# johnpeterflynn/surface-texture-inpainting-net

Hardware: AMD Instinct MI355X
Metric: vertices/sec forward+backward on 200k-vert ScanNet mesh; scatter-add GB/s vs HBM roofline (higher is better)
Workload: dtype f32; 1 GPU; STINet 3-D config, synthetic mesh 200704 vertices / 1200642 directed edges / 3 levels per GPU, step = plan build + fwd + L1 + bwd + all-reduce + Adam; vertices_per_gpu=200704, edges_per_gpu=1200642, levels=3, parallelism=dp1, hip_graph=False

## Files before the change

include/stin_hip.h:

```cpp
#ifndef STIN_HIP_H
#define STIN_HIP_H

#include <stddef.h>
#include <stdint.h>

#ifdef __cplusplus
extern "C" {
#endif

#define STIN_VERSION 102

#define STIN_OK 0
#define STIN_E_NULL (-1)
#define STIN_E_SIZE (-2)
#define STIN_E_ALIGN (-3)
#define STIN_E_WORKSPACE (-4)
#define STIN_E_UNSUPPORTED (-5)

typedef void* stin_stream_t;
typedef void* stin_event_t;
typedef uint16_t stin_bf16_t;

int stin_version(void);
const char* stin_error_string(int code);
// ... 44 lines not shown
int stin_relabel_many_i64(const stin_relabel_job_t* jobs, int n_jobs, stin_stream_t stream);
int stin_narrow_i64_to_i32(const int64_t* src, int64_t n, int64_t limit, int32_t* dst, int32_t* bad,
                           stin_stream_t stream);

#define STIN_SEG_NONTEMPORAL 2
int stin_segment_sum_f32(const float* src, int64_t ld_src, const int32_t* rowptr, const int32_t* col,
                         int64_t N, int C, int mean, float* out, int64_t ld_out, stin_stream_t stream);

int stin_edge_relu_mean_fwd_f32(const float* A, int64_t lda, const float* B, int64_t ldb,
                                const int32_t* rowptr, const int32_t* col, int64_t N, int H,
                                float* out, int64_t ldo, int indicator, uint32_t* mask, stin_stream_t stream);
int stin_edge_relu_mean_fwd_map_f32(const float* A, int64_t lda, const float* B, int64_t ldb, const int32_t* rowptr,
                                    const int32_t* col, const int32_t* row_map, int64_t N, int H, float* out, int64_t ldo,
                                    int indicator, uint32_t* mask, stin_stream_t stream);
int stin_edge_relu_mean_bwd_dst_mask_f32(const float* G, int64_t ldg, const uint32_t* mask, const int32_t* rowptr,
                                         int64_t N, int H, float* dA, int64_t ldda, stin_stream_t stream);
int stin_edge_relu_mean_bwd_src_mask_f32(const float* G, int64_t ldg, const float* w_src, const uint32_t* mask,
                                         const int32_t* rowptr_src, const int32_t* col_src, const int32_t* xslot,
                                         int64_t N, int H, float* dB, int64_t lddb, stin_stream_t stream);
int stin_edge_relu_mean_bwd_mask_f32(const float* G, int64_t ldg, const uint32_t* mask, const int32_t* rowptr_dst,
                                     const float* w_src, const int32_t* rowptr_src, const int32_t* col_src,
                                     const int32_t* xslot, int64_t N, int H, float* dA, int64_t ldda, float* dB,
                                     int64_t lddb, const float* copy_src, int64_t ld_copy_src, float* copy_dst,
                                     int64_t ld_copy_dst, int C_copy, stin_stream_t stream);
int stin_edge_relu_mean_fwd_ti_f32(const float* b1, const float* B, int64_t ldb, const int32_t* rowptr, const int32_t* col,
                                   int64_t N, int H, float* out, int64_t ldo, int indicator, uint32_t* mask, stin_stream_t stream);
int64_t stin_edge_bwd_ti_colsum_rows(int64_t N, int H);
int stin_edge_bwd_ti_colsum_fold_f32(const float* colsum, int64_t rows, int H, float* db1, stin_stream_t stream);
int stin_edge_relu_mean_bwd_mask_ti_f32(const float* G, int64_t ldg, const uint32_t* mask, const int32_t* rowptr_dst,
                                        const float* w_src, const int32_t* rowptr_src, const int32_t* col_src,
                                        const int32_t* xslot, int64_t N, int H, float* D, int64_t ldd, const float* copy_src,
                                        int64_t ld_copy_src, float* copy_dst, int64_t ld_copy_dst, int C_copy, float* colsum,
                                        int64_t colsum_rows, stin_stream_t stream);
int stin_edge_relu_mean_bwd_dst_f32(const float* A, int64_t lda, const float* B, int64_t ldb,
                                    const float* G, int64_t ldg, const int32_t* rowptr,
                                    const int32_t* col, int64_t N, int H, float* dA, int64_t ldda,
                                    stin_stream_t stream);
int stin_edge_relu_mean_bwd_src_f32(const float* A, int64_t lda, const float* B, int64_t ldb,
                                    const float* G, int64_t ldg, const float* inv_deg,
                                    const int32_t* rowptr_src, const int32_t* col_src, int64_t N, int H,
                                    float* dB, int64_t lddb, stin_stream_t stream);

int stin_pool_max_fwd_f32(const float* x, int64_t ldx, const int32_t* rowptr, const int32_t* col,
                          int64_t n_coarse, int C, float* out, int64_t ldo, int32_t* arg,
                          stin_stream_t stream);
int stin_pool_max_bwd_f32(const float* g, int64_t ldg, const int32_t* arg, const int32_t* trace,
                          int64_t n_fine, int C, float* gx, int64_t ldgx, stin_stream_t stream);
int stin_gather_rows_f32(const float* src, int64_t ld_src, const int32_t* idx, const float* row_scale,
                         int64_t n_out, int C, float* out, int64_t ldo, stin_stream_t stream);
int stin_gather_add_rows_f32(const float* a, int64_t lda, const int32_t* idx_a, const float* b, int64_t ldb,
                             const int32_t* idx_b, int64_t n_out, int C, float* out, int64_t ldo, stin_stream_t stream);
int64_t stin_segment_mean_stats_groups(int64_t N, int C);
int stin_segment_mean_stats_f32(const float* src, int64_t ld_src, const int32_t* rowptr, const int32_t* col, int64_t N, int C,
                                float* out, int64_t ldo, double* partial, size_t partial_bytes, stin_stream_t stream);
int64_t stin_gather_add_rows_stats_groups(int64_t N, int C);
int stin_gather_add_rows_stats_f32(const float* a, int64_t lda, const int32_t* idx_a, const float* b, int64_t ldb,
                                   const int32_t* idx_b, int64_t N, int C, float* out, int64_t ldo, double* partial,
                                   size_t partial_bytes, stin_stream_t stream);
int stin_batch_pool_i64(const int64_t* batch, const int32_t* rowptr, const int32_t* col, int64_t n_coarse,
                        int64_t* out, stin_stream_t stream);
int stin_gather_i64(const int64_t* src, const int32_t* idx, int64_t n_out, int64_t* out,
                    stin_stream_t stream);
int stin_norm_group_ids_i64(const int64_t* batch, const int32_t* ptr_sum, int B, int64_t n_rows, int32_t* gid, int32_t* sid,
                            stin_stream_t stream);

#define STIN_RED_SUM 0
#define STIN_RED_CSQ 1
#define STIN_RED_DOT_ELU 2
#define STIN_RED_COEF_XC 3
#define STIN_RED_MOMENTS 4
#define STIN_RED_DOT_BN 5
#define STIN_RED_DOT_BN_RELU 6
#define STIN_POST_NONE 0
#define STIN_POST_SCALE 1
#define STIN_POST_RSTD 2
#define STIN_POST_NORM_COEF 3
size_t stin_colreduce_workspace_bytes(int C, int B);
int stin_colreduce_f32(int mode, const float* x, int64_t ldx, const float* gout, int64_t ldg, int64_t N,
                       int C, const int32_t* ptr, int B, const int32_t* gid, const int32_t* sid,
                       const float* mean, const float* rstd, const float* coef, int post,
                       const float* inv_cnt, float eps, float* out0, float* out1,
                       void* workspace, size_t workspace_bytes, stin_stream_t stream);
int stin_norm_act_res_fwd_f32(const float* x, int64_t ldx, const float* mean, const float* rstd,
                              const int32_t* gid, const float* res, int64_t ldres, int64_t N, int C, int act,
                              float* y, int64_t ldy, stin_stream_t stream);
int stin_norm_act_res_fwd_map_f32(const float* x, int64_t ldx, const float* mean, const float* rstd, const int32_t* gid,
                                  const float* res, int64_t ldres, const int32_t* row_map, int64_t N, int C, int act, float* y,
                                  int64_t ldy, stin_stream_t stream);
int stin_norm_act_bwd_f32(const float* x, int64_t ldx, const float* gout, int64_t ldg, const float* mean,
                          const float* rstd, const float* a, const float* k, const float* m,
                          const int32_t* gid, const int32_t* sid, int64_t N, int C, int act, float* dx,
                          int64_t lddx, stin_stream_t stream);

#define STIN_GEMM_F32 0
#define STIN_GEMM_BF16X3 2
#define STIN_GEMM_BF16X6 3
#define STIN_GEMM_F16X3 4
#define STIN_GEMM_W_BF16 0x200
#define STIN_GEMM_W_PRESPLIT 0x100
#define STIN_GEMM_W_FRAG 0x400
int stin_gemm_w_is_frag(int Nc, int K);
int stin_gemm_split_weights_f32(const float* W, int64_t ldw, int Nc, int K, int precision, float* out, int64_t ldo,
                                stin_stream_t stream);
int stin_gemm_nt_f32(const float* A, int64_t lda, const float* W, int64_t ldw, const float* bias,
                     const float* row_mask, int64_t ld_mask, const float* residual, int64_t ld_res, int64_t M,
                     int Nc, int K, float* C, int64_t ldc, int precision, stin_stream_t stream);
size_t stin_gemm_tn_workspace_bytes(int64_t M, int Nc, int K, int ones_column);
int stin_gemm_tn_f32(const float* G, int64_t ldg, const float* X, int64_t ldx, int64_t M, int Nc, int K,
                     int ones_column, const float* row_weight, int64_t ld_weight, float* dW, int64_t lddw,
                     int precision, void* workspace, size_t workspace_bytes, stin_stream_t stream);

int stin_gemm_tn_wb_f32(const float* G, int64_t ldg, const float* X, int64_t ldx, int64_t M, int Nc, int K,
                        const float* row_weight, int64_t ld_weight, float* dW, int64_t lddw, float* db, int precision,
                        void* workspace, size_t workspace_bytes, stin_stream_t stream);

size_t stin_linear_tanh_bwd_workspace_bytes(int64_t N, int K, int Nc);
int stin_linear_tanh_fwd_f32(const float* x, int64_t ldx, const float* W, const float* b, int64_t N, int K, int Nc, float* y,
                             stin_stream_t stream);
int stin_linear_tanh_bwd_f32(const float* g, const float* y, const float* x, int64_t ldx, const float* W, int64_t N, int K, int Nc,
                             float* dx, int64_t lddx, float* dW, float* db, void* workspace, size_t workspace_bytes,
                             stin_stream_t stream);

int stin_cols_axpy_rowmask_f32(float* dst, int64_t ldd, const float* src, int64_t lds, const int32_t* rowptr, int64_t N, int c0,
                               int c1, float alpha, stin_stream_t stream);
int stin_cols_axpy_rowmask_bf16(stin_bf16_t* dst, int64_t ldd, const stin_bf16_t* src, int64_t lds, const int32_t* rowptr,
                                int64_t N, int c0, int c1, float alpha, stin_stream_t stream);

int stin_pad_rows_f32(const float* x, int64_t ldx, int64_t N, int Cin, int Cp, float* out, stin_stream_t stream);
int stin_pad_rows_bf16(const stin_bf16_t* x, int64_t ldx, int64_t N, int Cin, int Cp, stin_bf16_t* out, stin_stream_t stream);

int64_t stin_gemm_nt_dotelu_groups(int64_t M, int Nc, int K, int precision);
int stin_gemm_nt_dotelu_f32(const float* A, int64_t lda, const float* W, int64_t ldw, const float* bias, const float* residual,
                            int64_t ld_res, int64_t M, int Nc, int K, float* C, int64_t ldc, int precision, const float* nx,
                            int64_t ld_nx, const float* nmean, const float* nrstd, double* partial, size_t partial_bytes,
                            stin_stream_t stream);
int stin_norm_coef_from_partials_f32(const double* partial, int64_t groups, int C, const float* rstd, const float* inv_cnt,
                                     float* k, float* m, stin_stream_t stream);

int stin_bn_act_fwd_f32(const float* x, int64_t ldx, const float* mean, const float* rstd, const float* gamma,
                        const float* beta, int64_t N, int C, int act, float* y, int64_t ldy, stin_stream_t stream);
int stin_bn_act_bwd_f32(const float* x, int64_t ldx, const float* gout, int64_t ldg, const float* mean, const float* rstd,
                        const float* gamma, const float* beta, const float* P, const float* Q, float inv_n, int64_t N,
                        int C, int act, float* dx, int64_t lddx, stin_stream_t stream);

int stin_bn_mean_bwd_f32(const float* m, int64_t ldm, const float* g, int64_t ldg, const int32_t* dst, const float* inv_deg,
                         const float* mean, const float* rstd, const float* gamma, const float* P, const float* Q,
                         float inv_e, int64_t E, int C, float* dm, int64_t lddm, stin_stream_t stream);

int stin_bn_running_stats_f32(const float* mean, const float* rstd, int C, float eps, float unbias, float momentum,
                              float* running_mean, float* running_var, stin_stream_t stream);

int stin_gemm_nt_bn_f32(const float* A, int64_t lda, const float* W, int64_t ldw, const float* mean, const float* rstd,
                        const float* gamma, const float* beta, int64_t M, int Nc, int K, float* C, int64_t ldc, int precision,
                        stin_stream_t stream);
int stin_gemm_tn_bn_f32(const float* G, int64_t ldg, const float* X, int64_t ldx, const float* mean, const float* rstd,
                        const float* gamma, const float* beta, int64_t M, int Nc, int K, float* dW, int64_t lddw, int precision,
                        void* workspace, size_t workspace_bytes, stin_stream_t stream);
int stin_gemm_nt_stream_f32(const float* A, int64_t lda, const float* W, int64_t ldw, const float* mean, const float* rstd,
                            const float* gamma, const float* beta, int64_t M, int Nc, int K, float* C, int64_t ldc, int precision,
                            stin_stream_t stream);
int64_t stin_gemm_nt_bn_bwd_groups(int64_t M, int Nc, int K, int precision);
int stin_gemm_nt_bn_bwd_stats_f32(const float* A, int64_t lda, const float* W, int64_t ldw, const float* X, int64_t ldx,
                                  const float* mean, const float* rstd, const float* gamma, const float* beta, int64_t M, int Nc,
                                  int K, int precision, double* partial, size_t partial_bytes, float* sums, stin_stream_t stream);
int stin_gemm_nt_bn_bwd_apply_f32(const float* A, int64_t lda, const float* W, int64_t ldw, const float* X, int64_t ldx,
                                  const float* mean, const float* rstd, const float* gamma, const float* beta, const float* sums,
                                  float inv_n, int64_t M, int Nc, int K, float* dx, int64_t lddx, int precision,
                                  stin_stream_t stream);
int stin_scmn_pack_f32(const float* W1, const float* W2, const float* gamma1, const float* beta1, const float* gamma2,
                       const float* beta2, int cin, int h2, int cout, int trans_inv, float* wcat, float* wcatT, float* w2T,
                       float* gb1, float* gb2, stin_stream_t stream);
int stin_scmn_unpack_f32(const float* dwcat, int cin, int h2, int trans_inv, float* dW1, stin_stream_t stream);
int stin_bn_affine_res_fwd_f32(const float* x, int64_t ldx, const float* mean, const float* rstd, const float* gamma,
                               const float* beta, const int32_t* rowptr, const float* res, int64_t ldres, int64_t N, int C,
                               int relu, float* y, int64_t ldy, stin_stream_t stream);
int stin_relu_mask_bwd_f32(const float* g, int64_t ldg, const float* y, int64_t ldy, const int32_t* rowptr, int64_t N, int C,
                           int relu, float* g_eff, float* g_in, stin_stream_t stream);
int stin_concat_unpool_f32(const float* skip, int64_t ld_skip, const float* coarse, int64_t ld_coarse, const int32_t* trace, int64_t N,
                           int cs, int cu, float* out, int64_t ldo, stin_stream_t stream);

typedef struct stin_pack_job {
    const float *W1, *b1, *Ws, *bs, *W2;
    float *wcat, *bcat, *wcatT, *w2T, *w2s;
    int Cin, Cp, H, Cout, has_shortcut, trans_inv, fwd_split, bwd_split;
} stin_pack_job_t;
int stin_edgeconv_pack_many_f32(const stin_pack_job_t* jobs_device, int n_jobs, int64_t max_elems, stin_stream_t stream);
int stin_edgeconv_pack_f32(const float* W1, const float* b1, const float* Ws, const float* bs, const float* W2,
                           int Cin, int Cp, int H, int Cout, int has_shortcut, int trans_inv, float* wcat,
                           float* bcat, float* wcatT, float* w2T, float* w2s, int fwd_split, int bwd_split,
                           stin_stream_t stream);
int stin_edgeconv_unpack_grads_f32(const float* dwb, const float* dw2b, int Cin, int Cp, int H, int Cout,
                                   int has_shortcut, int trans_inv, float* dW1, float* db1, float* dWs, float* dbs,
                                   float* dW2, float* db2, stin_stream_t stream);
int stin_norm_bwd_coef_f32(const float* T1, const float* S0, const float* rstd, const float* inv_cnt, int B, int C,
                           float* k, float* m, stin_stream_t stream);
int stin_norm_bwd_coef_m_quirk_f32(const float* S0, const float* U, const float* rstd, const float* inv_cnt, int B, int C,
                                   float* m, stin_stream_t stream);

size_t stin_masked_l1_workspace_bytes(int64_t N, int C);
int stin_masked_l1_loss_f32(const float* out, const float* color, const int64_t* mask, int64_t N, int C,
                            int use_weight, float* loss, float* grad, void* workspace, size_t workspace_bytes,
                            stin_stream_t stream);
#define STIN_SEG_MIN_CLASSES 2
#define STIN_SEG_MAX_CLASSES 128
size_t stin_seg_ce_workspace_bytes(int64_t N);
int stin_seg_ce_fwd_f32(const float* logits, int64_t ld, int64_t M, const int64_t* rows, const int64_t* target, int64_t N, int C,
                        const float* weight, int64_t ignore_index, float* loss, double* den, int64_t* confusion, int32_t* bad,
                        void* workspace, size_t workspace_bytes, stin_stream_t stream);
int stin_seg_ce_bwd_f32(const float* logits, int64_t ld, const int64_t* target, int64_t N, int C, const float* weight,
                        int64_t ignore_index, const float* grad_loss, const double* den, float* dlogits, int64_t ldd,
                        stin_stream_t stream);
size_t stin_total_variation_workspace_bytes(int64_t N);
int stin_total_variation_f32(const float* x, int64_t ldx, const int32_t* rowptr_dst, const int32_t* col_dst, int64_t N, int C,
                             float* out, void* workspace, size_t workspace_bytes, stin_stream_t stream);
int stin_graph_laplace_f32(const float* x, int64_t ldx, const int32_t* rowptr_dst, const int32_t* col_dst, int64_t N, int C,
                           float* out, int64_t ldo, stin_stream_t stream);
#define STIN_METRICS_ONE_PASS 0
#define STIN_METRICS_STAGED 1
size_t stin_inpaint_metrics_workspace_bytes(int64_t N);
int stin_inpaint_metrics_f32(const float* out, int64_t ldo, const float* color, const int64_t* mask, const int32_t* rowptr_dst,
                             const int32_t* col_dst, const int32_t* perm, int64_t N, int C, int composite, int use_weight,
                             float data_range, const float* loss, int layout, float* row_out, void* workspace,
                             size_t workspace_bytes, stin_stream_t stream);
int stin_adam_f32(float* p, const float* g, float* m, float* v, float* vmax, int64_t n, double lr, double beta1,
                  double beta2, double eps, double weight_decay, int step, int amsgrad, stin_stream_t stream);

int64_t stin_gemm_nt_colstats_groups(int64_t M, int Nc, int K, int precision);
int stin_gemm_nt_colstats_f32(const float* A, int64_t lda, const float* W, int64_t ldw, const float* bias,
                              const float* row_mask, int64_t ld_mask, const float* residual, int64_t ld_res, int64_t M,
                              int Nc, int K, float* C, int64_t ldc, int precision, double* colstats, size_t colstats_bytes,
                              stin_stream_t stream);
int stin_moments_final_f32(const double* partial, int64_t groups, int C, const float* inv_cnt, float eps, float* mean,
                           float* rstd, stin_stream_t stream);
int stin_norm_fold_rows(int64_t N, int C, int64_t groups);
int stin_norm_act_res_fwd_fold_f32(const double* partial, int64_t groups, const float* x, int64_t ldx, const float* res,
                                   int64_t ldres, const float* inv_cnt, float eps, int64_t N, int C, float* mean, float* rstd,
                                   float* y, int64_t ldy, stin_stream_t stream);
int stin_norm_act_res_fwd_fold_map_f32(const double* partial, int64_t groups, const float* x, int64_t ldx, const float* res,
                                       int64_t ldres, const int32_t* row_map, const float* inv_cnt, float eps, int64_t N, int C,
                                       float* mean, float* rstd, float* y, int64_t ldy, stin_stream_t stream);
int stin_norm_act_bwd_fold_f32(const double* partial, int64_t groups, const float* x, int64_t ldx, const float* gout, int64_t ldg,
                               const float* mean, const float* rstd, const float* inv_cnt, int64_t N, int C, float* dx,
                               int64_t lddx, stin_stream_t stream);

int stin_segment_sum_bf16(const stin_bf16_t* src, int64_t ld_src, const int32_t* rowptr, const int32_t* col,
                          int64_t n_rows, int C, int mean, stin_bf16_t* out, int64_t ld_out, stin_stream_t stream);
int stin_edge_relu_mean_fwd_bf16(const stin_bf16_t* A, int64_t lda, const stin_bf16_t* B, int64_t ldb,
                                 const int32_t* rowptr, const int32_t* col, int64_t N, int H, stin_bf16_t* out,
                                 int64_t ldo, int indicator, uint32_t* mask, stin_stream_t stream);
int stin_edge_relu_mean_bwd_dst_mask_bf16(const stin_bf16_t* G, int64_t ldg, const uint32_t* mask,
                                          const int32_t* rowptr, int64_t N, int H, stin_bf16_t* dA, int64_t ldda,
                                          stin_stream_t stream);
int stin_edge_relu_mean_bwd_src_mask_bf16(const stin_bf16_t* G, int64_t ldg, const float* w_src, const uint32_t* mask,
                                          const int32_t* rowptr_src, const int32_t* col_src, const int32_t* xslot,
                                          int64_t N, int H, stin_bf16_t* dB, int64_t lddb, stin_stream_t stream);
int stin_edge_relu_mean_bwd_mask_bf16(const stin_bf16_t* G, int64_t ldg, const uint32_t* mask, const int32_t* rowptr_dst,
                                      const float* w_src, const int32_t* rowptr_src, const int32_t* col_src,
                                      const int32_t* xslot, int64_t N, int H, stin_bf16_t* dA, int64_t ldda,
                                      stin_bf16_t* dB, int64_t lddb, const stin_bf16_t* copy_src, int64_t ld_copy_src,
                                      stin_bf16_t* copy_dst, int64_t ld_copy_dst, int C_copy, stin_stream_t stream);
int stin_pool_max_fwd_bf16(const stin_bf16_t* x, int64_t ldx, const int32_t* rowptr, const int32_t* col,
                           int64_t n_coarse, int C, stin_bf16_t* out, int64_t ldo, int32_t* arg, stin_stream_t stream);
int stin_pool_max_bwd_bf16(const stin_bf16_t* g, int64_t ldg, const int32_t* arg, const int32_t* trace,
                           int64_t n_fine, int C, stin_bf16_t* gx, int64_t ldgx, stin_stream_t stream);
int stin_gather_rows_bf16(const stin_bf16_t* src, int64_t ld_src, const int32_t* idx, const float* row_scale,
                          int64_t n_out, int C, stin_bf16_t* out, int64_t ldo, stin_stream_t stream);
int stin_colreduce_bf16(int mode, const stin_bf16_t* x, int64_t ldx, const stin_bf16_t* gout, int64_t ldg, int64_t N,
                        int C, const int32_t* ptr, int B, const int32_t* gid, const int32_t* sid, const float* mean,
                        const float* rstd, const float* coef, int post, const float* inv_cnt, float eps, float* out0,
                        float* out1, void* workspace, size_t workspace_bytes, stin_stream_t stream);
int stin_norm_act_res_fwd_bf16(const stin_bf16_t* x, int64_t ldx, const float* mean, const float* rstd,
                               const int32_t* gid, const stin_bf16_t* res, int64_t ldres, int64_t N, int C, int act,
                               stin_bf16_t* y, int64_t ldy, stin_stream_t stream);
int stin_norm_act_bwd_bf16(const stin_bf16_t* x, int64_t ldx, const stin_bf16_t* gout, int64_t ldg, const float* mean,
                           const float* rstd, const float* a, const float* k, const float* m, const int32_t* gid,
                           const int32_t* sid, int64_t N, int C, int act, stin_bf16_t* dx, int64_t lddx,
                           stin_stream_t stream);
int stin_gemm_nt_bf16(const stin_bf16_t* A, int64_t lda, const float* W, int64_t ldw, const float* bias,
                      const stin_bf16_t* row_mask, int64_t ld_mask, const stin_bf16_t* residual, int64_t ld_res,
                      int64_t M, int Nc, int K, void* C, int64_t ldc, int c_is_f32, stin_stream_t stream);
int stin_gemm_tn_bf16(const stin_bf16_t* G, int64_t ldg, const stin_bf16_t* X, int64_t ldx, int64_t M, int Nc, int K,
                      int ones_column, const stin_bf16_t* row_weight, int64_t ld_weight, float* dW, int64_t lddw,
                      void* workspace, size_t workspace_bytes, stin_stream_t stream);
int stin_gemm_tn_wb_bf16(const stin_bf16_t* G, int64_t ldg, const stin_bf16_t* X, int64_t ldx, int64_t M, int Nc, int K,
                         const stin_bf16_t* row_weight, int64_t ld_weight, float* dW, int64_t lddw, float* db,
                         void* workspace, size_t workspace_bytes, stin_stream_t stream);
int stin_linear_tanh_fwd_bf16(const stin_bf16_t* x, int64_t ldx, const float* W, const float* b, int64_t N, int K, int Nc,
                              float* y, stin_stream_t stream);
int stin_linear_tanh_bwd_bf16(const float* g, const float* y, const stin_bf16_t* x, int64_t ldx, const float* W, int64_t N, int K,
                              int Nc, stin_bf16_t* dx, int64_t lddx, float* dW, float* db, void* workspace,
                              size_t workspace_bytes, stin_stream_t stream);

#define STIN_TI_COMPACT 2
#define STIN_BLOCK_PACKED 0x800
size_t stin_edgeconv_block_fwd_workspace_bytes(int Cin, int Cp, int H, int Cout, int has_shortcut, int B);
int stin_edgeconv_block_fwd_pack_offsets(int Cp, int H, int Cout, int has_shortcut, size_t* off_wcat, size_t* off_w2s,
                                         size_t* off_bcat);
size_t stin_edgeconv_block_bwd_workspace_bytes(int64_t N, int Cp, int H, int Cout, int has_shortcut, int B, int storage);
#define STIN_OP_BLOCK 0
#define STIN_OP_POOL_MAX 1
#define STIN_OP_UNPOOL 2
typedef struct stin_net_op {
    int32_t kind, Cin, Cp, H, Cout, has_shortcut, trans_inv, prec_fwd, fwd_split, bwd_split, B, slice_quirk, use_side, y_from_src,
        reserved1, reserved2;
    float eps;
    int32_t reserved3;
    int64_t n_out, n_in, ldx, ldo, lddx, ldy, ldh;
    uint64_t fwd_ws_bytes, bwd_ws_bytes;
    const void* x;
    void* out;
    void* dx;
    const float *W1, *b1, *W2, *b2, *Ws, *bs;
    float *wcatT, *w2T;
    void* fwd_ws;
    const int32_t *rowptr_dst, *col_dst, *rowptr_src, *col_src, *xslot;
    const float* w_src;
    const int32_t *ptr_sum, *ptr_true, *gid, *sid;
    const float* inv_cnt;
    void *Y, *hE;
    uint32_t* mask;
    void* agg;
    float *mean, *rstd;
    int32_t* arg;
    const int32_t* trace;
    float *dW1, *db1, *dW2, *db2, *dWs, *dbs;
    void* bwd_ws;
    stin_event_t ev_dy, ev_done;
    stin_event_t ev_edge0, ev_edge1;
} stin_net_op_t;
int stin_net_fwd(int storage, const stin_net_op_t* ops, int n_ops, stin_stream_t stream);
int stin_net_bwd(int storage, const stin_net_op_t* ops, int n_ops, const void* g, int64_t ldg, int prec_bwd, stin_stream_t stream,
                 stin_stream_t wgrad_stream);

size_t stin_edgeconv_wgrad_workspace_bytes(int64_t N, int Cp, int H, int Cout, int has_shortcut);
int stin_edgeconv_wgrad(int storage, const void* dagg, int64_t ld_dagg, const void* hE, int64_t ldh, const void* dY,
                        int64_t ldy, const void* x, int64_t ldx, int64_t N, int Cin, int Cp, int H, int Cout,
                        int has_shortcut, int trans_inv, int precision, float* dW1, float* db1, float* dW2, float* db2,
                        float* dWs, float* dbs, void* workspace, size_t workspace_bytes, stin_stream_t stream);
int stin_edgeconv_wgrad_ti(int storage, const void* dagg, int64_t ld_dagg, const void* hE, int64_t ldh, const void* dY,
                           int64_t ldy, const void* x, int64_t ldx, int64_t N, int Cin, int Cp, int H, int Cout,
                           int has_shortcut, int trans_inv, int precision, float* dW1, float* db1, float* dW2, float* db2,
                           float* dWs, float* dbs, const float* ti_colsum, int64_t ti_rows, void* workspace,
                           size_t workspace_bytes, stin_stream_t stream);

int stin_dilated_walk_f32(const int32_t* rowptr, const int32_t* col, const int32_t* row_of, const float* pos,
                          const float* nrm, int64_t N, int64_t E, const int32_t* dilations, int n_dil, int32_t* out,
                          stin_stream_t stream);
int stin_dilated_walk_f64(const int32_t* rowptr, const int32_t* col, const int32_t* row_of, const double* pos,
                          const double* nrm, int64_t N, int64_t E, const int32_t* dilations, int n_dil, int32_t* out,
                          stin_stream_t stream);

size_t stin_voxel_cluster_workspace_bytes(int64_t N);
int stin_voxel_cluster_f64(const double* coords, int64_t N, double voxel, int64_t* trace, float* new_coords, int64_t* state,
                           void* workspace, size_t workspace_bytes, stin_stream_t stream);
size_t stin_coalesce_workspace_bytes(int64_t E);
int stin_coalesce_pairs_i64(const int64_t* a, const int64_t* b, const int64_t* map, int64_t map_n, int64_t E, int64_t n, int drop_loops,
                            int64_t* out_a, int64_t* out_b, int64_t* state, void* workspace, size_t workspace_bytes,
                            stin_stream_t stream);

size_t stin_mask_adjacency_workspace_bytes(int64_t N);
int stin_mask_adjacency_i64(const int64_t* src, const int64_t* dst, int64_t E, int64_t N, int32_t* rowptr, int32_t* col,
                            int32_t* bad, void* workspace, size_t workspace_bytes, stin_stream_t stream);
size_t stin_circle_mask_workspace_bytes(int64_t N, int num_masks, int num_graphs);
int stin_circle_mask_run(const int32_t* rowptr, const int32_t* col, int64_t N, const int64_t* ptr, int num_graphs, int num_masks,
                         int radius, double frac, uint64_t seed, const int64_t* graph_seeds, int max_iters, const int64_t* centres,
                         int64_t num_centres,
                         int32_t* dist, int64_t* mask, int64_t* info, int64_t* centre_log, int64_t log_cap, void* workspace,
                         size_t workspace_bytes, stin_stream_t stream);
int stin_augment_rewrite_f32(float* x, int64_t ldx, const float* color, int64_t ldc, const int32_t* dist, int radius, int64_t* mask,
                             int64_t N, const float* lin, const float* rot, stin_stream_t stream);

#define STIN_CROP_VERTICES 0
#define STIN_CROP_EDGES 1
#define STIN_CROP_DILATED 2
#define STIN_CROP_OCCURS 3
#define STIN_CROP_TRACE 4
#define STIN_CROP_MAX_SEGS 1024
#define STIN_CROP_MAX_CROPS 65535
typedef struct stin_crop_seg {
    int64_t kind, level, vseg, aux, n, base, width, ibase;
    const void* src;
    void* out;
    int64_t* ids_out;
    void *p0, *p1;
    int64_t reserved[3];
} stin_crop_seg_t;
size_t stin_crop_workspace_bytes(int64_t total);
int stin_crop_mark(const stin_crop_seg_t* segs, int n_segs, int64_t max_n, const double* boxes, int n_crops, int64_t total,
                   int64_t inbox_total, uint8_t* inbox, uint8_t* flags, int32_t* pos, int64_t* bounds, int32_t* status,
                   void* workspace, size_t workspace_bytes, stin_stream_t stream);
int stin_crop_gather(const stin_crop_seg_t* segs, int n_segs, int64_t max_n, int n_crops, const uint8_t* flags, const int32_t* pos,
                     stin_stream_t stream);
int stin_crop_traces(const stin_crop_seg_t* segs, int n_segs, int64_t max_n, int n_crops, const uint8_t* flags, const int32_t* pos,
                     int32_t* info, int32_t* status, stin_stream_t stream);
size_t stin_label_pool_workspace_bytes(int64_t n0, int n_labels);
int stin_label_pool_i64(const int64_t* trace0, const int64_t* labels, int64_t n_orig, int64_t n0, int n_labels, int64_t* out,
                        int32_t* status, void* workspace, size_t workspace_bytes, stin_stream_t stream);

int stin_nearest_chunks(int64_t Q, int64_t P);
size_t stin_nearest_workspace_bytes(int64_t Q, int chunks);
int stin_nearest_f64(const double* queries, int64_t n_query_rows, const double* points, int64_t P, const int64_t* q_index,
                     const int64_t* q_count, int64_t Q, int chunks, int64_t* out_index, double* out_d2, int64_t* flags,
                     void* workspace, size_t workspace_bytes, stin_stream_t stream);
size_t stin_trace_workspace_bytes(int64_t n_old, int64_t n_new);
int stin_trace_scatter_i64(const int64_t* new_id, const int64_t* row_ptr, int64_t R, const int64_t* old_id, const int64_t* row_of,
                           int64_t n_entries, int64_t n_old, int64_t n_new, int64_t* trace, int64_t* state, void* workspace,
                           size_t workspace_bytes, stin_stream_t stream);
int stin_trace_unassigned_i64(const int64_t* trace, int64_t n_old, int64_t* list, int64_t* state, stin_stream_t stream);
int stin_trace_check_i64(const int64_t* trace, int64_t n_old, const int64_t* row_ptr, int64_t R, int64_t n_new, int64_t* state,
                         void* workspace, size_t workspace_bytes, stin_stream_t stream);
int stin_cluster_mean_f32(const float* coords, int64_t n, const int64_t* order, const int64_t* seg_ptr, int64_t n_seg, float* out,
                          stin_stream_t stream);

#ifdef __cplusplus
}
#endif
#endif
```

surface_texture_inpainting_net_amd/csrc/stin_block.hip:

```cpp
#include "stin_common.h"

namespace {

inline size_t up256(size_t v) { return (v + 255) & ~(size_t)255; }
inline char* align256(void* p) { return reinterpret_cast<char*>((reinterpret_cast<uintptr_t>(p) + 255) & ~(uintptr_t)255); }
inline char* carve(char*& p, size_t bytes) {
    char* r = p;
    p += up256(bytes);
    return r;
}
#define STIN_TRY(expr)            \
    do {                          \
        const int rc_ = (expr);   \
        if (rc_ != STIN_OK) return rc_; \
    } while (0)

inline const void* col_off(const void* base, int64_t cols, int storage) {
    return static_cast<const char*>(base) + cols * (storage ? 2 : 4);
}

inline size_t yw_wide(int H, int Cout, int has_shortcut) { return 2 * (size_t)H + (has_shortcut ? Cout : 0); }

struct BwdLayout {
    size_t dagg, dhE, dY;
    size_t coef[5];
    size_t red, red_bytes;
    size_t tn;
};
inline BwdLayout bwd_layout(int64_t N, int H, int Cout, int has_shortcut, int B, int storage) {
    const size_t es = storage ? 2 : 4;
    BwdLayout L;
    size_t o = 0;
    auto take = [&o](size_t bytes) {
        const size_t r = o;
        o += up256(bytes);
        return r;
    };
    L.dagg = take((size_t)N * Cout * es);
    L.dhE = take((size_t)N * H * es);
    L.dY = take((size_t)N * yw_wide(H, Cout, has_shortcut) * es);
    for (size_t& c : L.coef) c = take((size_t)B * Cout * 4);
    L.red_bytes = stin_colreduce_workspace_bytes(Cout, B);
    L.red = take(L.red_bytes);
    L.tn = o;
    return L;
}

inline int colreduce(int storage, int mode, const void* x, int64_t ldx, const void* gout, int64_t ldg, int64_t N, int C, const int32_t* ptr,
                     int B, const int32_t* gid, const int32_t* sid, const float* mean, const float* rstd, const float* coef, int post,
                     const float* inv_cnt, float eps, float* out0, float* out1, void* ws, size_t ws_bytes, stin_stream_t stream) {
    if (storage)
        return stin_colreduce_bf16(mode, static_cast<const stin_bf16_t*>(x), ldx, static_cast<const stin_bf16_t*>(gout), ldg, N, C, ptr, B,
                                   gid, sid, mean, rstd, coef, post, inv_cnt, eps, out0, out1, ws, ws_bytes, stream);
    return stin_colreduce_f32(mode, static_cast<const float*>(x), ldx, static_cast<const float*>(gout), ldg, N, C, ptr, B, gid, sid, mean,
                              rstd, coef, post, inv_cnt, eps, out0, out1, ws, ws_bytes, stream);
}

int fwd_stats(int storage, const stin_net_op_t& J, void* red_ws, size_t red_bytes, stin_stream_t stream) {
    if (!J.slice_quirk)
        return colreduce(storage, STIN_RED_MOMENTS, J.agg, J.Cout, nullptr, 0, J.n_out, J.Cout, J.ptr_sum, J.B, J.gid, nullptr, nullptr,
                         nullptr, nullptr, STIN_POST_NONE, J.inv_cnt, J.eps, J.mean, J.rstd, red_ws, red_bytes, stream);
    STIN_TRY(colreduce(storage, STIN_RED_SUM, J.agg, J.Cout, nullptr, 0, J.n_out, J.Cout, J.ptr_sum, J.B, J.gid, nullptr, nullptr, nullptr,
                       nullptr, STIN_POST_SCALE, J.inv_cnt, J.eps, J.mean, nullptr, red_ws, red_bytes, stream));
    return colreduce(storage, STIN_RED_CSQ, J.agg, J.Cout, nullptr, 0, J.n_out, J.Cout, J.ptr_sum, J.B, J.gid, nullptr, J.mean, nullptr,
                     nullptr, STIN_POST_RSTD, J.inv_cnt, J.eps, J.rstd, nullptr, red_ws, red_bytes, stream);
}

int bwd_norm_coef(int storage, const stin_net_op_t& J, const void* g, int64_t ldg, float* const coef[5], void* red_ws, size_t red_bytes,
                  stin_stream_t stream) {
    float *kk = coef[0], *mm = coef[1], *t1 = coef[2], *s0 = coef[3], *uu = coef[4];
    if (!J.sid)
        return colreduce(storage, STIN_RED_DOT_ELU, J.agg, J.Cout, g, ldg, J.n_out, J.Cout, J.ptr_true, J.B, J.gid, nullptr, J.mean, J.rstd,
                         nullptr, STIN_POST_NORM_COEF, J.inv_cnt, 0.f, kk, mm, red_ws, red_bytes, stream);
    STIN_TRY(colreduce(storage, STIN_RED_DOT_ELU, J.agg, J.Cout, g, ldg, J.n_out, J.Cout, J.ptr_true, J.B, J.gid, nullptr, J.mean, J.rstd,
                       nullptr, STIN_POST_NONE, J.inv_cnt, 0.f, t1, s0, red_ws, red_bytes, stream));
    STIN_TRY(stin_norm_bwd_coef_f32(t1, s0, J.rstd, J.inv_cnt, J.B, J.Cout, kk, mm, stream));
    STIN_TRY(colreduce(storage, STIN_RED_COEF_XC, J.agg, J.Cout, nullptr, 0, J.n_out, J.Cout, J.ptr_true, J.B, J.gid, J.sid, J.mean, nullptr,
                       kk, STIN_POST_NONE, J.inv_cnt, 0.f, uu, nullptr, red_ws, red_bytes, stream));
    return stin_norm_bwd_coef_m_quirk_f32(s0, uu, J.rstd, J.inv_cnt, J.B, J.Cout, mm, stream);
}

#define STIN_EDGE_BRACKET(CALL)                                                               \
    do {                                                                                      \
        if (J.ev_edge0) (void)hipEventRecord((hipEvent_t)J.ev_edge0, (hipStream_t)stream);    \
        STIN_TRY(CALL);                                                                       \
        if (J.ev_edge1) (void)hipEventRecord((hipEvent_t)J.ev_edge1, (hipStream_t)stream);    \
    } while (0)

}

extern "C" size_t stin_edgeconv_block_fwd_workspace_bytes(int Cin, int Cp, int H, int Cout, int has_shortcut, int B) {
    if (Cp <= 0 || H <= 0 || Cout <= 0 || B <= 0) return 0;
    const size_t Yw = yw_wide(H, Cout, has_shortcut);
    (void)Cin;
    return up256(Yw * Cp * 4) + up256((size_t)Cout * H * 4) + up256(Yw * 4) + up256(stin_colreduce_workspace_bytes(Cout, B)) + 256;
}

extern "C" int stin_edgeconv_block_fwd_pack_offsets(int Cp, int H, int Cout, int has_shortcut, size_t* off_wcat, size_t* off_w2s,
                                                    size_t* off_bcat) {
    if (Cp <= 0 || H <= 0 || Cout <= 0 || !off_wcat || !off_w2s || !off_bcat) return STIN_E_SIZE;
    *off_wcat = 0;
    *off_w2s = up256(yw_wide(H, Cout, has_shortcut) * Cp * 4);
    *off_bcat = *off_w2s + up256((size_t)Cout * H * 4);
    return STIN_OK;
}

extern "C" size_t stin_edgeconv_block_bwd_workspace_bytes(int64_t N, int Cp, int H, int Cout, int has_shortcut, int B,
                                                          int storage) {
    if (N < 0 || Cp <= 0 || H <= 0 || Cout <= 0 || B <= 0) return 0;
    return bwd_layout(N, H, Cout, has_shortcut, B, storage).tn + up256(stin_edgeconv_wgrad_workspace_bytes(N, Cp, H, Cout, has_shortcut)) + 256;
}

static bool commutes(int storage, const stin_net_op_t& Un, const stin_net_op_t& J) {
    return storage == 0 && Un.kind == STIN_OP_UNPOOL && J.kind == STIN_OP_BLOCK && J.y_from_src != 0 && J.x == Un.out &&
           J.n_out == Un.n_out && J.Cin == Un.Cout && J.Cp == J.Cin && J.ldx == Un.ldo && J.has_shortcut != 0 &&
           J.trans_inv != STIN_TI_COMPACT && Un.trace != nullptr && Un.x != nullptr && Un.n_in > 0;
}

static int block_fwd(int storage, const stin_net_op_t& J, stin_stream_t stream, const stin_net_op_t* Un = nullptr) {
    const int64_t N = J.n_out;
    const int Cp = J.Cp, H = J.H, Cout = J.Cout;
    STIN_REQUIRE(N >= 0 && J.Cin > 0 && Cp >= J.Cin && H > 0 && Cout > 0 && J.B > 0, STIN_E_SIZE);
    STIN_REQUIRE((J.x || Un) && J.W1 && J.W2 && J.rowptr_dst && J.wcatT && J.w2T && J.Y && J.hE && J.agg && J.mean && J.rstd && J.out &&
                     J.fwd_ws,
                 STIN_E_NULL);
    STIN_REQUIRE(J.fwd_ws_bytes >= stin_edgeconv_block_fwd_workspace_bytes(J.Cin, Cp, H, Cout, J.has_shortcut, J.B), STIN_E_WORKSPACE);
    const bool compact = J.trans_inv == STIN_TI_COMPACT;
    STIN_REQUIRE(!compact || storage == 0, STIN_E_UNSUPPORTED);
    const int Yw = stin_yw(H, Cout, J.has_shortcut, J.trans_inv);
    const size_t Yw_max = yw_wide(H, Cout, J.has_shortcut);
    STIN_REQUIRE(J.ldy >= Yw, STIN_E_SIZE);
    char* p = align256(J.fwd_ws);
    float* wcat = reinterpret_cast<float*>(carve(p, Yw_max * Cp * 4));
    float* w2s = reinterpret_cast<float*>(carve(p, (size_t)Cout * H * 4));
    float* bcat = reinterpret_cast<float*>(carve(p, Yw_max * 4));
    void* red_ws = p;
    const size_t red_bytes = stin_colreduce_workspace_bytes(Cout, J.B);

    const bool packed = (J.fwd_split & STIN_BLOCK_PACKED) != 0;
    int fwd_split = J.fwd_split & ~STIN_BLOCK_PACKED, bwd_split = J.bwd_split;
    if (storage == 1) fwd_split = bwd_split = (Cp % 8 == 0 && Cout % 8 == 0) ? STIN_GEMM_W_BF16 : 0;
    if (!packed)
        STIN_TRY(stin_edgeconv_pack_f32(J.W1, J.b1, J.Ws, J.bs, J.W2, J.Cin, Cp, H, Cout, J.has_shortcut, J.trans_inv, wcat, bcat, J.wcatT,
                                        J.w2T, fwd_split ? w2s : nullptr, fwd_split, bwd_split, stream));
    const float* w2_op = fwd_split ? w2s : J.W2;
    const int wbf = (storage == 1 && fwd_split) ? STIN_GEMM_W_BF16 : 0;
    const int pf = fwd_split ? (J.prec_fwd | STIN_GEMM_W_PRESPLIT | (fwd_split & STIN_GEMM_W_FRAG)) : J.prec_fwd;
    const void* res = J.has_shortcut ? col_off(static_cast<const void*>(J.Y), (int64_t)(Yw - Cout), storage) : J.x;
    const int64_t ld_res = J.has_shortcut ? J.ldy : J.ldx;
    if (storage == 0) {
        float* Yf = static_cast<float*>(J.Y);
        float* hf = static_cast<float*>(J.hE);
        float* aggf = static_cast<float*>(J.agg);
        const int32_t* row_map = Un ? Un->trace : nullptr;
        if (Un)
            STIN_TRY(stin_gemm_nt_f32(static_cast<const float*>(Un->x), Un->ldx, wcat, Cp, bcat, nullptr, 0, nullptr, 0, Un->n_in, Yw, Cp,
                                      Yf, J.ldy, pf, stream));
        else
            STIN_TRY(stin_gemm_nt_f32(static_cast<const float*>(J.x), J.ldx, wcat, Cp, bcat, nullptr, 0, nullptr, 0, N, Yw, Cp, Yf, J.ldy,
                                      pf, stream));
        if (Un)
            STIN_EDGE_BRACKET(stin_edge_relu_mean_fwd_map_f32(Yf, J.ldy, Yf + H, J.ldy, J.rowptr_dst, J.col_dst, row_map, N, H, hf, J.ldh,
                                                              1, J.mask, stream));
        else if (compact)
            STIN_EDGE_BRACKET(stin_edge_relu_mean_fwd_ti_f32(J.b1, Yf, J.ldy, J.rowptr_dst, J.col_dst, N, H, hf, J.ldh, 1, J.mask, stream));
        else
            STIN_EDGE_BRACKET(stin_edge_relu_mean_fwd_f32(Yf, J.ldy, Yf + H, J.ldy, J.rowptr_dst, J.col_dst, N, H, hf, J.ldh, 1, J.mask,
                                                          stream));
        const int64_t stat_groups = (J.B == 1 && J.gid == nullptr && !J.slice_quirk) ? stin_gemm_nt_colstats_groups(N, Cout, H, pf) : 0;
        const bool fused_stats = stat_groups > 0 && (size_t)stat_groups * 2 * Cout * sizeof(double) + 256 <= red_bytes;
        bool normed = false;
        if (fused_stats) {
            double* partial = reinterpret_cast<double*>(align256(red_ws));
            STIN_TRY(stin_gemm_nt_colstats_f32(hf, J.ldh, w2_op, H, J.b2, hf + H, J.ldh, nullptr, 0, N, Cout, H, aggf, Cout, pf, partial,
                                               (size_t)stat_groups * 2 * Cout * sizeof(double), stream));
            int rc_fold = STIN_E_UNSUPPORTED;
            if (N > 0 && stin_norm_fold_rows(N, Cout, stat_groups) > 0)
                rc_fold = row_map
                              ? stin_norm_act_res_fwd_fold_map_f32(partial, stat_groups, aggf, Cout, static_cast<const float*>(res), ld_res,
                                                                   row_map, J.inv_cnt, J.eps, N, Cout, J.mean, J.rstd,
                                                                   static_cast<float*>(J.out), J.ldo, stream)
                              : stin_norm_act_res_fwd_fold_f32(partial, stat_groups, aggf, Cout, static_cast<const float*>(res), ld_res,
                                                               J.inv_cnt, J.eps, N, Cout, J.mean, J.rstd, static_cast<float*>(J.out),
                                                               J.ldo, stream);
            if (rc_fold == STIN_OK) normed = true;
            else if (rc_fold != STIN_E_UNSUPPORTED) return rc_fold;
            else STIN_TRY(stin_moments_final_f32(partial, stat_groups, Cout, J.inv_cnt, J.eps, J.mean, J.rstd, stream));
        } else {
            STIN_TRY(stin_gemm_nt_f32(hf, J.ldh, w2_op, H, J.b2, hf + H, J.ldh, nullptr, 0, N, Cout, H, aggf, Cout, pf, stream));
            STIN_TRY(fwd_stats(0, J, red_ws, red_bytes, stream));
        }
        if (!normed && row_map)
            STIN_TRY(stin_norm_act_res_fwd_map_f32(aggf, Cout, J.mean, J.rstd, J.gid, static_cast<const float*>(res), ld_res, row_map, N,
                                                   Cout, 1, static_cast<float*>(J.out), J.ldo, stream));
        else if (!normed)
            STIN_TRY(stin_norm_act_res_fwd_f32(aggf, Cout, J.mean, J.rstd, J.gid, static_cast<const float*>(res), ld_res, N, Cout, 1,
                                               static_cast<float*>(J.out), J.ldo, stream));
    } else {
        stin_bf16_t* Yh = static_cast<stin_bf16_t*>(J.Y);
        stin_bf16_t* hh = static_cast<stin_bf16_t*>(J.hE);
        STIN_TRY(stin_gemm_nt_bf16(static_cast<const stin_bf16_t*>(J.x), J.ldx, wcat, Cp, bcat, nullptr, 0, nullptr, 0, N, Yw, Cp, Yh, J.ldy,
                                   wbf, stream));
        STIN_EDGE_BRACKET(stin_edge_relu_mean_fwd_bf16(Yh, J.ldy, Yh + H, J.ldy, J.rowptr_dst, J.col_dst, N, H, hh, J.ldh, 1, J.mask, stream));
        STIN_TRY(stin_gemm_nt_bf16(hh, J.ldh, w2_op, H, J.b2, hh + H, J.ldh, nullptr, 0, N, Cout, H, J.agg, Cout, wbf, stream));
        STIN_TRY(fwd_stats(1, J, red_ws, red_bytes, stream));
        STIN_TRY(stin_norm_act_res_fwd_bf16(static_cast<const stin_bf16_t*>(J.agg), Cout, J.mean, J.rstd, J.gid,
                                            static_cast<const stin_bf16_t*>(res), ld_res, N, Cout, 1, static_cast<stin_bf16_t*>(J.out),
                                            J.ldo, stream));
    }
    return STIN_OK;
}

struct BwdLink {
    const float* next_agg = nullptr;
    int64_t next_ld = 0;
    const float* next_mean = nullptr;
    const float* next_rstd = nullptr;
    double* next_partial = nullptr;
    size_t next_partial_bytes = 0;
    int64_t produced_groups = 0;
    const double* pre_partial = nullptr;
    int64_t pre_groups = 0;
};

static int block_bwd(int storage, const stin_net_op_t& J, const void* g, int64_t ldg, int prec_bwd, stin_stream_t stream,
                     stin_stream_t wgrad_stream, BwdLink* link) {
    const int64_t N = J.n_out;
    const int Cp = J.Cp, H = J.H, Cout = J.Cout, has_shortcut = J.has_shortcut;
    STIN_REQUIRE(N >= 0 && J.Cin > 0 && Cp >= J.Cin && H > 0 && Cout > 0 && J.B > 0, STIN_E_SIZE);
    STIN_REQUIRE(g && J.x && J.hE && J.mask && J.agg && J.mean && J.rstd && J.wcatT && J.w2T && J.rowptr_dst && J.rowptr_src && J.col_src &&
                     J.xslot && J.w_src && J.inv_cnt && J.dW1 && J.dW2 && J.bwd_ws && (!has_shortcut || J.dWs),
                 STIN_E_NULL);
    STIN_REQUIRE(J.bwd_ws_bytes >= stin_edgeconv_block_bwd_workspace_bytes(N, Cp, H, Cout, has_shortcut, J.B, storage), STIN_E_WORKSPACE);
    const bool compact = J.trans_inv == STIN_TI_COMPACT;
    STIN_REQUIRE(!compact || storage == 0, STIN_E_UNSUPPORTED);
    const int Yw = stin_yw(H, Cout, has_shortcut, J.trans_inv);
    const BwdLayout L = bwd_layout(N, H, Cout, has_shortcut, J.B, storage);
    char* base = align256(J.bwd_ws);
    void* dagg = base + L.dagg;
    void* dhE = base + L.dhE;
    void* dY = base + L.dY;
    float* ti_colsum = nullptr;
    int64_t ti_rows = 0;
    if (compact) {
        ti_rows = stin_edge_bwd_ti_colsum_rows(N, H);
        ti_colsum = reinterpret_cast<float*>(static_cast<char*>(dY) + up256((size_t)N * Yw * 4));
        STIN_REQUIRE(up256((size_t)N * Yw * 4) + (size_t)ti_rows * H * 4 <= up256((size_t)N * yw_wide(H, Cout, has_shortcut) * 4),
                     STIN_E_WORKSPACE);
    }
    float* coef[5];
    for (int i = 0; i < 5; ++i) coef[i] = reinterpret_cast<float*>(base + L.coef[i]);
    float *kk = coef[0], *mm = coef[1];
    const int32_t* sid_n = J.sid ? J.sid : J.gid;
    void* red_ws = base + L.red;
    void* tn_ws = base + L.tn;
    const size_t tn_bytes = (size_t)J.bwd_ws_bytes - (size_t)(static_cast<char*>(tn_ws) - static_cast<char*>(J.bwd_ws));
    const int pb = J.bwd_split ? (prec_bwd | STIN_GEMM_W_PRESPLIT | (J.bwd_split & STIN_GEMM_W_FRAG)) : prec_bwd;
    hipStream_t hs = (hipStream_t)stream;
    const bool side = J.use_side && wgrad_stream != nullptr && wgrad_stream != stream;
    if (side) STIN_REQUIRE(J.ev_dy && J.ev_done, STIN_E_NULL);
    stin_stream_t ws_ = side ? wgrad_stream : stream;
    bool bind_on = false;
    if (side && N > 0 && J.ev_edge1 == nullptr) {
        hipStreamCaptureStatus cs = hipStreamCaptureStatusNone;
        bind_on = hipStreamIsCapturing(hs, &cs) == hipSuccess && cs == hipStreamCaptureStatusNone;
    }
    struct StopEventGuard { ~StopEventGuard() { stin_tl_stop_event = nullptr; } } stop_event_guard;
    bool bound = false;
    auto fork = [&]() -> int {
        if (!side) return STIN_OK;
        hipError_t e = bound ? hipSuccess : hipEventRecord((hipEvent_t)J.ev_dy, hs);
        if (e == hipSuccess) e = hipStreamWaitEvent((hipStream_t)wgrad_stream, (hipEvent_t)J.ev_dy, 0);
        return (int)e;
    };

    if (storage == 0) {
        const float* gf = static_cast<const float*>(g);
        const float* hf = static_cast<const float*>(J.hE);
        const float* aggf = static_cast<const float*>(J.agg);
        float* dYf = static_cast<float*>(dY);
        if (link != nullptr && link->pre_partial != nullptr && link->pre_groups > 0 && !J.sid && J.B == 1 && J.gid == nullptr) {
            STIN_TRY(stin_norm_coef_from_partials_f32(link->pre_partial, link->pre_groups, Cout, J.rstd, J.inv_cnt, kk, mm, stream));
        } else {
            STIN_TRY(bwd_norm_coef(0, J, g, ldg, coef, red_ws, L.red_bytes, stream));
        }
        STIN_TRY(stin_norm_act_bwd_f32(aggf, Cout, gf, ldg, J.mean, J.rstd, J.rstd, kk, mm, J.gid, sid_n, N, Cout, 1,
                                       static_cast<float*>(dagg), Cout, stream));
        STIN_TRY(stin_gemm_nt_f32(static_cast<const float*>(dagg), Cout, J.w2T, Cout, nullptr, nullptr, 0, nullptr, 0, N, H, Cout,
                                  static_cast<float*>(dhE), H, pb, stream));
        float* dYs = dYf + (Yw - Cout);
        const bool ride = has_shortcut && N > 0 && Cout % 4 == 0 && ldg % 4 == 0 && Yw % 4 == 0 && stin_aligned16(gf) &&
                          stin_aligned16(dYs) && Cout <= H;
        const bool bind = bind_on && (!has_shortcut || ride);
        if (bind) stin_tl_stop_event = (hipEvent_t)J.ev_dy;
        if (compact)
            STIN_EDGE_BRACKET(stin_edge_relu_mean_bwd_mask_ti_f32(static_cast<const float*>(dhE), H, J.mask, J.rowptr_dst, J.w_src,
                                                                 J.rowptr_src, J.col_src, J.xslot, N, H, dYf, Yw, ride ? gf : nullptr, ldg,
                                                                 ride ? dYs : nullptr, Yw, ride ? Cout : 0, ti_colsum, ti_rows, stream));
        else
            STIN_EDGE_BRACKET(stin_edge_relu_mean_bwd_mask_f32(static_cast<const float*>(dhE), H, J.mask, J.rowptr_dst, J.w_src, J.rowptr_src,
                                                              J.col_src, J.xslot, N, H, dYf, Yw, dYf + H, Yw, ride ? gf : nullptr, ldg,
                                                              ride ? dYs : nullptr, Yw, ride ? Cout : 0, stream));
        if (has_shortcut && N > 0 && !ride) {
            hipError_t e = hipMemcpy2DAsync(dYs, (size_t)Yw * 4, gf, (size_t)ldg * 4, (size_t)Cout * 4, (size_t)N,
                                            hipMemcpyDeviceToDevice, hs);
            if (e != hipSuccess) return (int)e;
        }
        bound = bind && stin_tl_stop_event == nullptr;
        stin_tl_stop_event = nullptr;
        STIN_TRY(fork());
        STIN_TRY(stin_edgeconv_wgrad_ti(0, dagg, Cout, hf, J.ldh, dYf, Yw, J.x, J.ldx, N, J.Cin, Cp, H, Cout, has_shortcut, J.trans_inv,
                                        prec_bwd, J.dW1, J.db1, J.dW2, J.db2, J.dWs, J.dbs, ti_colsum, ti_rows, tn_ws, tn_bytes, ws_));
        if (J.dx != nullptr) {
            const bool link_ok = link != nullptr && link->next_agg != nullptr && link->next_ld % 4 == 0 && stin_aligned16(link->next_agg) &&
                                 stin_aligned16(link->next_mean) && stin_aligned16(link->next_rstd) && link->next_partial != nullptr;
            const int64_t lg = link_ok ? stin_gemm_nt_dotelu_groups(N, Cp, Yw, pb) : 0;
            if (lg > 0 && (size_t)lg * 2 * Cp * sizeof(double) <= link->next_partial_bytes) {
                STIN_TRY(stin_gemm_nt_dotelu_f32(dYf, Yw, J.wcatT, Yw, nullptr, has_shortcut ? nullptr : gf, ldg, N, Cp, Yw,
                                                 static_cast<float*>(J.dx), J.lddx, pb, link->next_agg, link->next_ld, link->next_mean,
                                                 link->next_rstd, link->next_partial, link->next_partial_bytes, stream));
                link->produced_groups = lg;
            } else {
                STIN_TRY(stin_gemm_nt_f32(dYf, Yw, J.wcatT, Yw, nullptr, nullptr, 0, has_shortcut ? nullptr : gf, ldg, N, Cp, Yw,
                                          static_cast<float*>(J.dx), J.lddx, pb, stream));
            }
        }
    } else {
        const stin_bf16_t* gh = static_cast<const stin_bf16_t*>(g);
        const stin_bf16_t* hh = static_cast<const stin_bf16_t*>(J.hE);
        stin_bf16_t* dYh = static_cast<stin_bf16_t*>(dY);
        STIN_TRY(bwd_norm_coef(1, J, g, ldg, coef, red_ws, L.red_bytes, stream));
        STIN_TRY(stin_norm_act_bwd_bf16(static_cast<const stin_bf16_t*>(J.agg), Cout, gh, ldg, J.mean, J.rstd, J.rstd, kk, mm, J.gid, sid_n,
                                        N, Cout, 1, static_cast<stin_bf16_t*>(dagg), Cout, stream));
        const int wbb = (Cp % 8 == 0 && Cout % 8 == 0) ? STIN_GEMM_W_BF16 : 0;
        STIN_TRY(stin_gemm_nt_bf16(static_cast<const stin_bf16_t*>(dagg), Cout, J.w2T, Cout, nullptr, nullptr, 0, nullptr, 0, N, H, Cout,
                                   dhE, H, wbb, stream));
        const bool ride = has_shortcut && N > 0 && Cout % 8 == 0 && ldg % 8 == 0 && Yw % 8 == 0 && stin_aligned16(gh) &&
                          stin_aligned16(dYh + 2 * H);
        const bool bind = bind_on && (!has_shortcut || ride);
        if (bind) stin_tl_stop_event = (hipEvent_t)J.ev_dy;
        STIN_EDGE_BRACKET(stin_edge_relu_mean_bwd_mask_bf16(static_cast<const stin_bf16_t*>(dhE), H, J.mask, J.rowptr_dst, J.w_src,
                                                           J.rowptr_src, J.col_src, J.xslot, N, H, dYh, Yw, dYh + H, Yw, ride ? gh : nullptr,
                                                           ldg, ride ? dYh + 2 * H : nullptr, Yw, ride ? Cout : 0, stream));
        if (has_shortcut && N > 0 && !ride) {
            hipError_t e = hipMemcpy2DAsync(dYh + 2 * H, (size_t)Yw * 2, gh, (size_t)ldg * 2, (size_t)Cout * 2, (size_t)N,
                                            hipMemcpyDeviceToDevice, hs);
            if (e != hipSuccess) return (int)e;
        }
        bound = bind && stin_tl_stop_event == nullptr;
        stin_tl_stop_event = nullptr;
        STIN_TRY(fork());
        STIN_TRY(stin_edgeconv_wgrad(1, dagg, Cout, hh, J.ldh, dYh, Yw, J.x, J.ldx, N, J.Cin, Cp, H, Cout, has_shortcut, J.trans_inv, prec_bwd,
                                     J.dW1, J.db1, J.dW2, J.db2, J.dWs, J.dbs, tn_ws, tn_bytes, ws_));
        if (J.dx != nullptr)
            STIN_TRY(stin_gemm_nt_bf16(dYh, Yw, J.wcatT, Yw, nullptr, nullptr, 0, has_shortcut ? nullptr : gh, ldg, N, Cp, Yw, J.dx, J.lddx,
                                       wbb, stream));
    }
    if (side || J.ev_done != nullptr) {
        hipError_t e = hipEventRecord((hipEvent_t)J.ev_done, side ? (hipStream_t)wgrad_stream : hs);
        if (e != hipSuccess) return (int)e;
    }
    return STIN_OK;
}

extern "C" int stin_net_fwd(int storage, const stin_net_op_t* ops, int n_ops, stin_stream_t stream) {
    STIN_REQUIRE(n_ops >= 0 && (n_ops == 0 || ops != nullptr), STIN_E_NULL);
    STIN_REQUIRE(storage == 0 || storage == 1, STIN_E_UNSUPPORTED);
    for (int i = 0; i < n_ops; ++i) {
        const stin_net_op_t& J = ops[i];
        if (J.kind == STIN_OP_BLOCK) {
            const stin_net_op_t* un = (i > 0 && commutes(storage, ops[i - 1], J)) ? &ops[i - 1] : nullptr;
            STIN_REQUIRE(un != nullptr || J.y_from_src == 0, STIN_E_UNSUPPORTED);
            STIN_TRY(block_fwd(storage, J, stream, un));
        } else if (J.kind == STIN_OP_POOL_MAX) {
            if (storage)
                STIN_TRY(stin_pool_max_fwd_bf16(static_cast<const stin_bf16_t*>(J.x), J.ldx, J.rowptr_dst, J.col_dst, J.n_out, J.Cout,
                                                static_cast<stin_bf16_t*>(J.out), J.ldo, J.arg, stream));
            else
                STIN_TRY(stin_pool_max_fwd_f32(static_cast<const float*>(J.x), J.ldx, J.rowptr_dst, J.col_dst, J.n_out, J.Cout,
                                               static_cast<float*>(J.out), J.ldo, J.arg, stream));
        } else if (J.kind == STIN_OP_UNPOOL) {
            if (J.out == nullptr && i + 1 < n_ops && commutes(storage, J, ops[i + 1])) continue;
            if (storage)
                STIN_TRY(stin_gather_rows_bf16(static_cast<const stin_bf16_t*>(J.x), J.ldx, J.trace, nullptr, J.n_out, J.Cout,
                                               static_cast<stin_bf16_t*>(J.out), J.ldo, stream));
            else
                STIN_TRY(stin_gather_rows_f32(static_cast<const float*>(J.x), J.ldx, J.trace, nullptr, J.n_out, J.Cout,
                                              static_cast<float*>(J.out), J.ldo, stream));
        } else {
            return STIN_E_UNSUPPORTED;
        }
    }
    return STIN_OK;
}

extern "C" int stin_net_bwd(int storage, const stin_net_op_t* ops, int n_ops, const void* g, int64_t ldg, int prec_bwd,
                            stin_stream_t stream, stin_stream_t wgrad_stream) {
    STIN_REQUIRE(n_ops >= 0 && (n_ops == 0 || ops != nullptr), STIN_E_NULL);
    STIN_REQUIRE(storage == 0 || storage == 1, STIN_E_UNSUPPORTED);
    const void* gi = g;
    int64_t ldgi = ldg;
    const double* pre_partial = nullptr;
    int64_t pre_groups = 0;
    for (int i = n_ops - 1; i >= 0; --i) {
        const stin_net_op_t& J = ops[i];
        STIN_REQUIRE(J.dx != nullptr || i == 0, STIN_E_NULL);
        if (J.kind == STIN_OP_BLOCK) {
            BwdLink link;
            link.pre_partial = pre_partial;
            link.pre_groups = pre_groups;
            pre_partial = nullptr;
            pre_groups = 0;
            if (storage == 0 && i > 0 && J.dx != nullptr && ops[i - 1].kind == STIN_OP_BLOCK) {
                const stin_net_op_t& Pn = ops[i - 1];
                if (Pn.B == 1 && Pn.gid == nullptr && Pn.sid == nullptr && Pn.n_out == J.n_out && Pn.Cout == J.Cp && J.Cin == J.Cp &&
                    Pn.bwd_ws != nullptr) {
                    const BwdLayout Ln = bwd_layout(Pn.n_out, Pn.H, Pn.Cout, Pn.has_shortcut, Pn.B, storage);
                    link.next_agg = static_cast<const float*>(Pn.agg);
                    link.next_ld = Pn.Cout;
                    link.next_mean = Pn.mean;
                    link.next_rstd = Pn.rstd;
                    link.next_partial = reinterpret_cast<double*>(align256(Pn.bwd_ws) + Ln.red);
                    link.next_partial_bytes = Ln.red_bytes > 256 ? Ln.red_bytes - 256 : 0;
                }
            }
            STIN_TRY(block_bwd(storage, J, gi, ldgi, prec_bwd, stream, wgrad_stream, &link));
            if (link.produced_groups > 0) {
                pre_partial = link.next_partial;
                pre_groups = link.produced_groups;
            }
        } else if (J.kind == STIN_OP_POOL_MAX) {
            if (J.dx != nullptr) {
                if (storage)
                    STIN_TRY(stin_pool_max_bwd_bf16(static_cast<const stin_bf16_t*>(gi), ldgi, J.arg, J.trace, J.n_in, J.Cout,
                                                    static_cast<stin_bf16_t*>(J.dx), J.lddx, stream));
                else
                    STIN_TRY(stin_pool_max_bwd_f32(static_cast<const float*>(gi), ldgi, J.arg, J.trace, J.n_in, J.Cout,
                                                   static_cast<float*>(J.dx), J.lddx, stream));
            }
        } else if (J.kind == STIN_OP_UNPOOL) {
            if (J.dx != nullptr) {
                if (storage)
                    STIN_TRY(stin_segment_sum_bf16(static_cast<const stin_bf16_t*>(gi), ldgi, J.rowptr_dst, J.col_dst, J.n_in, J.Cout, 0,
                                                   static_cast<stin_bf16_t*>(J.dx), J.lddx, stream));
                else
                    STIN_TRY(stin_segment_sum_f32(static_cast<const float*>(gi), ldgi, J.rowptr_dst, J.col_dst, J.n_in, J.Cout,
                                                  (J.n_out * (int64_t)J.Cout * 4 > ((int64_t)256 << 20)) ? STIN_SEG_NONTEMPORAL : 0,
                                                  static_cast<float*>(J.dx), J.lddx, stream));
            }
        } else {
            return STIN_E_UNSUPPORTED;
        }
        gi = J.dx;
        ldgi = J.lddx;
    }
    return STIN_OK;
}
```

surface_texture_inpainting_net_amd/csrc/stin_common.h:

```cpp
#pragma once
#include <hip/hip_runtime.h>
#include <hip/hip_ext.h>
#include <stdint.h>
#include "../../include/stin_hip.h"

static_assert(sizeof(stin_plan_job_t) == 120, "stin_plan_job_t layout");
static_assert(sizeof(stin_order_level_t) == 32, "stin_order_level_t layout");
static_assert(sizeof(stin_relabel_job_t) == 64, "stin_relabel_job_t layout");
static_assert(sizeof(stin_pack_job_t) == 112, "stin_pack_job_t layout");
static_assert(sizeof(stin_net_op_t) == 480, "stin_net_op_t layout");
static_assert(sizeof(stin_crop_seg_t) == 128, "stin_crop_seg_t layout");

#define STIN_WAVE 64

#define STIN_REQUIRE(cond, code) \
    do {                         \
        if (!(cond)) return (code); \
    } while (0)

static inline void stin_clear_stale_error() { (void)hipGetLastError(); }

extern thread_local hipEvent_t stin_tl_stop_event;
#define STIN_LAUNCH_STOP(KERNEL, GRID, BLOCK_, STREAM, ...)                                                          \
    do {                                                                                                             \
        if (stin_tl_stop_event != nullptr) {                                                                         \
            hipExtLaunchKernelGGL(KERNEL, GRID, BLOCK_, 0, STREAM, nullptr, stin_tl_stop_event, 0, __VA_ARGS__);     \
            stin_tl_stop_event = nullptr;                                                                            \
        } else {                                                                                                     \
            hipLaunchKernelGGL(KERNEL, GRID, BLOCK_, 0, STREAM, __VA_ARGS__);                                        \
        }                                                                                                            \
    } while (0)

static inline int stin_launch_status() {
    hipError_t e = hipGetLastError();
    return e == hipSuccess ? STIN_OK : (int)e;
}

__host__ __device__ static inline bool stin_w_frag_shape(int Nc, int K) {
    if (K % 64 != 0) return false;
    if ((Nc == 256 && K >= 512) || (Nc == 128 && K >= 256)) return true;
    return Nc % 32 == 0 && K >= 128 && K <= 256 && Nc >= 320;
}

__host__ __device__ static inline int stin_yw(int H, int Cout, int has_shortcut, int trans_inv) {
    return (trans_inv == STIN_TI_COMPACT ? H : 2 * H) + (has_shortcut ? Cout : 0);
}

#include <atomic>
static inline int stin_ticket_slot(std::atomic<unsigned>& seq_eager, std::atomic<unsigned>& seq_captured, int slots, hipStream_t stream) {
    hipStreamCaptureStatus cs = hipStreamCaptureStatusNone;
    const bool capturing = hipStreamIsCapturing(stream, &cs) == hipSuccess && cs != hipStreamCaptureStatusNone;
    const unsigned half = (unsigned)slots / 2;
    if (capturing) return (int)(half + seq_captured.fetch_add(1, std::memory_order_relaxed) % half);
    return (int)(seq_eager.fetch_add(1, std::memory_order_relaxed) % half);
}

static inline int stin_device_slot() {
    int d = 0;
    return (hipGetDevice(&d) == hipSuccess && d >= 0 && d < 64) ? d : 0;
}
static inline int stin_cu_count_dev() {
    static std::atomic<int> n[64];
    const int d = stin_device_slot();
    int v = n[d].load(std::memory_order_relaxed);
    if (v == 0) {
        if (hipDeviceGetAttribute(&v, hipDeviceAttributeMultiprocessorCount, d) != hipSuccess || v <= 0) v = 256;
        n[d].store(v, std::memory_order_relaxed);
    }
    return v;
}
struct stin_once_per_device {
    std::atomic<unsigned long long> mask{0};
    bool first() {
        const unsigned long long bit = 1ull << stin_device_slot();
        return (mask.fetch_or(bit, std::memory_order_relaxed) & bit) == 0;
    }
};

static inline bool stin_aligned16(const void* p) { return (reinterpret_cast<uintptr_t>(p) & 15u) == 0; }

static inline int stin_group_lanes(int c4) {
    int g = 1;
    while (g < c4 && g < STIN_WAVE) g <<= 1;
    return g;
}

__device__ __forceinline__ float4 ld4(const float* p) { return *reinterpret_cast<const float4*>(p); }
__device__ __forceinline__ void st4(float* p, float4 v) { *reinterpret_cast<float4*>(p) = v; }

typedef __bf16 stin_bf16;
typedef __bf16 stin_bf16x4 __attribute__((ext_vector_type(4)));
__device__ __forceinline__ float4 ld4(const stin_bf16* p) {
    const uint2 r = *reinterpret_cast<const uint2*>(p);
    return make_float4(__uint_as_float(r.x << 16), __uint_as_float(r.x & 0xffff0000u), __uint_as_float(r.y << 16),
                       __uint_as_float(r.y & 0xffff0000u));
}
__device__ __forceinline__ void st4(stin_bf16* p, float4 v) {
    stin_bf16x4 h = {(stin_bf16)v.x, (stin_bf16)v.y, (stin_bf16)v.z, (stin_bf16)v.w};
    *reinterpret_cast<stin_bf16x4*>(p) = h;
}
__device__ __forceinline__ float ld1(const float* p) { return *p; }
__device__ __forceinline__ float ld1(const stin_bf16* p) { return (float)*p; }
__device__ __forceinline__ void st1(float* p, float v) { *p = v; }
__device__ __forceinline__ void st1(stin_bf16* p, float v) { *p = (stin_bf16)v; }

template <typename T> static inline bool stin_aligned_vec4(const void* p) {
    return (reinterpret_cast<uintptr_t>(p) & (4 * sizeof(T) - 1)) == 0;
}

struct stin_bn_tf {
    const float *mean, *rstd, *gamma, *beta;
};
__device__ __forceinline__ void stin_bn_st(const stin_bn_tf& tf, int c, float& s, float& t) {
    s = tf.gamma[c] * tf.rstd[c];
    t = tf.beta[c] - tf.mean[c] * s;
}
__device__ __forceinline__ float stin_bn_relu(float v, float s, float t) { return fmaxf(v * s + t, 0.f); }
struct stin_bn_coef4 {
    float4 s, t;
};
__device__ __forceinline__ stin_bn_coef4 stin_bn_coef4_load(const stin_bn_tf& tf, int c) {
    stin_bn_coef4 q;
    stin_bn_st(tf, c, q.s.x, q.t.x);
    stin_bn_st(tf, c + 1, q.s.y, q.t.y);
    stin_bn_st(tf, c + 2, q.s.z, q.t.z);
    stin_bn_st(tf, c + 3, q.s.w, q.t.w);
    return q;
}
__device__ __forceinline__ float4 stin_bn_relu4(float4 v, const stin_bn_coef4& q) {
    return make_float4(stin_bn_relu(v.x, q.s.x, q.t.x), stin_bn_relu(v.y, q.s.y, q.t.y), stin_bn_relu(v.z, q.s.z, q.t.z),
                       stin_bn_relu(v.w, q.s.w, q.t.w));
}
__device__ __forceinline__ float4 stin_bn_relu4_ragged(float4 v, const stin_bn_tf& tf, int c, int lim) {
    float s, t;
    if (c + 0 < lim) { stin_bn_st(tf, c, s, t); v.x = stin_bn_relu(v.x, s, t); }
    if (c + 1 < lim) { stin_bn_st(tf, c + 1, s, t); v.y = stin_bn_relu(v.y, s, t); }
    if (c + 2 < lim) { stin_bn_st(tf, c + 2, s, t); v.z = stin_bn_relu(v.z, s, t); }
    if (c + 3 < lim) { stin_bn_st(tf, c + 3, s, t); v.w = stin_bn_relu(v.w, s, t); }
    return v;
}

struct stin_tn_problem {
    stin_bn_tf xtf;
    const float *G, *X, *row_w;
    float* slab;
    int64_t ldg, ldx, ld_w, M, chunks;
    int Nc, K, Kq, has_bias, rows_per_chunk, tiles_i, tiles_j, TI, TJ, vec;
    unsigned block0;
};
struct stin_tn_batch {
    stin_tn_problem p[2];
    int n;
};
int stin_tn_problem_init(stin_tn_problem* p, int storage, const void* G, int64_t ldg, const void* X, int64_t ldx, int64_t M,
                         int Nc, int K, int ones_column, const void* row_w, int64_t ld_w, int precision, float* slab,
                         int* ws_eligible);
int stin_tn_slabs(const stin_tn_problem* p, int storage, int precision, stin_stream_t stream);
bool stin_tn_ws_enabled();
int stin_tn_ws_launch(stin_tn_batch batch, stin_stream_t stream);
```

surface_texture_inpainting_net_amd/csrc/stin_gemm.hip:

```cpp
#include <cstdlib>
#include <type_traits>
#include "stin_common.h"

namespace {

typedef float f32x16 __attribute__((ext_vector_type(16)));

constexpr int BLOCK = 256;
constexpr int BK = 32;

__device__ __forceinline__ bool nt_block_tile(int64_t M, int Nc, int BM, int BN, int64_t& m0, int& n0) {
    const int64_t L = blockIdx.x;
    const int ncol = (Nc + BN - 1) / BN;
    if ((M + BM - 1) / BM < 16) {
        m0 = (L / ncol) * BM;
        n0 = (int)(L % ncol) * BN;
        return true;
    }
    const int64_t j = L >> 3;
    const int64_t rt = (j / ncol) * 8 + (L & 7);
    if (rt * BM >= M) return false;
    m0 = rt * BM;
    n0 = (int)(j % ncol) * BN;
    return true;
// ... 176 lines not shown
            else
                hipLaunchKernelGGL((k_gemm_nt_bf16s<128, 128, 2, 2, 2, _Float16, true, true>), grid, dim3(BLOCK), 0, stream, STIN_NT_ARGS);
        } else {
            dim3 grid(nt_grid(M, Nc, 64, 64));
            if (precision == STIN_GEMM_BF16X3)
                hipLaunchKernelGGL((k_gemm_nt_bf16s<64, 64, 2, 2, 2, __bf16, true, true>), grid, dim3(BLOCK), 0, stream, STIN_NT_ARGS);
            else
                hipLaunchKernelGGL((k_gemm_nt_bf16s<64, 64, 2, 2, 2, _Float16, true, true>), grid, dim3(BLOCK), 0, stream, STIN_NT_ARGS);
        }
    } else if (precision == STIN_GEMM_BF16X3) STIN_NT_PICK(k_gemm_nt_bf16s, 2, __bf16);
    else if (precision == STIN_GEMM_BF16X6) STIN_NT_PICK(k_gemm_nt_bf16s, 3, __bf16);
    else if (precision == STIN_GEMM_F16X3) STIN_NT_PICK(k_gemm_nt_bf16s, 2, _Float16);
    else STIN_NT_PICK(k_gemm_nt);
#undef STIN_NT_PICK
#undef STIN_NT
#undef STIN_NT_ARGS
    return stin_launch_status();
}

extern "C" int stin_gemm_nt_stream_f32(const float* A, int64_t lda, const float* W, int64_t ldw, const float* mean, const float* rstd,
                                       const float* gamma, const float* beta, int64_t M, int Nc, int K, float* C, int64_t ldc,
                                       int precision, stin_stream_t stream);
namespace {
constexpr int64_t STREAM_MIN_ROWS = 65536;
inline bool stream_enabled() {
    const char* e = getenv("STIN_NT_STREAM");
    return e == nullptr || atoi(e) != 0;
}
}

extern "C" int stin_gemm_nt_f32(const float* A, int64_t lda, const float* W, int64_t ldw, const float* bias,
                                const float* row_mask, int64_t ld_mask, const float* residual, int64_t ld_res, int64_t M,
                                int Nc, int K, float* C, int64_t ldc, int precision, stin_stream_t stream) {
    if (M >= STREAM_MIN_ROWS && bias == nullptr && row_mask == nullptr && residual == nullptr && stream_enabled()) {
        const int rc = stin_gemm_nt_stream_f32(A, lda, W, ldw, nullptr, nullptr, nullptr, nullptr, M, Nc, K, C, ldc, precision, stream);
        if (rc != STIN_E_UNSUPPORTED) return rc;
    } else if (M >= STREAM_MIN_ROWS && stream_enabled()) {
        const int rc = stream_nt_epi_try(A, lda, W, ldw, bias, row_mask, ld_mask, residual, ld_res, M, Nc, K, C, ldc, precision, (hipStream_t)stream, 0);
        if (rc != STIN_E_UNSUPPORTED) return rc;
    }
    return gemm_nt_f32_impl(A, lda, W, ldw, bias, row_mask, ld_mask, residual, ld_res, M, Nc, K, C, ldc, precision, nullptr, stream);
}

extern "C" int stin_gemm_nt_bn_f32(const float* A, int64_t lda, const float* W, int64_t ldw, const float* mean, const float* rstd,
                                   const float* gamma, const float* beta, int64_t M, int Nc, int K, float* C, int64_t ldc,
                                   int precision, stin_stream_t stream) {
    STIN_REQUIRE((precision & (STIN_GEMM_W_PRESPLIT | STIN_GEMM_W_FRAG)) == 0, STIN_E_UNSUPPORTED);
    if (M >= STREAM_MIN_ROWS && mean != nullptr && stream_enabled()) {
        const int rc = stin_gemm_nt_stream_f32(A, lda, W, ldw, mean, rstd, gamma, beta, M, Nc, K, C, ldc, precision, stream);
        if (rc != STIN_E_UNSUPPORTED) return rc;
    }
    stin_bn_tf tf;
    tf.mean = mean;
    tf.rstd = rstd;
    tf.gamma = gamma;
    tf.beta = beta;
    return gemm_nt_f32_impl(A, lda, W, ldw, nullptr, nullptr, 0, nullptr, 0, M, Nc, K, C, ldc, precision, nullptr, stream, nullptr, &tf);
}

namespace {
struct StreamGeo {
    int kc, nt, ncb, bpc;
    size_t lds;
    int64_t gx;
};
inline bool stream_geo(int64_t M, int Nc, int K, bool tf, StreamGeo* g, int mode = 0, int precision = STIN_GEMM_BF16X3) {
    if (M <= 0 || Nc <= 0 || Nc % 4 != 0 || K < 64 || K > 512 || K % 64 != 0) return false;
    g->kc = 64;
    const char* e = getenv("STIN_NT_STREAM_NT");
    int nt = e != nullptr ? atoi(e) : 0;
    if (nt != 2 && nt != 4) nt = (Nc <= 64 || mode == 1) ? 2 : 4;
    const size_t esz = precision == STIN_GEMM_BF16X6 ? 6 : 4;
    auto lds_of = [&](int nt_) { return esz * ((size_t)K * 32 * nt_ + (size_t)128 * g->kc) + (tf ? (size_t)8 * K : 0) + (mode != 0 ? (size_t)24 * 32 * nt_ : 0); };
    if (lds_of(nt) > 160 * 1024) nt = 2;
    if (lds_of(nt) > 160 * 1024) return false;
    g->nt = nt;
    g->lds = lds_of(nt);
    if (g->lds < 4 * 2 * 32 * nt * sizeof(double)) g->lds = 4 * 2 * 32 * nt * sizeof(double);
    g->ncb = (Nc + 32 * nt - 1) / (32 * nt);
    g->bpc = (int)((160 * 1024) / g->lds);
    if (g->bpc > 2) g->bpc = 2;
    int64_t gx = (int64_t)stin_cu_count() * g->bpc / g->ncb;
    if (gx < 1) gx = 1;
    const int64_t need = ((M + 31) / 32 + 3) / 4;
    g->gx = need < gx ? need : gx;
    return true;
}
inline bool stream_ok(const float* A, int64_t lda, const float* W, int64_t ldw, const float* X, int64_t ldx, const float* C, int64_t ldc,
                      int precision) {
    return lda % 4 == 0 && ldw % 4 == 0 && stin_aligned16(A) && stin_aligned16(W) && ldx % 4 == 0 && ldc % 4 == 0 && stin_aligned16(X) &&
           stin_aligned16(C) &&
           (precision == STIN_GEMM_BF16X3 || precision == STIN_GEMM_BF16X6 || precision == STIN_GEMM_F16X3);
}
struct StreamEpi {
    const float *bias = nullptr, *row_mask = nullptr, *res = nullptr;
    int64_t ld_mask = 0, ld_res = 0;
    int wpre = 0;
};
template <int MODE, bool TF>
int stream_launch(const float* A, int64_t lda, const float* W, int64_t ldw, const float* X, int64_t ldx, const stin_bn_tf& tf,
                  const float* P, const float* Q, float inv_n, int64_t M, int Nc, int K, double* partial, float* C, int64_t ldc,
                  int precision, hipStream_t stream, const StreamEpi epi = StreamEpi()) {
    StreamGeo g;
    if (!stream_geo(M, Nc, K, TF, &g, MODE, precision)) return STIN_E_UNSUPPORTED;
    const dim3 grid((unsigned)g.gx, (unsigned)g.ncb);
#define STIN_STREAM(KC_, NT_, NS_, PT_)                                                                                              \
    do {                                                                                                                             \
        static stin_once_per_device attr_once;                                                                                                \
        if (attr_once.first()) {                                                                                                             \
            (void)hipFuncSetAttribute((const void*)k_gemm_nt_stream<KC_, NT_, NS_, PT_, MODE, TF>, hipFuncAttributeMaxDynamicSharedMemorySize, \
                                      160 * 1024);                                                                                   \
        }                                                                                                                            \
        hipLaunchKernelGGL((k_gemm_nt_stream<KC_, NT_, NS_, PT_, MODE, TF>), grid, dim3(BLOCK), g.lds, stream, A, lda, W, ldw, M, Nc, K, X, \
                           ldx, tf, P, Q, inv_n, partial, C, ldc, epi.bias, epi.row_mask, epi.ld_mask, epi.res, epi.ld_res, epi.wpre);       \
    } while (0)
#define STIN_STREAM_P(KC_, NT_)                                                  \
    do {                                                                         \
        if (precision == STIN_GEMM_BF16X3) STIN_STREAM(KC_, NT_, 2, __bf16);     \
        else if (precision == STIN_GEMM_BF16X6) STIN_STREAM(KC_, NT_, 3, __bf16); \
        else STIN_STREAM(KC_, NT_, 2, _Float16);                                 \
    } while (0)
    if (g.kc == 64 && g.nt == 2) STIN_STREAM_P(64, 2);
    else if (g.kc == 64) STIN_STREAM_P(64, 4);
    else if (g.nt == 2) STIN_STREAM_P(128, 2);
    else STIN_STREAM_P(128, 4);
#undef STIN_STREAM_P
#undef STIN_STREAM
    return stin_launch_status();
}
}
static int stream_nt_presplit_try(const float* A, int64_t lda, const float* W, int64_t ldw, const float* bias, const float* row_mask,
                                  int64_t ld_mask, const float* residual, int64_t ld_res, int64_t M, int Nc, int K, float* C,
                                  int64_t ldc, int precision, hipStream_t stream) {
    const char* er = getenv("STIN_NT_STREAM_PRE_ROWS");
    const int64_t min_rows = er != nullptr ? atoll(er) : 500000;
    const char* e = getenv("STIN_NT_STREAM");
    if (M < min_rows || (e != nullptr && atoi(e) == 0)) return STIN_E_UNSUPPORTED;
    return stream_nt_epi_try(A, lda, W, ldw, bias, row_mask, ld_mask, residual, ld_res, M, Nc, K, C, ldc, precision, stream, 1);
}
static int stream_nt_epi_try(const float* A, int64_t lda, const float* W, int64_t ldw, const float* bias, const float* row_mask,
                             int64_t ld_mask, const float* residual, int64_t ld_res, int64_t M, int Nc, int K, float* C, int64_t ldc,
                             int precision, hipStream_t stream, int wpre) {
    StreamGeo g;
    if (!(precision == STIN_GEMM_BF16X3 || precision == STIN_GEMM_F16X3) || !stream_geo(M, Nc, K, false, &g, 0, precision) ||
        !stream_ok(A, lda, W, ldw, nullptr, 0, C, ldc, precision) || (bias != nullptr && !stin_aligned16(bias)) ||
        (residual != nullptr && (ld_res % 4 != 0 || !stin_aligned16(residual))))
        return STIN_E_UNSUPPORTED;
    StreamEpi epi;
    epi.bias = bias;
    epi.row_mask = row_mask;
    epi.ld_mask = ld_mask;
    epi.res = residual;
    epi.ld_res = ld_res;
    epi.wpre = wpre;
    stin_bn_tf tf;
    tf.mean = tf.rstd = tf.gamma = tf.beta = nullptr;
    return stream_launch<0, false>(A, lda, W, ldw, nullptr, 0, tf, nullptr, nullptr, 0.f, M, Nc, K, nullptr, C, ldc, precision, stream, epi);
}
extern "C" int64_t stin_gemm_nt_bn_bwd_groups(int64_t M, int Nc, int K, int precision) {
    if (!(precision == STIN_GEMM_BF16X3 || precision == STIN_GEMM_BF16X6 || precision == STIN_GEMM_F16X3)) return 0;
    const char* e = getenv("STIN_NT_BNBWD");
    if (e != nullptr && atoi(e) == 0) return 0;
    StreamGeo g;
    return (K <= 128 && stream_geo(M, Nc, K, false, &g, 1, precision)) ? g.gx : 0;
}
extern "C" int stin_gemm_nt_bn_bwd_stats_f32(const float* A, int64_t lda, const float* W, int64_t ldw, const float* X, int64_t ldx,
                                             const float* mean, const float* rstd, const float* gamma, const float* beta, int64_t M,
                                             int Nc, int K, int precision, double* partial, size_t partial_bytes, float* sums,
                                             stin_stream_t stream) {
    stin_clear_stale_error();
    STIN_REQUIRE(lda >= K && ldw >= K && ldx >= Nc, STIN_E_SIZE);
    StreamGeo g;
    STIN_REQUIRE(K <= 128 && stream_geo(M, Nc, K, false, &g, 1, precision) && stream_ok(A, lda, W, ldw, X, ldx, nullptr, 0, precision), STIN_E_UNSUPPORTED);
    STIN_REQUIRE(A && W && X && mean && rstd && gamma && beta && partial && sums, STIN_E_NULL);
    STIN_REQUIRE(partial_bytes >= (size_t)g.gx * 2 * (size_t)Nc * sizeof(double), STIN_E_WORKSPACE);
    stin_bn_tf tf;
    tf.mean = mean;
    tf.rstd = rstd;
    tf.gamma = gamma;
    tf.beta = beta;
    const int rc = stream_launch<1, false>(A, lda, W, ldw, X, ldx, tf, nullptr, nullptr, 0.f, M, Nc, K, partial, nullptr, 0, precision,
                                           (hipStream_t)stream);
    if (rc != STIN_OK) return rc;
    hipLaunchKernelGGL(k_partial_sums_final, dim3((unsigned)((2 * Nc + 63) / 64)), dim3(1024), 0, (hipStream_t)stream, partial, g.gx, 2 * Nc,
                       sums);
    return stin_launch_status();
}
extern "C" int stin_gemm_nt_bn_bwd_apply_f32(const float* A, int64_t lda, const float* W, int64_t ldw, const float* X, int64_t ldx,
                                             const float* mean, const float* rstd, const float* gamma, const float* beta,
                                             const float* sums, float inv_n, int64_t M, int Nc, int K, float* dx, int64_t lddx,
                                             int precision, stin_stream_t stream) {
    stin_clear_stale_error();
    STIN_REQUIRE(lda >= K && ldw >= K && ldx >= Nc && lddx >= Nc, STIN_E_SIZE);
    StreamGeo g;
    STIN_REQUIRE(K <= 128 && stream_geo(M, Nc, K, false, &g, 2, precision) && stream_ok(A, lda, W, ldw, X, ldx, dx, lddx, precision), STIN_E_UNSUPPORTED);
    STIN_REQUIRE(A && W && X && mean && rstd && gamma && beta && sums && dx, STIN_E_NULL);
    stin_bn_tf tf;
    tf.mean = mean;
    tf.rstd = rstd;
    tf.gamma = gamma;
    tf.beta = beta;
    return stream_launch<2, false>(A, lda, W, ldw, X, ldx, tf, sums, sums + Nc, inv_n, M, Nc, K, nullptr, dx, lddx, precision,
                                   (hipStream_t)stream);
}
extern "C" int stin_gemm_nt_stream_f32(const float* A, int64_t lda, const float* W, int64_t ldw, const float* mean, const float* rstd,
                                       const float* gamma, const float* beta, int64_t M, int Nc, int K, float* C, int64_t ldc,
                                       int precision, stin_stream_t stream) {
    stin_clear_stale_error();
    STIN_REQUIRE(lda >= K && ldw >= K && ldc >= Nc, STIN_E_SIZE);
    StreamGeo g;
    STIN_REQUIRE(stream_geo(M, Nc, K, mean != nullptr, &g, 0, precision) && stream_ok(A, lda, W, ldw, nullptr, 0, C, ldc, precision), STIN_E_UNSUPPORTED);
    STIN_REQUIRE(A && W && C && (mean == nullptr || (rstd && gamma && beta)), STIN_E_NULL);
    stin_bn_tf tf;
    tf.mean = mean;
    tf.rstd = rstd;
    tf.gamma = gamma;
    tf.beta = beta;
    if (mean != nullptr)
        return stream_launch<0, true>(A, lda, W, ldw, nullptr, 0, tf, nullptr, nullptr, 0.f, M, Nc, K, nullptr, C, ldc, precision,
                                      (hipStream_t)stream);
    return stream_launch<0, false>(A, lda, W, ldw, nullptr, 0, tf, nullptr, nullptr, 0.f, M, Nc, K, nullptr, C, ldc, precision,
                                   (hipStream_t)stream);
}

extern "C" int64_t stin_gemm_nt_colstats_groups(int64_t M, int Nc, int K, int precision) {
    const bool ok = (precision & STIN_GEMM_W_PRESPLIT) && (precision & STIN_GEMM_W_FRAG) && Nc <= 256 && stin_w_frag_shape(Nc, K);
    const int p = precision & ~(STIN_GEMM_W_PRESPLIT | STIN_GEMM_W_FRAG);
    if (!ok || M <= 0 || (p != STIN_GEMM_BF16X3 && p != STIN_GEMM_F16X3)) return 0;
    const int pmts = panel_tiles(M, Nc, K);
    if (pmts > 0) return 2 * ((M + 32 * pmts - 1) / (32 * pmts));
    return (M + 63) / 64;
}
extern "C" int stin_gemm_nt_colstats_f32(const float* A, int64_t lda, const float* W, int64_t ldw, const float* bias,
                                         const float* row_mask, int64_t ld_mask, const float* residual, int64_t ld_res,
                                         int64_t M, int Nc, int K, float* C, int64_t ldc, int precision, double* colstats,
                                         size_t colstats_bytes, stin_stream_t stream) {
    const int64_t groups = stin_gemm_nt_colstats_groups(M, Nc, K, precision);
    STIN_REQUIRE(groups > 0, STIN_E_UNSUPPORTED);
    STIN_REQUIRE(colstats != nullptr, STIN_E_NULL);
    STIN_REQUIRE(colstats_bytes >= (size_t)groups * 2 * (size_t)Nc * sizeof(double), STIN_E_WORKSPACE);
    return gemm_nt_f32_impl(A, lda, W, ldw, bias, row_mask, ld_mask, residual, ld_res, M, Nc, K, C, ldc, precision, colstats, stream);
}

extern "C" int64_t stin_gemm_nt_dotelu_groups(int64_t M, int Nc, int K, int precision) {
    const bool ok = (precision & STIN_GEMM_W_PRESPLIT) && (precision & STIN_GEMM_W_FRAG) && stin_w_frag_shape(Nc, K);
    const int p = precision & ~(STIN_GEMM_W_PRESPLIT | STIN_GEMM_W_FRAG);
    if (!ok || M <= 0 || (p != STIN_GEMM_BF16X3 && p != STIN_GEMM_F16X3)) return 0;
    const char* e = getenv("STIN_DOTELU_FUSED");
    if (e != nullptr && atoi(e) == 0) return 0;
    const int pmts = panel_tiles(M, Nc, K);
    return pmts > 0 ? 2 * ((M + 32 * pmts - 1) / (32 * pmts)) : 0;
}
extern "C" int stin_gemm_nt_dotelu_f32(const float* A, int64_t lda, const float* W, int64_t ldw, const float* bias,
                                       const float* residual, int64_t ld_res, int64_t M, int Nc, int K, float* C, int64_t ldc,
                                       int precision, const float* nx, int64_t ld_nx, const float* nmean, const float* nrstd,
                                       double* partial, size_t partial_bytes, stin_stream_t stream) {
    const int64_t groups = stin_gemm_nt_dotelu_groups(M, Nc, K, precision);
    STIN_REQUIRE(groups > 0, STIN_E_UNSUPPORTED);
    STIN_REQUIRE(nx && nmean && nrstd && partial, STIN_E_NULL);
    STIN_REQUIRE(ld_nx >= Nc, STIN_E_SIZE);
    STIN_REQUIRE(ld_nx % 4 == 0 && stin_aligned16(nx) && stin_aligned16(nmean) && stin_aligned16(nrstd), STIN_E_ALIGN);
    STIN_REQUIRE(partial_bytes >= (size_t)groups * 2 * (size_t)Nc * sizeof(double), STIN_E_WORKSPACE);
    NtDotElu de;
    de.x = nx;
    de.ldx = ld_nx;
    de.mean = nmean;
    de.rstd = nrstd;
    return gemm_nt_f32_impl(A, lda, W, ldw, bias, nullptr, 0, residual, ld_res, M, Nc, K, C, ldc, precision, partial, stream, &de);
}

extern "C" size_t stin_gemm_tn_workspace_bytes(int64_t M, int Nc, int K, int ones_column) {
    if (M < 0 || Nc <= 0 || K <= 0) return 0;
    (void)ones_column;
    const int TI = tn_tile(Nc), TJ = tn_tile(K);
    const int tiles = ((Nc + TI - 1) / TI) * ((K + TJ - 1) / TJ);
    int64_t chunks = 1;
    for (int rule = 0; rule < 2; ++rule) {
        const int rows = tn_rows_per_chunk(M, tiles, rule == 1);
        const int64_t c = (M + rows - 1) / rows;
        if (c > chunks) chunks = c;
    }
    if (K <= 16) {
        const int rows = tn_skinny_rows(M);
        const int64_t c = (M + rows - 1) / rows;
        if (c > chunks) chunks = c;
    }
    if (Nc >= 256 && K >= 256) {
        const int rows = tn_rows_per_chunk(M, ((Nc + 255) / 256) * ((K + 255) / 256), true);
        const int64_t c = (M + rows - 1) / rows;
        if (c > chunks) chunks = c;
    }
    return (size_t)chunks * (size_t)tn_chunk_stride(Nc, (K + 3) & ~3) * sizeof(float) + 256;
}

int stin_tn_problem_init(stin_tn_problem* p, int storage, const void* G, int64_t ldg, const void* X, int64_t ldx, int64_t M,
                         int Nc, int K, int ones_column, const void* row_w, int64_t ld_w, int precision, float* slab,
                         int* ws_eligible) {
    STIN_REQUIRE(M >= 0 && Nc > 0 && K > 0 && ldg >= Nc && ldx >= K, STIN_E_SIZE);
    STIN_REQUIRE(slab && (M == 0 || (G && X)), STIN_E_NULL);
    p->xtf.mean = p->xtf.rstd = p->xtf.gamma = p->xtf.beta = nullptr;
    p->G = static_cast<const float*>(G);
    p->X = static_cast<const float*>(X);
    p->row_w = static_cast<const float*>(row_w);
    p->slab = slab;
    p->ldg = ldg;
    p->ldx = ldx;
    p->ld_w = ld_w;
    p->M = M;
    p->Nc = Nc;
    p->K = K;
    const int a16 = storage ? 8 : 4;
    const bool vec16 = (Nc % a16 == 0) && (K % a16 == 0) && (ldg % a16 == 0) && (ldx % a16 == 0) && stin_aligned16(G) && stin_aligned16(X);
    const bool big = storage == 1 && vec16 && tn_b16_big_tile(Nc, K);
    p->TI = big ? 256 : tn_tile(Nc);
    p->TJ = big ? 256 : tn_tile(K);
    if (!big && storage == 0 && precision == STIN_GEMM_BF16X3 && vec16 && M > 0 && Nc >= 32 && K >= 32 && stin_tn_ws_enabled()) {
        p->TI = 128;
        p->TJ = 128;
    }
    p->tiles_i = (Nc + p->TI - 1) / p->TI;
    p->tiles_j = (K + p->TJ - 1) / p->TJ;
    p->rows_per_chunk = tn_rows_per_chunk(M, p->tiles_i * p->tiles_j, big || tn_one_per_cu(storage, precision, p->TI, p->TJ, M));
    if (tn_skinny_shape(storage, Nc, K, ldg, ldx, G, X)) {
        p->TI = p->TJ = 0;
        p->tiles_i = p->tiles_j = 1;
        p->rows_per_chunk = tn_skinny_rows(M);
    }
    p->chunks = M > 0 ? (M + p->rows_per_chunk - 1) / p->rows_per_chunk : 0;
    p->Kq = (K + 3) & ~3;
    p->has_bias = ones_column ? 1 : 0;
    p->block0 = 0;
    const int a = storage ? 8 : 4;
    p->vec = (Nc % a == 0) && (K % a == 0) && (ldg % a == 0) && (ldx % a == 0) && stin_aligned16(G) && stin_aligned16(X);
    if (ws_eligible)
        *ws_eligible = (storage == 0 && precision == STIN_GEMM_BF16X3 && p->TI == 128 && p->TJ == 128 && p->vec && M > 0 &&
                        stin_tn_ws_enabled()) ? 1 : 0;
    return STIN_OK;
}

int stin_tn_slabs(const stin_tn_problem* p, int storage, int precision, stin_stream_t stream_) {
    hipStream_t stream = (hipStream_t)stream_;
    if (p->chunks <= 0) return STIN_OK;
    const int64_t M = p->M, ldg = p->ldg, ldx = p->ldx, ld_weight = p->ld_w, chunks = p->chunks;
    const int Nc = p->Nc, K = p->K, Kq = p->Kq, has_bias = p->has_bias, rows = p->rows_per_chunk, tiles_i = p->tiles_i,
              tiles_j = p->tiles_j, TI = p->TI, TJ = p->TJ;
    const bool vec = p->vec != 0;
    float* slab = p->slab;
    const int64_t blocks = (chunks >= 8 ? ((chunks + 7) / 8) * 8 : chunks) * (int64_t)tiles_i * tiles_j;
    if (storage == 1) {
        const stin_bf16* G = reinterpret_cast<const stin_bf16*>(p->G);
        const stin_bf16* X = reinterpret_cast<const stin_bf16*>(p->X);
        const stin_bf16* row_weight = reinterpret_cast<const stin_bf16*>(p->row_w);
#define STIN_TNK(TI_, TJ_)                                                                                            \
    do {                                                                                                              \
        if (vec) hipLaunchKernelGGL((k_gemm_tn_b16<TI_, TJ_, true>), dim3((unsigned)blocks), dim3(BLOCK), 0, stream, G, ldg, X, ldx, M, Nc, K, Kq, has_bias, row_weight, ld_weight, rows, tiles_i, tiles_j, chunks, slab); \
        else hipLaunchKernelGGL((k_gemm_tn_b16<TI_, TJ_, false>), dim3((unsigned)blocks), dim3(BLOCK), 0, stream, G, ldg, X, ldx, M, Nc, K, Kq, has_bias, row_weight, ld_weight, rows, tiles_i, tiles_j, chunks, slab);    \
    } while (0)
#define STIN_TNTR(WI_, WJ_, MT_, NT_)                                                                                  \
    do {                                                                                                              \
        typedef TrGeom<WI_, WJ_, MT_, NT_> Geo_;                                                                      \
        static stin_once_per_device attr_once;                                                                                 \
        if (attr_once.first()) {                                                                                              \
            (void)hipFuncSetAttribute((const void*)k_gemm_tn_b16_tr<WI_, WJ_, MT_, NT_>, hipFuncAttributeMaxDynamicSharedMemorySize, Geo_::LDS); \
        }                                                                                                             \
        hipLaunchKernelGGL((k_gemm_tn_b16_tr<WI_, WJ_, MT_, NT_>), dim3((unsigned)blocks), dim3(Geo_::THREADS), Geo_::LDS, stream, G, ldg, X, \
                           ldx, M, Nc, K, Kq, has_bias, row_weight, ld_weight, rows, tiles_i, tiles_j, chunks, slab);  \
    } while (0)
        if (TI == 256 && TJ == 256) {
            STIN_TNTR(2, 4, 4, 2);
        } else if (TI == 128 && TJ == 128 && vec && Nc % 8 == 0 && K % 8 == 0 && tn_b16_tr_enabled(Nc, K)) {
            STIN_TNTR(2, 2, 2, 2);
        } else if (TI == 128 && TJ == 128) STIN_TNK(128, 128);
        else if (TI == 128) STIN_TNK(128, 64);
        else if (TJ == 128) STIN_TNK(64, 128);
        else STIN_TNK(64, 64);
#undef STIN_TNK
#undef STIN_TNTR
        return stin_launch_status();
    }
    const float *G = p->G, *X = p->X, *row_weight = p->row_w;
    if (TI == 0) {
        const int kp = (K + 3) & ~3;
        const size_t lds_x = (size_t)rows * (kp + 4) * sizeof(float), lds_o = (size_t)Nc * (kp + 1) * sizeof(float);
        const size_t lds = lds_x > lds_o ? lds_x : lds_o;
#define STIN_TNS(KP_)                                                                                                 \
    hipLaunchKernelGGL((k_gemm_tn_skinny<KP_>), dim3((unsigned)chunks), dim3(BLOCK), lds, stream, G, ldg, X, ldx, M, Nc, K, Kq, has_bias, \
                       row_weight, ld_weight, rows, slab)
        if (K <= 4) STIN_TNS(4);
        else if (K <= 8) STIN_TNS(8);
        else if (K <= 12) STIN_TNS(12);
        else STIN_TNS(16);
#undef STIN_TNS
        return stin_launch_status();
    }
    if (precision == STIN_GEMM_BF16X3 && TI == 128 && TJ == 128 && vec && stin_tn_ws_enabled()) {
        stin_tn_batch batch;
        batch.p[0] = *p;
        batch.p[1] = *p;
        batch.n = 1;
        return stin_tn_ws_launch(batch, stream_);
    }
#define STIN_TN(TI_, TJ_)                                                                                            \
    do {                                                                                                             \
        if (vec) hipLaunchKernelGGL((k_gemm_tn<TI_, TJ_, true>), dim3((unsigned)blocks), dim3(BLOCK), 0, stream, G, ldg, X, ldx, M, Nc, K, Kq, has_bias, row_weight, ld_weight, rows, tiles_i, tiles_j, chunks, slab, p->xtf); \
        else hipLaunchKernelGGL((k_gemm_tn<TI_, TJ_, false>), dim3((unsigned)blocks), dim3(BLOCK), 0, stream, G, ldg, X, ldx, M, Nc, K, Kq, has_bias, row_weight, ld_weight, rows, tiles_i, tiles_j, chunks, slab, p->xtf);    \
    } while (0)
#define STIN_TNB(TI_, TJ_, NS_)                                                                                      \
    do {                                                                                                             \
        if (vec) hipLaunchKernelGGL((k_gemm_tn_bf16s<TI_, TJ_, NS_, true>), dim3((unsigned)blocks), dim3(BLOCK), 0, stream, G, ldg, X, ldx, M, Nc, K, Kq, has_bias, row_weight, ld_weight, rows, tiles_i, tiles_j, chunks, slab, p->xtf); \
        else hipLaunchKernelGGL((k_gemm_tn_bf16s<TI_, TJ_, NS_, false>), dim3((unsigned)blocks), dim3(BLOCK), 0, stream, G, ldg, X, ldx, M, Nc, K, Kq, has_bias, row_weight, ld_weight, rows, tiles_i, tiles_j, chunks, slab, p->xtf);    \
    } while (0)
#define STIN_TN_PICK(LAUNCH, ...)                                   \
    do {                                                            \
        if (TI == 128 && TJ == 128) LAUNCH(128, 128, ##__VA_ARGS__); \
        else if (TI == 128) LAUNCH(128, 64, ##__VA_ARGS__);          \
        else if (TJ == 128) LAUNCH(64, 128, ##__VA_ARGS__);          \
        else LAUNCH(64, 64, ##__VA_ARGS__);                          \
    } while (0)
    if (precision == STIN_GEMM_BF16X3) STIN_TN_PICK(STIN_TNB, 2);
    else if (precision == STIN_GEMM_BF16X6) STIN_TN_PICK(STIN_TNB, 3);
    else STIN_TN_PICK(STIN_TN);
#undef STIN_TN_PICK
#undef STIN_TNB
#undef STIN_TN
    return stin_launch_status();
}

static int gemm_tn_f32_impl(const float* G, int64_t ldg, const float* X, int64_t ldx, int64_t M, int Nc, int K,
                           int ones_column, const float* row_weight, int64_t ld_weight, float* dW, int64_t lddw, float* db,
                           int precision, void* workspace, size_t workspace_bytes, stin_stream_t stream_,
                           const stin_bn_tf* xtf = nullptr) {
    stin_clear_stale_error();
    hipStream_t stream = (hipStream_t)stream_;
    const int Kp = K + ((ones_column && db == nullptr) ? 1 : 0);
    STIN_REQUIRE(M >= 0 && Nc > 0 && K > 0 && ldg >= Nc && ldx >= K && lddw >= Kp, STIN_E_SIZE);
    STIN_REQUIRE(dW && workspace && (M == 0 || (G && X)), STIN_E_NULL);
    STIN_REQUIRE(workspace_bytes >= stin_gemm_tn_workspace_bytes(M, Nc, K, ones_column), STIN_E_WORKSPACE);
    STIN_REQUIRE(precision == STIN_GEMM_F32 || precision == STIN_GEMM_BF16X3 || precision == STIN_GEMM_BF16X6,
                 STIN_E_UNSUPPORTED);
    float* slab = reinterpret_cast<float*>((reinterpret_cast<uintptr_t>(workspace) + 255) & ~(uintptr_t)255);
    stin_tn_problem p;
    int rc = stin_tn_problem_init(&p, 0, G, ldg, X, ldx, M, Nc, K, ones_column, row_weight, ld_weight, precision, slab, nullptr);
    if (rc != STIN_OK) return rc;
    STIN_REQUIRE((size_t)p.chunks * (size_t)tn_chunk_stride(Nc, p.Kq) * sizeof(float) + 256 <= workspace_bytes, STIN_E_WORKSPACE);
    if (xtf != nullptr) {
        STIN_REQUIRE(xtf->mean && xtf->rstd && xtf->gamma && xtf->beta, STIN_E_NULL);
        STIN_REQUIRE(p.TI != 0, STIN_E_UNSUPPORTED);
        p.xtf = *xtf;
        if (!(stin_aligned16(xtf->mean) && stin_aligned16(xtf->rstd) && stin_aligned16(xtf->gamma) && stin_aligned16(xtf->beta))) p.vec = 0;
    }
    rc = stin_tn_slabs(&p, 0, precision, stream_);
    if (rc != STIN_OK) return rc;
    const int64_t n4 = (int64_t)Nc * p.Kq / 4 + (p.has_bias ? (Nc + 3) / 4 : 0);
    hipLaunchKernelGGL(k_reduce_slabs, dim3((unsigned)((n4 + RS_COLS - 1) / RS_COLS)), dim3(BLOCK), 0, stream, slab, p.chunks, Nc, K,
                       p.Kq, p.has_bias, dW, lddw, db);
    return stin_launch_status();
}
extern "C" int stin_gemm_tn_f32(const float* G, int64_t ldg, const float* X, int64_t ldx, int64_t M, int Nc, int K,
                                int ones_column, const float* row_weight, int64_t ld_weight, float* dW, int64_t lddw,
                                int precision, void* workspace, size_t workspace_bytes, stin_stream_t stream_) {
    return gemm_tn_f32_impl(G, ldg, X, ldx, M, Nc, K, ones_column, row_weight, ld_weight, dW, lddw, nullptr, precision, workspace,
                            workspace_bytes, stream_);
}
extern "C" int stin_gemm_tn_bn_f32(const float* G, int64_t ldg, const float* X, int64_t ldx, const float* mean, const float* rstd,
                                   const float* gamma, const float* beta, int64_t M, int Nc, int K, float* dW, int64_t lddw,
                                   int precision, void* workspace, size_t workspace_bytes, stin_stream_t stream_) {
    stin_bn_tf tf;
    tf.mean = mean;
    tf.rstd = rstd;
    tf.gamma = gamma;
    tf.beta = beta;
    return gemm_tn_f32_impl(G, ldg, X, ldx, M, Nc, K, 0, nullptr, 0, dW, lddw, nullptr, precision, workspace, workspace_bytes, stream_, &tf);
}
extern "C" int stin_gemm_tn_wb_f32(const float* G, int64_t ldg, const float* X, int64_t ldx, int64_t M, int Nc, int K,
                                   const float* row_weight, int64_t ld_weight, float* dW, int64_t lddw, float* db, int precision,
                                   void* workspace, size_t workspace_bytes, stin_stream_t stream_) {
    STIN_REQUIRE(db != nullptr, STIN_E_NULL);
    return gemm_tn_f32_impl(G, ldg, X, ldx, M, Nc, K, 1, row_weight, ld_weight, dW, lddw, db, precision, workspace, workspace_bytes,
                            stream_);
}

extern "C" int stin_gemm_nt_bf16(const stin_bf16_t* A_, int64_t lda, const float* W, int64_t ldw, const float* bias,
                                 const stin_bf16_t* row_mask_, int64_t ld_mask, const stin_bf16_t* residual_,
                                 int64_t ld_res, int64_t M, int Nc, int K, void* C, int64_t ldc, int c_is_f32,
                                 stin_stream_t stream_) {
    stin_clear_stale_error();
    hipStream_t stream = (hipStream_t)stream_;
    const stin_bf16* A = reinterpret_cast<const stin_bf16*>(A_);
    const stin_bf16* row_mask = reinterpret_cast<const stin_bf16*>(row_mask_);
    const stin_bf16* residual = reinterpret_cast<const stin_bf16*>(residual_);
    STIN_REQUIRE(M >= 0 && Nc > 0 && K > 0 && lda >= K && ldw >= K && ldc >= Nc, STIN_E_SIZE);
    STIN_REQUIRE(residual == nullptr || ld_res >= Nc, STIN_E_SIZE);
    if (M == 0) return STIN_OK;
    STIN_REQUIRE(A && W && C, STIN_E_NULL);
    const bool wb = (c_is_f32 & STIN_GEMM_W_BF16) != 0;
    c_is_f32 &= 1;
    const bool vec = (K % 8 == 0) && (lda % 8 == 0) && (ldw % (wb ? 8 : 4) == 0) && stin_aligned16(A) && stin_aligned16(W);
    STIN_REQUIRE(!wb || vec, STIN_E_ALIGN);
    const int vec_out = (!c_is_f32 && Nc % 8 == 0 && ldc % 8 == 0 && stin_aligned16(C)) ? 1 : 0;
    const int force_tile = stin_nt_force_tile();
    const bool tall_tile = K >= 512 && ((M + 127) / 128) * ((Nc + 63) / 64) >= 1000;
#define STIN_NTB(BM_, BN_, WM_, WN_, OUT_)                                                                             \
    do {                                                                                                               \
        dim3 grid(nt_grid(M, Nc, BM_, BN_));                                                                           \
        if (wb) hipLaunchKernelGGL((k_gemm_nt_b16<BM_, BN_, WM_, WN_, OUT_, true, true>), grid, dim3(BLOCK), 0, stream, A, lda, W, ldw, bias, row_mask, ld_mask, residual, ld_res, M, Nc, K, (OUT_*)C, ldc, vec_out); \
        else if (vec) hipLaunchKernelGGL((k_gemm_nt_b16<BM_, BN_, WM_, WN_, OUT_, true>), grid, dim3(BLOCK), 0, stream, A, lda, W, ldw, bias, row_mask, ld_mask, residual, ld_res, M, Nc, K, (OUT_*)C, ldc, vec_out); \
        else hipLaunchKernelGGL((k_gemm_nt_b16<BM_, BN_, WM_, WN_, OUT_, false>), grid, dim3(BLOCK), 0, stream, A, lda, W, ldw, bias, row_mask, ld_mask, residual, ld_res, M, Nc, K, (OUT_*)C, ldc, vec_out);    \
    } while (0)
#define STIN_NTB_PICK(OUT_)                                                                          \
    do {                                                                                             \
        if (Nc <= 32) STIN_NTB(128, 32, 4, 1, OUT_);                                                 \
        else if (force_tile == 1) STIN_NTB(128, 128, 2, 2, OUT_);                                    \
        else if (force_tile == 2 || (force_tile == 0 && tall_tile)) STIN_NTB(128, 64, 2, 2, OUT_);   \
        else STIN_NTB(64, 64, 2, 2, OUT_);                                                           \
    } while (0)
    if (wb && K % BKB == 0 && nt_b16_glds_pays(M, Nc, K)) {
        const stin_bf16* Wb = reinterpret_cast<const stin_bf16*>(W);
#define STIN_GLDS(OUT_, WM_, WN_, MT_, NT_)                                                                             \
    do {                                                                                                               \
        typedef GlGeom<WM_, WN_, MT_, NT_> Geo_;                                                                       \
        static stin_once_per_device attr_once;                                                                                  \
        if (attr_once.first()) {                                                                                               \
            (void)hipFuncSetAttribute((const void*)k_gemm_nt_b16_glds<OUT_, WM_, WN_, MT_, NT_>, hipFuncAttributeMaxDynamicSharedMemorySize, Geo_::LDS); \
        }                                                                                                              \
        const int64_t nrow = (M + Geo_::BM - 1) / Geo_::BM, ncol = (Nc + Geo_::BN - 1) / Geo_::BN;                     \
        dim3 grid(ncol % 8 == 0 ? (unsigned)(nrow * ncol) : nt_grid(M, Nc, Geo_::BM, Geo_::BN));                       \
        hipLaunchKernelGGL((k_gemm_nt_b16_glds<OUT_, WM_, WN_, MT_, NT_>), grid, dim3(Geo_::THREADS), Geo_::LDS, stream, A, lda, Wb, ldw, \
                           bias, row_mask, ld_mask, residual, ld_res, M, Nc, K, (OUT_*)C, ldc, vec_out);                \
    } while (0)
        const bool big = nt_b16_big_tile(M, Nc, K);
        if (c_is_f32) {
            if (big) STIN_GLDS(float, 2, 4, 4, 2);
            else STIN_GLDS(float, 2, 2, 2, 2);
        } else {
            if (big) STIN_GLDS(stin_bf16, 2, 4, 4, 2);
            else STIN_GLDS(stin_bf16, 2, 2, 2, 2);
        }
#undef STIN_GLDS
        return stin_launch_status();
    }
    if (c_is_f32) STIN_NTB_PICK(float);
    else STIN_NTB_PICK(stin_bf16);
#undef STIN_NTB_PICK
#undef STIN_NTB
    return stin_launch_status();
}

static int gemm_tn_bf16_impl(const stin_bf16_t* G_, int64_t ldg, const stin_bf16_t* X_, int64_t ldx, int64_t M, int Nc,
                            int K, int ones_column, const stin_bf16_t* row_weight_, int64_t ld_weight, float* dW,
                            int64_t lddw, float* db, void* workspace, size_t workspace_bytes, stin_stream_t stream_) {
    stin_clear_stale_error();
    hipStream_t stream = (hipStream_t)stream_;
    const int Kp = K + ((ones_column && db == nullptr) ? 1 : 0);
    STIN_REQUIRE(M >= 0 && Nc > 0 && K > 0 && ldg >= Nc && ldx >= K && lddw >= Kp, STIN_E_SIZE);
    STIN_REQUIRE(dW && workspace && (M == 0 || (G_ && X_)), STIN_E_NULL);
    STIN_REQUIRE(workspace_bytes >= stin_gemm_tn_workspace_bytes(M, Nc, K, ones_column), STIN_E_WORKSPACE);
    float* slab = reinterpret_cast<float*>((reinterpret_cast<uintptr_t>(workspace) + 255) & ~(uintptr_t)255);
    stin_tn_problem p;
    int rc = stin_tn_problem_init(&p, 1, G_, ldg, X_, ldx, M, Nc, K, ones_column, row_weight_, ld_weight, STIN_GEMM_BF16X3, slab, nullptr);
    if (rc != STIN_OK) return rc;
    rc = stin_tn_slabs(&p, 1, STIN_GEMM_BF16X3, stream_);
    if (rc != STIN_OK) return rc;
    const int64_t n4 = (int64_t)Nc * p.Kq / 4 + (p.has_bias ? (Nc + 3) / 4 : 0);
    hipLaunchKernelGGL(k_reduce_slabs, dim3((unsigned)((n4 + RS_COLS - 1) / RS_COLS)), dim3(BLOCK), 0, stream, slab, p.chunks, Nc, K,
                       p.Kq, p.has_bias, dW, lddw, db);
    return stin_launch_status();
}
extern "C" int stin_gemm_tn_bf16(const stin_bf16_t* G_, int64_t ldg, const stin_bf16_t* X_, int64_t ldx, int64_t M, int Nc,
                                 int K, int ones_column, const stin_bf16_t* row_weight_, int64_t ld_weight, float* dW,
                                 int64_t lddw, void* workspace, size_t workspace_bytes, stin_stream_t stream_) {
    return gemm_tn_bf16_impl(G_, ldg, X_, ldx, M, Nc, K, ones_column, row_weight_, ld_weight, dW, lddw, nullptr, workspace,
                             workspace_bytes, stream_);
}
extern "C" int stin_gemm_tn_wb_bf16(const stin_bf16_t* G_, int64_t ldg, const stin_bf16_t* X_, int64_t ldx, int64_t M, int Nc,
                                    int K, const stin_bf16_t* row_weight_, int64_t ld_weight, float* dW, int64_t lddw, float* db,
                                    void* workspace, size_t workspace_bytes, stin_stream_t stream_) {
    STIN_REQUIRE(db != nullptr, STIN_E_NULL);
    return gemm_tn_bf16_impl(G_, ldg, X_, ldx, M, Nc, K, 1, row_weight_, ld_weight, dW, lddw, db, workspace, workspace_bytes, stream_);
}
```

surface_texture_inpainting_net_amd/csrc/stin_wgrad.hip:

```cpp
#include <cstdlib>
#include <type_traits>
#include "stin_common.h"

namespace {

typedef float f32x16 __attribute__((ext_vector_type(16)));
typedef __bf16 bf16x8 __attribute__((ext_vector_type(8)));
typedef __bf16 bf16x4 __attribute__((ext_vector_type(4)));

constexpr int WS_T = 128;
constexpr int WS_R = 32;
constexpr int WS_THREADS = 512;
constexpr int WS_PLANE = WS_T * WS_R;
__device__ __forceinline__ int ws_lds(int col, int g) {
    return ((col ^ ((col >> 5) & 1)) << 5) + ((((g >> 1) ^ (col >> 2)) & 3) << 3) + ((g & 1) << 2);
}

typedef float f32x2 __attribute__((ext_vector_type(2)));
typedef __bf16 bf16x2 __attribute__((ext_vector_type(2)));
__device__ __forceinline__ unsigned pack_bf16(float a, float b) {
    const f32x2 v = {a, b};
    return __builtin_bit_cast(unsigned, __builtin_convertvector(v, bf16x2));
}

#ifdef STIN_WS_STAMPS
__device__ unsigned long long* stin_ws_stamp_buf = nullptr;
#define WS_STAMP(i)                                                                                                   \
    do {                                                                                                              \
        if (lane == 0 && stin_ws_stamp_buf != nullptr && (i) < 64)                                                    \
            stin_ws_stamp_buf[((size_t)blockIdx.x * 8 + wave) * 64 + (i)] = __builtin_amdgcn_s_memtime();             \
    } while (0)
#define WS_ABL(bit) (((prio >> 4) & (bit)) != 0)
#else
#define WS_STAMP(i)
#define WS_ABL(bit) false
#endif

struct WsSlab {
    float4 g[4], x[4];
    float pw[4];
    bool pv[4];
};

__global__ __launch_bounds__(WS_THREADS) void k_gemm_tn_ws(const stin_tn_batch batch, const int prio) {
    __shared__ __attribute__((aligned(16))) __bf16 Gt[2][2][WS_PLANE];
    __shared__ __attribute__((aligned(16))) __bf16 Xt[2][2][WS_PLANE];
    __shared__ float bsum[8][WS_T + 4];

    const int tid = threadIdx.x, lane = tid & 63;
    const int wave = __builtin_amdgcn_readfirstlane(tid >> 6);
    const bool producer = wave >= 4;
    const int pi = (batch.n > 1 && blockIdx.x >= batch.p[1].block0) ? 1 : 0;
    const float* __restrict__ G = batch.p[pi].G;
    const float* __restrict__ X = batch.p[pi].X;
    const float* __restrict__ row_w = batch.p[pi].row_w;
    const int64_t ldg = batch.p[pi].ldg, ldx = batch.p[pi].ldx, ld_w = batch.p[pi].ld_w, M = batch.p[pi].M;
    const int64_t chunks = batch.p[pi].chunks;
    const int Nc = batch.p[pi].Nc, K = batch.p[pi].K, Kq = batch.p[pi].Kq;
    const int tiles_j = batch.p[pi].tiles_j, tiles = batch.p[pi].tiles_i * tiles_j;
    const int rows_per_chunk = batch.p[pi].rows_per_chunk;

    const int64_t b = (int64_t)blockIdx.x - batch.p[pi].block0;
    const int64_t xcd = b % 8, q = b / 8;
    const int64_t chunk = chunks >= 8 ? (q / tiles) * 8 + xcd : b / tiles;
    const int tile = (int)(chunks >= 8 ? q % tiles : b % tiles);
    if (chunk >= chunks) return;
    const int tj = tile % tiles_j, ti = tile / tiles_j;
    const int i0 = ti * WS_T, j0 = tj * WS_T;
    const int64_t mb = chunk * rows_per_chunk;
    const int64_t me = (mb + rows_per_chunk < M) ? mb + rows_per_chunk : M;
    const bool want_bias = batch.p[pi].has_bias && (tj == 0);

    if (prio == 1 && !producer) __builtin_amdgcn_s_setprio(1);
    if (prio == 2 && producer) __builtin_amdgcn_s_setprio(1);

    float* out = batch.p[pi].slab + chunk * ((int64_t)Nc * Kq + ((Nc + 3) & ~3));

    if (producer) {
        const int ptid = tid & 255;
        const int c4 = ptid % 32, rg = (ptid / 32) ^ ((c4 >> 2) & 1);
        const float* gp = G + (i0 + c4 * 4 < Nc ? i0 + c4 * 4 : 0) + (mb + rg * 4) * ldg;
        const int xcol = j0 + c4 * 4 < K ? j0 + c4 * 4 : 0;
        const float* xp = X + xcol + (mb + rg * 4) * ldx;
        const stin_bn_tf xtf = batch.p[pi].xtf;
        stin_bn_coef4 xq;
        xq.s = xq.t = make_float4(0.f, 0.f, 0.f, 0.f);
        if (xtf.mean != nullptr) xq = stin_bn_coef4_load(xtf, xcol);
        const float* wp = (want_bias && row_w != nullptr) ? row_w + (mb + rg * 4) * ld_w : nullptr;
        int64_t m_next = mb + rg * 4;
        float4 bs = make_float4(0.f, 0.f, 0.f, 0.f);
        auto load_slab = [&](WsSlab& S, auto FULL) {
            if (WS_ABL(4)) return;
#pragma unroll
            for (int r = 0; r < 4; ++r) {
                if (decltype(FULL)::value) {
                    S.g[r] = ld4(gp + r * ldg);
                    S.x[r] = ld4(xp + r * ldx);
                    if (wp != nullptr) S.pw[r] = wp[r * ld_w];
                    S.pv[r] = true;
                } else {
                    const bool in = m_next + r < me;
                    float4 vg = make_float4(0.f, 0.f, 0.f, 0.f), vx = vg;
                    if (in) {
                        vg = ld4(gp + r * ldg);
                        vx = ld4(xp + r * ldx);
                    }
                    S.g[r] = vg;
                    S.x[r] = vx;
                    S.pw[r] = (in && wp != nullptr) ? wp[r * ld_w] : 0.f;
                    S.pv[r] = in;
                }
            }
            gp += WS_R * ldg;
            xp += WS_R * ldx;
            if (wp != nullptr) wp += WS_R * ld_w;
            m_next += WS_R;
        };
        auto split_col = [&](float a, float b, float c, float d, __bf16* dst) {
            const unsigned h01 = pack_bf16(a, b), h23 = pack_bf16(c, d);
            const float r0 = a - __uint_as_float(h01 << 16), r1 = b - __uint_as_float(h01 & 0xffff0000u);
            const float r2 = c - __uint_as_float(h23 << 16), r3 = d - __uint_as_float(h23 & 0xffff0000u);
            *reinterpret_cast<uint2*>(dst) = make_uint2(h01, h23);
            *reinterpret_cast<uint2*>(dst + WS_PLANE) = make_uint2(pack_bf16(r0, r1), pack_bf16(r2, r3));
        };
        const int o0 = ws_lds(c4 * 4, rg), o1 = ws_lds(c4 * 4 + 1, rg), o2 = ws_lds(c4 * 4 + 2, rg), o3 = ws_lds(c4 * 4 + 3, rg);
        auto split_store = [&](const float4 (&p)[4], __bf16* plane) {
            split_col(p[0].x, p[1].x, p[2].x, p[3].x, plane + o0);
            split_col(p[0].y, p[1].y, p[2].y, p[3].y, plane + o1);
            split_col(p[0].z, p[1].z, p[2].z, p[3].z, plane + o2);
            split_col(p[0].w, p[1].w, p[2].w, p[3].w, plane + o3);
        };
        auto store_slab = [&](const WsSlab& S, int buf) {
            if (WS_ABL(2)) return;
            if (want_bias) {
#pragma unroll
                for (int r = 0; r < 4; ++r) {
                    const float w = S.pv[r] ? (row_w != nullptr ? S.pw[r] : 1.f) : 0.f;
                    bs.x += w * S.g[r].x;
                    bs.y += w * S.g[r].y;
                    bs.z += w * S.g[r].z;
                    bs.w += w * S.g[r].w;
                }
            }
            split_store(S.g, &Gt[buf][0][0]);
            if (xtf.mean != nullptr) {
                const float4 tx[4] = {stin_bn_relu4(S.x[0], xq), stin_bn_relu4(S.x[1], xq), stin_bn_relu4(S.x[2], xq), stin_bn_relu4(S.x[3], xq)};
                split_store(tx, &Xt[buf][0][0]);
            } else {
                split_store(S.x, &Xt[buf][0][0]);
            }
        };
        WsSlab S0, S1;
        WS_STAMP(0);
        load_slab(S0, std::false_type());
        load_slab(S1, std::false_type());
        store_slab(S0, 0);
        WS_STAMP(1);
        load_slab(S0, std::false_type());
        __syncthreads();
        WS_STAMP(2);
        int64_t m0 = mb;
        int st = 3;
        (void)st;
        for (; m0 + 5 * WS_R <= me; m0 += 2 * WS_R) {
            store_slab(S1, 1);
            WS_STAMP(st);
            load_slab(S1, std::true_type());
            __syncthreads();
            WS_STAMP(st + 1);
            store_slab(S0, 0);
            load_slab(S0, std::true_type());
            __syncthreads();
            st += 2;
        }
        WS_STAMP(62);
        for (; m0 < me; m0 += 2 * WS_R) {
            store_slab(S1, 1);
            load_slab(S1, std::false_type());
            __syncthreads();
            store_slab(S0, 0);
            load_slab(S0, std::false_type());
            __syncthreads();
        }
        WS_STAMP(63);
        if (want_bias) st4(&bsum[rg][c4 * 4], bs);
    } else {
        const int wi = (wave >> 1) & 1, wj = wave & 1;
        const int kh = lane >> 5, li = lane & 31;
        f32x16 acc[2][2];
#pragma unroll
        for (int a = 0; a < 2; ++a)
#pragma unroll
            for (int c = 0; c < 2; ++c)
#pragma unroll
                for (int r = 0; r < 16; ++r) acc[a][c][r] = 0.f;
        int ga[2], gc[2];
#pragma unroll
        for (int t = 0; t < 2; ++t) {
            ga[t] = wi * 64 + t * 32 + li;
            gc[t] = wj * 64 + t * 32 + li;
        }
        auto frag = [&](const __bf16* plane, int col, int ks) {
            return *reinterpret_cast<const bf16x8*>(plane + ws_lds(col, (ks >> 2) + 2 * kh));
        };
        auto multiply = [&](int buf) {
            if (WS_ABL(1)) return;
#pragma unroll
            for (int ks = 0; ks < WS_R; ks += 16) {
                bf16x8 a[2][2], c[2][2];
#pragma unroll
                for (int p = 0; p < 2; ++p)
#pragma unroll
                    for (int t = 0; t < 2; ++t) {
                        a[p][t] = frag(&Gt[buf][p][0], ga[t], ks);
                        c[p][t] = frag(&Xt[buf][p][0], gc[t], ks);
                    }
#pragma unroll
                for (int t = 0; t < 2; ++t)
#pragma unroll
                    for (int u = 0; u < 2; ++u) {
                        acc[t][u] = __builtin_amdgcn_mfma_f32_32x32x16_bf16(a[0][t], c[1][u], acc[t][u], 0, 0, 0);
                        acc[t][u] = __builtin_amdgcn_mfma_f32_32x32x16_bf16(a[1][t], c[0][u], acc[t][u], 0, 0, 0);
                        acc[t][u] = __builtin_amdgcn_mfma_f32_32x32x16_bf16(a[0][t], c[0][u], acc[t][u], 0, 0, 0);
                    }
            }
        };
        WS_STAMP(0);
        __syncthreads();
        WS_STAMP(2);
        int st = 3;
        (void)st;
        for (int64_t m0 = mb; m0 < me; m0 += 2 * WS_R) {
            multiply(0);
            WS_STAMP(st);
            __syncthreads();
            WS_STAMP(st + 1);
            multiply(1);
            __syncthreads();
            st += 2;
        }
        WS_STAMP(62);
#pragma unroll
        for (int u = 0; u < 2; ++u) {
            const int col = j0 + wj * 64 + u * 32 + li;
            if (col >= K) continue;
#pragma unroll
            for (int t = 0; t < 2; ++t)
#pragma unroll
                for (int r = 0; r < 16; ++r) {
                    const int row = i0 + wi * 64 + t * 32 + (r & 3) + 8 * (r >> 2) + 4 * kh;
                    if (row < Nc) out[(int64_t)row * Kq + col] = acc[t][u][r];
                }
        }
        WS_STAMP(63);
    }
    if (want_bias) {
        __syncthreads();
        if (tid < WS_T) {
            float t = 0.f;
#pragma unroll
            for (int r = 0; r < 8; ++r) t += bsum[r][tid];
            if (i0 + tid < Nc) out[(int64_t)Nc * Kq + i0 + tid] = t;
        }
    }
}

constexpr int FN_COLS = 16, FN_KL = 16, FN_BLOCK = 256;
struct WgFinal {
    const float* slabA;
    const float* slabB;
    int64_t chunksA, chunksB;
    int KqA, KqB, Cin, Cp, H, Cout, has_shortcut, trans_inv;
    float *dW1, *db1, *dWs, *dbs, *dW2, *db2;
    const float* ti_colsum;
    int64_t ti_rows;
};
__device__ __forceinline__ void add4(float4& a, const float4 b) { a.x += b.x; a.y += b.y; a.z += b.z; a.w += b.w; }

__device__ __forceinline__ float4 fn_partial(const float* __restrict__ p, int64_t cs, int64_t chunks, int ty) {
        float4 s0 = make_float4(0.f, 0.f, 0.f, 0.f), s1 = s0, s2 = s0, s3 = s0;
        if (p != nullptr) {
            int64_t c = ty;
            for (; c + 15 * FN_KL < chunks; c += 16 * FN_KL) {
                float4 v[16];
#pragma unroll
                for (int u = 0; u < 16; ++u) v[u] = ld4(p + (c + u * FN_KL) * cs);
#pragma unroll
                for (int u = 0; u < 16; u += 4) {
                    add4(s0, v[u]);
                    add4(s1, v[u + 1]);
                    add4(s2, v[u + 2]);
                    add4(s3, v[u + 3]);
                }
            }
            for (; c + 3 * FN_KL < chunks; c += 4 * FN_KL) {
                add4(s0, ld4(p + c * cs));
                add4(s1, ld4(p + (c + FN_KL) * cs));
                add4(s2, ld4(p + (c + 2 * FN_KL) * cs));
                add4(s3, ld4(p + (c + 3 * FN_KL) * cs));
            }
            for (; c < chunks; c += FN_KL) add4(s0, ld4(p + c * cs));
        }
        add4(s0, s1);
        add4(s2, s3);
        add4(s0, s2);
        return s0;
}

__global__ __launch_bounds__(FN_BLOCK) void k_colsum_fold(const float* __restrict__ colsum, int64_t rows, int H, float* __restrict__ out) {
    __shared__ float4 sm[FN_KL][FN_COLS + 1];
    const int tx = threadIdx.x % FN_COLS, ty = threadIdx.x / FN_COLS;
    const int64_t g = (int64_t)blockIdx.x * FN_COLS + tx;
    const bool on = g < H / 4;
    sm[ty][tx] = fn_partial(on ? colsum + 4 * g : nullptr, H, rows, ty);
    __syncthreads();
    if (ty != 0 || !on) return;
    float4 a = make_float4(0.f, 0.f, 0.f, 0.f);
#pragma unroll
    for (int k = 0; k < FN_KL; ++k) add4(a, sm[k][tx]);
    st4(out + 4 * g, a);
}

__global__ __launch_bounds__(FN_BLOCK) void k_wgrad_finalize(const WgFinal f) {
    __shared__ float4 sm[2][FN_KL][FN_COLS + 1];
    const int tx = threadIdx.x % FN_COLS, ty = threadIdx.x / FN_COLS;
    const bool compact = f.trans_inv == STIN_TI_COMPACT;
    const int Yw = stin_yw(f.H, f.Cout, f.has_shortcut, f.trans_inv);
    const int s0 = Yw - (f.has_shortcut ? f.Cout : 0);
    const int64_t csA = (int64_t)f.Cout * f.KqA + ((f.Cout + 3) & ~3), csB = (int64_t)Yw * f.KqB + ((Yw + 3) & ~3);
    const int64_t nAw = (int64_t)f.Cout * f.KqA / 4, nAb = (f.Cout + 3) / 4;
    const int64_t nB1 = (int64_t)f.H * f.KqB / 4, nB2 = f.has_shortcut ? (int64_t)f.Cout * f.KqB / 4 : 0, nBb = (Yw + 3) / 4;
    const int64_t nT = (compact && f.db1 != nullptr) ? f.H / 4 : 0;
    int64_t g = (int64_t)blockIdx.x * FN_COLS + tx;
    const float *p0 = nullptr, *p1 = nullptr;
    int64_t cs = 0, chunks = 0;
    int section = -1;
    if (g < nAw) section = 0, p0 = f.slabA + 4 * g, cs = csA, chunks = f.chunksA;
    else if ((g -= nAw) < nAb) section = 1, p0 = f.slabA + (int64_t)f.Cout * f.KqA + 4 * g, cs = csA, chunks = f.chunksA;
    else if ((g -= nAb) < nB1) section = 2, p0 = f.slabB + 4 * g, p1 = compact ? nullptr : p0 + (int64_t)f.H * f.KqB, cs = csB, chunks = f.chunksB;
    else if ((g -= nB1) < nB2) section = 3, p0 = f.slabB + (int64_t)s0 * f.KqB + 4 * g, cs = csB, chunks = f.chunksB;
    else if ((g -= nB2) < nBb) section = 4, p0 = f.slabB + (int64_t)Yw * f.KqB + 4 * g, cs = csB, chunks = f.chunksB;
    else if ((g -= nBb) < nT) section = 5, p0 = f.ti_colsum + 4 * g, cs = f.H, chunks = f.ti_rows;
    auto partial = [&](const float* p) { return fn_partial(p, cs, chunks, ty); };
    sm[0][ty][tx] = partial(p0);
    sm[1][ty][tx] = partial(p1);
    __syncthreads();
    if (ty != 0 || section < 0) return;
    float4 a = make_float4(0.f, 0.f, 0.f, 0.f), b = a;
#pragma unroll
    for (int k = 0; k < FN_KL; ++k) add4(a, sm[0][k][tx]);
    if (section == 2) {
#pragma unroll
        for (int k = 0; k < FN_KL; ++k) add4(b, sm[1][k][tx]);
    }
    const float va[4] = {a.x, a.y, a.z, a.w}, vb[4] = {b.x, b.y, b.z, b.w};
    if (section == 0) {
        const int64_t row = (4 * g) / f.KqA;
        const int col = (int)((4 * g) % f.KqA);
#pragma unroll
        for (int e = 0; e < 4; ++e)
            if (col + e < f.H) f.dW2[row * f.H + col + e] = va[e];
    } else if (section == 1) {
#pragma unroll
        for (int e = 0; e < 4; ++e)
            if (4 * g + e < f.Cout && f.db2 != nullptr) f.db2[4 * g + e] = va[e];
    } else if (section == 2) {
        const int64_t row = (4 * g) / f.KqB;
        const int col = (int)((4 * g) % f.KqB);
#pragma unroll
        for (int e = 0; e < 4; ++e) {
            if (col + e >= f.Cin) continue;
            if (compact) f.dW1[row * f.Cin + col + e] = va[e];
            else if (f.trans_inv) f.dW1[row * f.Cin + col + e] = vb[e] - va[e];
            else {
                f.dW1[row * 2 * f.Cin + col + e] = va[e];
                f.dW1[row * 2 * f.Cin + f.Cin + col + e] = vb[e] - va[e];
            }
        }
    } else if (section == 3) {
        const int64_t row = (4 * g) / f.KqB;
        const int col = (int)((4 * g) % f.KqB);
#pragma unroll
        for (int e = 0; e < 4; ++e)
            if (col + e < f.Cin) f.dWs[row * f.Cin + col + e] = va[e];
    } else if (section == 4) {
#pragma unroll
        for (int e = 0; e < 4; ++e) {
            const int64_t i = 4 * g + e;
            if (i < f.H && !compact) {
                if (f.db1 != nullptr) f.db1[i] = va[e];
            } else if (i >= s0 && i < Yw && f.dbs != nullptr) f.dbs[i - s0] = va[e];
        }
    } else {
#pragma unroll
        for (int e = 0; e < 4; ++e) f.db1[4 * g + e] = va[e];
    }
}

inline size_t up256(size_t v) { return (v + 255) & ~(size_t)255; }

}

bool stin_tn_ws_enabled() {
    const char* e = getenv("STIN_TN_WS");
    return e == nullptr || atoi(e) != 0;
}

int stin_tn_ws_launch(stin_tn_batch batch, stin_stream_t stream) {
    const int prio = 1;
    unsigned blocks = 0;
    for (int i = 0; i < batch.n; ++i) {
        stin_tn_problem& p = batch.p[i];
        blocks = (blocks + 7u) & ~7u;
        p.block0 = blocks;
        blocks += (unsigned)((p.chunks >= 8 ? ((p.chunks + 7) / 8) * 8 : p.chunks) * (int64_t)p.tiles_i * p.tiles_j);
    }
    if (blocks == 0) return STIN_OK;
    hipLaunchKernelGGL(k_gemm_tn_ws, dim3(blocks), dim3(WS_THREADS), 0, (hipStream_t)stream, batch, prio);
    return stin_launch_status();
}

extern "C" size_t stin_edgeconv_wgrad_workspace_bytes(int64_t N, int Cp, int H, int Cout, int has_shortcut) {
    if (N < 0 || Cp <= 0 || H <= 0 || Cout <= 0) return 0;
    const int Yw = 2 * H + (has_shortcut ? Cout : 0);
    return up256(stin_gemm_tn_workspace_bytes(N, Cout, H, 1)) + up256(stin_gemm_tn_workspace_bytes(N, Yw, Cp, 1)) + 256;
}

extern "C" int stin_edgeconv_wgrad(int storage, const void* dagg, int64_t ld_dagg, const void* hE, int64_t ldh, const void* dY,
                                   int64_t ldy, const void* x, int64_t ldx, int64_t N, int Cin, int Cp, int H, int Cout,
                                   int has_shortcut, int trans_inv, int precision, float* dW1, float* db1, float* dW2, float* db2,
                                   float* dWs, float* dbs, void* workspace, size_t workspace_bytes, stin_stream_t stream) {
    STIN_REQUIRE(trans_inv != STIN_TI_COMPACT, STIN_E_UNSUPPORTED);
    return stin_edgeconv_wgrad_ti(storage, dagg, ld_dagg, hE, ldh, dY, ldy, x, ldx, N, Cin, Cp, H, Cout, has_shortcut, trans_inv, precision,
                                  dW1, db1, dW2, db2, dWs, dbs, nullptr, 0, workspace, workspace_bytes, stream);
}

extern "C" int stin_edgeconv_wgrad_ti(int storage, const void* dagg, int64_t ld_dagg, const void* hE, int64_t ldh, const void* dY,
                                      int64_t ldy, const void* x, int64_t ldx, int64_t N, int Cin, int Cp, int H, int Cout,
                                      int has_shortcut, int trans_inv, int precision, float* dW1, float* db1, float* dW2, float* db2,
                                      float* dWs, float* dbs, const float* ti_colsum, int64_t ti_rows, void* workspace,
                                      size_t workspace_bytes, stin_stream_t stream) {
    stin_clear_stale_error();
    STIN_REQUIRE(storage == 0 || storage == 1, STIN_E_UNSUPPORTED);
    STIN_REQUIRE(N >= 0 && Cin > 0 && Cp >= Cin && H > 0 && Cout > 0, STIN_E_SIZE);
    STIN_REQUIRE(trans_inv >= 0 && trans_inv <= STIN_TI_COMPACT, STIN_E_UNSUPPORTED);
    const bool compact = trans_inv == STIN_TI_COMPACT;
    STIN_REQUIRE(!compact || (storage == 0 && H % 4 == 0 && (db1 == nullptr || N == 0 || (ti_colsum != nullptr && ti_rows > 0))), STIN_E_UNSUPPORTED);
    const int Yw = stin_yw(H, Cout, has_shortcut, trans_inv);
    STIN_REQUIRE(ld_dagg >= Cout && ldh >= H + 1 && ldy >= Yw && ldx >= Cp, STIN_E_SIZE);
    STIN_REQUIRE(dW1 && dW2 && workspace && (!has_shortcut || dWs) && (N == 0 || (dagg && hE && dY && x)), STIN_E_NULL);
    STIN_REQUIRE(workspace_bytes >= stin_edgeconv_wgrad_workspace_bytes(N, Cp, H, Cout, has_shortcut), STIN_E_WORKSPACE);
    char* p = reinterpret_cast<char*>((reinterpret_cast<uintptr_t>(workspace) + 255) & ~(uintptr_t)255);
    float* slabA = reinterpret_cast<float*>(p);
    float* slabB = reinterpret_cast<float*>(p + up256(stin_gemm_tn_workspace_bytes(N, Cout, H, 1)));
    const size_t es = storage ? 2 : 4;
    const void* row_w = static_cast<const char*>(hE) + (size_t)H * es;
    stin_tn_problem pa, pb;
    int wsa = 0, wsb = 0;
    int rc = stin_tn_problem_init(&pa, storage, dagg, ld_dagg, hE, ldh, N, Cout, H, 1, row_w, ldh, precision, slabA, &wsa);
    if (rc != STIN_OK) return rc;
    rc = stin_tn_problem_init(&pb, storage, dY, ldy, x, ldx, N, Yw, Cp, 1, nullptr, 0, precision, slabB, &wsb);
    if (rc != STIN_OK) return rc;
    if (wsa && wsb) {
        stin_tn_batch batch;
        batch.p[0] = pa;
        batch.p[1] = pb;
        batch.n = 2;
        rc = stin_tn_ws_launch(batch, stream);
    } else {
        rc = stin_tn_slabs(&pa, storage, precision, stream);
        if (rc == STIN_OK) rc = stin_tn_slabs(&pb, storage, precision, stream);
    }
    if (rc != STIN_OK) return rc;
    WgFinal f;
    f.slabA = slabA;
    f.slabB = slabB;
    f.chunksA = pa.chunks;
    f.chunksB = pb.chunks;
    f.KqA = pa.Kq;
    f.KqB = pb.Kq;
    f.Cin = Cin;
    f.Cp = Cp;
    f.H = H;
    f.Cout = Cout;
    f.has_shortcut = has_shortcut;
    f.trans_inv = trans_inv;
    f.dW1 = dW1;
    f.db1 = db1;
    f.dWs = dWs;
    f.dbs = dbs;
    f.dW2 = dW2;
    f.db2 = db2;
    f.ti_colsum = ti_colsum;
    f.ti_rows = ti_rows;
    const int64_t groups = (int64_t)Cout * pa.Kq / 4 + (Cout + 3) / 4 + (int64_t)H * pb.Kq / 4 +
                           (has_shortcut ? (int64_t)Cout * pb.Kq / 4 : 0) + (Yw + 3) / 4 + ((compact && db1 != nullptr) ? H / 4 : 0);
    hipLaunchKernelGGL(k_wgrad_finalize, dim3((unsigned)((groups + FN_COLS - 1) / FN_COLS)), dim3(FN_BLOCK), 0, (hipStream_t)stream, f);
    return stin_launch_status();
}

extern "C" int stin_edge_bwd_ti_colsum_fold_f32(const float* colsum, int64_t rows, int H, float* db1, stin_stream_t stream) {
    stin_clear_stale_error();
    STIN_REQUIRE(rows >= 0 && H > 0 && H % 4 == 0, STIN_E_SIZE);
    STIN_REQUIRE(db1 && (rows == 0 || colsum) && stin_aligned16(db1) && stin_aligned16(colsum), STIN_E_NULL);
    const unsigned grid = (unsigned)((H / 4 + FN_COLS - 1) / FN_COLS);
    hipLaunchKernelGGL(k_colsum_fold, dim3(grid), dim3(FN_BLOCK), 0, (hipStream_t)stream, colsum, rows, H, db1);
    return stin_launch_status();
}
```

surface_texture_inpainting_net_amd/functional.py:

```python
import collections
import os

import torch

from . import _lib
from .plan import _ptr, _stream

EPS = 1e-5
USE_EDGE_MASK = os.environ.get('STIN_EDGE_MASK', '1') != '0'
_C = _lib.CONSTANTS
RED_SUM, RED_CSQ, RED_DOT_ELU, RED_COEF_XC, RED_MOMENTS, RED_DOT_BN, RED_DOT_BN_RELU = (_C[n] for n in (
    'STIN_RED_SUM', 'STIN_RED_CSQ', 'STIN_RED_DOT_ELU', 'STIN_RED_COEF_XC', 'STIN_RED_MOMENTS', 'STIN_RED_DOT_BN',
    'STIN_RED_DOT_BN_RELU'))
POST_NONE, POST_SCALE, POST_RSTD, POST_NORM_COEF = (_C[n] for n in (
    'STIN_POST_NONE', 'STIN_POST_SCALE', 'STIN_POST_RSTD', 'STIN_POST_NORM_COEF'))
SEG_NONTEMPORAL = _C['STIN_SEG_NONTEMPORAL']


def _mat(t):
    if not (t.dim() == 2 and t.dtype in (torch.float32, torch.bfloat16) and t.is_cuda):
        raise TypeError('the STINet HIP path takes 2-D float32 (or bfloat16-storage) CUDA tensors (no CPU / eager '
                        'fallback exists); got shape %s dtype %s device %s' % (tuple(t.shape), t.dtype, t.device))
    if t.stride(1) != 1 or (t.shape[0] > 1 and t.stride(0) < t.shape[1]):
        t = t.contiguous()
# ... 518 lines not shown
def linear(x, weight, bias=None, out_fp32=False, precision=None, wT=None, wT_guard=None):
    return LinearFn.apply(x, weight, bias, out_fp32, precision, wT, wT_guard)


def forward_precision(unbounded_input):
    if unbounded_input and PREC_FWD == GEMM_F16X3:
        return GEMM_BF16X6
    return PREC_FWD


USE_WGRAD_STREAM = os.environ.get('STIN_WGRAD_STREAM', '1') == '1'
WGRAD_DEFER_JOIN = True
WGRAD_MAX_WORK = float(os.environ.get('STIN_WGRAD_MAX_WORK', 1.6e10))
WGRAD_MIN_WORK = float(os.environ.get('STIN_WGRAD_MIN_WORK', 2.0e9))
_WGRAD_SIDE = {}


class _WgradSide:
    RING = 64

    def __init__(self, dev):
        self.stream = torch.cuda.Stream(device=dev)
        self.ring = [[torch.cuda.Event() for _ in range(3)] for _ in range(self.RING)]
        for tri in self.ring:
            for e in tri:
                e.record(self.stream)
        self.at = 0
        self.last_done = self.ring[0][2]
        self.hold = []

    def next_events(self, track=True):
        self.at = (self.at + 1) % self.RING
        tri = self.ring[self.at]
        if track:
            self.last_done = tri[2]
        return tri


def _wgrad_side(dev):
    side = _WGRAD_SIDE.get(dev.index)
    if side is None:
        side = _WGRAD_SIDE[dev.index] = _WgradSide(dev)
    return side


USE_DIRECT_GRADS = True


def _direct_grad_views(params, dry_run=False):
    if not USE_DIRECT_GRADS:
        return None
    bucket, out = None, []
    for p in params:
        if p is None:
            out.append(None)
            continue
        slot = getattr(p, '_stin_slot', None)
        if slot is None or not slot[0].accepting or (bucket is not None and slot[0] is not bucket) or slot[0].written[slot[1]]:
            return None
        bucket = slot[0]
        out.append(bucket.views[slot[1]])
    if bucket is None:
        return None
    if dry_run:
        return out
    for p in params:
        if p is not None:
            bucket.written[p._stin_slot[1]] = True
    return out


def _plain_autograd_may_defer():
    import torch.distributed as dist
    return not (dist.is_available() and dist.is_initialized() and dist.get_world_size() > 1)


def _join_deferrable(params, direct):
    return WGRAD_DEFER_JOIN and (bool(direct) or (_plain_autograd_may_defer() and all(
        p is None or (p.is_leaf and p.grad is None and not p._backward_hooks and
                      not getattr(p, '_post_accumulate_grad_hooks', None)) for p in params)))


def wgrad_side_settle(dev):
    side = _WGRAD_SIDE.get(dev.index if dev.index is not None else torch.cuda.current_device())
    if side is not None and side.hold:
        torch.cuda.current_stream(dev).wait_event(side.last_done)
        side.hold.clear()


def _wgrad_deferred_join(dev, params, grads):
    side = _wgrad_side(dev)
    adopted = [(p, t.data_ptr()) for p, t in zip(params, grads) if p is not None and t is not None]

    def join():
        torch.cuda.current_stream(dev).wait_event(side.last_done)
        side.hold.clear()
        for p, ptr in adopted:
            if p.grad is not None and p.grad.data_ptr() != ptr:
                raise RuntimeError('weight-gradient stream: autograd copied a gradient before the end-of-backward join; '
                                   'set STIN_WGRAD_STREAM=0 for this autograd configuration')

    torch.autograd.Variable._execution_engine.queue_callback(join)


def block_split_modes(prec_fwd, b16, Cout):
    fsp = (prec_fwd | GEMM_W_FRAG) if (not b16 and prec_fwd in (GEMM_BF16X3, GEMM_F16X3) and WEIGHT_PRESPLIT) else 0
    bsp = (PREC_BWD | GEMM_W_FRAG) if (not b16 and PREC_BWD in (GEMM_BF16X3, GEMM_F16X3) and WEIGHT_PRESPLIT and Cout % 4 == 0) else 0
    return fsp, bsp


TI_COMPACT = os.environ.get('STIN_TI_COMPACT', '1') != '0'
TI_MODE_COMPACT = _C['STIN_TI_COMPACT']


def trans_inv_mode(trans_inv, b16, H):
    if not trans_inv:
        return 0
    return TI_MODE_COMPACT if (TI_COMPACT and not b16 and USE_EDGE_MASK and edge_mask_supported(H)) else 1


def block_yw(H, Cout, has_shortcut, ti_mode):
    return (H if ti_mode == TI_MODE_COMPACT else 2 * H) + (Cout if has_shortcut else 0)


def _pad_rows(x, pad):
    N, Cin = x.shape
    Cp = (Cin + pad - 1) // pad * pad
    if Cp == Cin:
        return x
    xp = torch.empty(N, Cp, dtype=x.dtype, device=x.device)
    _call('stin_pad_rows' + _sfx(x), _ptr(x), x.stride(0), N, Cin, Cp, _ptr(xp), _stream(x))
    return xp


def _fresh_grads(params, dev):
    return [None if p is None else torch.empty(p.shape, dtype=torch.float32, device=dev) for p in params]


BLOCK_PACKED = _C['STIN_BLOCK_PACKED']
_PACK_JOB = _lib.STRUCTS['stin_pack_job_t']
USE_PACK_MANY = True


class PackSet:

    def __init__(self, specs, dev, b16=False, transposes=()):
        import ctypes
        lib = _lib.load()
        self.key = self.key_of(specs) + (bool(b16),) + tuple((_ptr(W), tuple(W.shape)) for W in transposes)
        self.b16 = bool(b16)
        self.buffers = []
        blob, self.max_elems = b'', 0
        pad = 8 if b16 else 4
        for (W1, b1, W2, b2, Ws, bs, trans_inv, prec_fwd, B) in specs:
            H, Cout = W1.shape[0], W2.shape[0]
            Cin = W1.shape[1] if trans_inv else W1.shape[1] // 2
            Cp = (Cin + pad - 1) // pad * pad
            has_sc = Ws is not None
            ti = trans_inv_mode(trans_inv, b16, H)
            Yw = block_yw(H, Cout, has_sc, ti)
            fsp, bsp = block_split_modes(prec_fwd, b16, Cout)
            jf, jb = ((GEMM_W_BF16, GEMM_W_BF16) if (Cp % 8 == 0 and Cout % 8 == 0) else (0, 0)) if b16 else (fsp, bsp)
            ws = torch.empty(lib.stin_edgeconv_block_fwd_workspace_bytes(Cin, Cp, H, Cout, int(has_sc), B), dtype=torch.uint8, device=dev)
            wts = torch.empty(Yw * Cp + H * Cout, dtype=torch.float32, device=dev)
            off = [ctypes.c_size_t(0) for _ in range(3)]
            _lib.check(lib.stin_edgeconv_block_fwd_pack_offsets(Cp, H, Cout, int(has_sc), *[ctypes.byref(o) for o in off]),
                       'stin_edgeconv_block_fwd_pack_offsets')
            base = (ws.data_ptr() + 255) & ~255
            wcat, w2s, bcat = (base + o.value for o in off)
            W1c, W2c = W1.contiguous(), W2.contiguous()
            assert W1c.data_ptr() == W1.data_ptr() and W2c.data_ptr() == W2.data_ptr(), 'pack_many needs contiguous weights'
            blob += _PACK_JOB.pack(W1=_ptr(W1), b1=_ptr(b1), Ws=_ptr(Ws), bs=_ptr(bs), W2=_ptr(W2), wcat=wcat, bcat=bcat,
                                   wcatT=_ptr(wts), w2T=_ptr(wts) + 4 * Yw * Cp, w2s=w2s if jf else 0, Cin=Cin, Cp=Cp, H=H,
                                   Cout=Cout, has_shortcut=int(has_sc), trans_inv=ti, fwd_split=jf, bwd_split=jb)
            self.max_elems = max(self.max_elems, Yw * Cp + H * Cout)
            self.buffers.append((ws, wts, fsp, bsp, wts[:Yw * Cp].view(Cp, Yw), wts[Yw * Cp:].view(H, Cout), bool(b16)))
        self.transposed = []
        for W in transposes:
            Nc, K = W.shape
            assert W.is_contiguous() and W.dtype == torch.float32
            wT = torch.empty(K, Nc, dtype=torch.float32, device=dev)
            blob += _PACK_JOB.pack(W2=_ptr(W), w2T=_ptr(wT), H=K, Cout=Nc)
            self.max_elems = max(self.max_elems, K * Nc)
            self.transposed.append(wT)
        self.jobs = torch.frombuffer(bytearray(blob), dtype=torch.uint8).to(dev)
        self.n = len(specs) + len(transposes)

    @staticmethod
    def key_of(specs):
        return tuple((_ptr(W1), _ptr(b1), _ptr(W2), _ptr(Ws), _ptr(bs), tuple(W1.shape), tuple(W2.shape), bool(t), int(pf), int(B),
                      PREC_BWD, WEIGHT_PRESPLIT, GEMM_W_FRAG, TI_COMPACT, USE_EDGE_MASK) for (W1, b1, W2, b2, Ws, bs, t, pf, B) in specs)

    def matches(self, specs, b16=False, transposes=()):
        return self.key == self.key_of(specs) + (bool(b16),) + tuple((_ptr(W), tuple(W.shape)) for W in transposes)

    def run(self):
        self.runs = getattr(self, 'runs', 0) + 1
        _call('stin_edgeconv_pack_many_f32', _ptr(self.jobs), self.n, self.max_elems, _stream(self.jobs))


class EdgeConvBlockFn(torch.autograd.Function):

    @staticmethod
    def forward(ctx, x, W1, b1, W2, b2, Ws, bs, edges, groups, trans_inv, eps=EPS, prec_fwd=None):
        prec_fwd = PREC_FWD if prec_fwd is None else int(prec_fwd)
        x, _ = _mat(x)
        N, Cin = x.shape
        H, Cout = W1.shape[0], W2.shape[0]
        has_shortcut = Ws is not None
        dev = x.device
        b16 = x.dtype == torch.bfloat16
        ti = trans_inv_mode(trans_inv, b16, H)
        Yw = block_yw(H, Cout, has_shortcut, ti)
        oS = Yw - (Cout if has_shortcut else 0)
        pad = 8 if b16 else 4
        xp = _pad_rows(x, pad)
        Cp = xp.shape[1]
        fsp, bsp = block_split_modes(prec_fwd, b16, Cout)
        pack = torch.empty(Yw * Cp * 2 + 2 * H * Cout + Yw, dtype=torch.float32, device=dev)
        wcat = pack[:Yw * Cp].view(Yw, Cp)
        wcatT = pack[Yw * Cp:2 * Yw * Cp].view(Cp, Yw)
        w2T = pack[2 * Yw * Cp:2 * Yw * Cp + H * Cout].view(H, Cout)
        w2s = pack[2 * Yw * Cp + H * Cout:2 * Yw * Cp + 2 * H * Cout].view(Cout, H)
        bcat = pack[2 * Yw * Cp + 2 * H * Cout:]
        W1c, W2c = W1.contiguous(), W2.contiguous()
        _call('stin_edgeconv_pack_f32', _ptr(W1c), _ptr(b1), _ptr(Ws), _ptr(bs), _ptr(W2c), Cin, Cp, H, Cout,
              int(has_shortcut), ti, _ptr(wcat), _ptr(bcat), _ptr(wcatT), _ptr(w2T), _ptr(w2s) if fsp else None,
              fsp, bsp, _stream(x))
        pf = (prec_fwd | GEMM_W_PRESPLIT | GEMM_W_FRAG) if fsp else prec_fwd
        Y = gemm_nt(xp, wcat, bcat, precision=pf)
        hE = torch.empty(N, H + pad, dtype=x.dtype, device=dev)
        use_mask = USE_EDGE_MASK and edge_mask_supported(H) and Y.stride(0) % 4 == 0
        if b16 and not use_mask:
            raise NotImplementedError('bf16 storage needs the saved ReLU mask: hidden width %d not in '
                                      '{128, 256, 512, 1024, 2048} (or STIN_EDGE_MASK=0)' % H)
        mask = torch.empty(max(edges.n_edges, 1) * (H // 32), dtype=torch.int32, device=dev) if use_mask else None
        if ti == TI_MODE_COMPACT:
            if not use_mask:
                raise RuntimeError('compact trans-inv layout needs the saved ReLU mask (16-byte aligned rows)')
            edge_relu_mean_fwd_ti(b1, Y[:, :H], edges.by_dst, hE, indicator=True, mask=mask)
        else:
            edge_relu_mean_fwd(Y[:, :H], Y[:, H:2 * H], edges.by_dst, hE, indicator=True, mask=mask)
        fused = None
        if fsp and groups.B == 1 and groups.gid is None and not groups.quirk and N > 1:
            fused = gemm_nt_colstats(hE[:, :H], w2s, b2, hE[:, H], pf, Cout)
        if fused is not None:
            agg = fused[0]
            mean, rstd = moments_final(fused[1], groups.inv_cnt, eps)
        else:
            agg = gemm_nt(hE[:, :H], w2s if fsp else W2c, b2, row_mask=hE[:, H], precision=pf)
            mean, rstd = instance_stats(agg, groups, eps)
        res = Y[:, oS:] if has_shortcut else x
        out = norm_act_res_fwd(agg, mean, rstd, groups, res=res, act=True)
        ctx.save_for_backward(xp, Y, hE, agg, mean, rstd, wcatT, w2T)
        ctx.mask = mask
        ctx.cin = Cin
        ctx.edges, ctx.groups, ctx.H, ctx.has_shortcut, ctx.trans_inv = edges, groups, H, has_shortcut, ti
        ctx.params = (W1, b1, W2, b2, Ws, bs)
        ctx.prec_bwd_nt = (PREC_BWD | GEMM_W_PRESPLIT | GEMM_W_FRAG) if bsp else PREC_BWD
        return out

    @staticmethod
    def backward(ctx, g):
        x, Y, hE, agg, mean, rstd, wcatT, w2T = ctx.saved_tensors
        edges, groups, H = ctx.edges, ctx.groups, ctx.H
        Cin, Cp, Cout = ctx.cin, x.shape[1], agg.shape[1]
        g, ldg = _mat(g)
        dagg = instance_norm_act_bwd(agg, g, mean, rstd, groups, act=True)
        dw2b = gemm_tn(dagg, hE[:, :H], ones_column=True, row_weight=hE[:, H], precision=PREC_BWD)
        dhE = gemm_nt(dagg, w2T, precision=ctx.prec_bwd_nt)
        dY = torch.empty_like(Y)
        compact = ctx.trans_inv == TI_MODE_COMPACT
        oS = Y.shape[1] - (Cout if ctx.has_shortcut else 0)
        db1_ti = None
        if compact:
            db1_ti = edge_relu_mean_bwd_mask_ti(dhE, ctx.mask, edges, dY[:, :H])
            ctx.mask = None
        elif ctx.mask is not None:
            edge_relu_mean_bwd_mask(dhE, ctx.mask, edges, dY[:, :H], dY[:, H:2 * H])
            ctx.mask = None
        else:
            A, B = Y[:, :H], Y[:, H:2 * H]
            edge_relu_mean_bwd_dst(A, B, dhE, edges.by_dst, dY[:, :H])
            edge_relu_mean_bwd_src(A, B, dhE, edges.inv_deg, edges.by_src, dY[:, H:2 * H])
        if ctx.has_shortcut:
            dY[:, oS:].copy_(g)
        dwb = gemm_tn(dY, x, ones_column=True, precision=PREC_BWD)
        dx = None
        if ctx.needs_input_grad[0]:
            dx = gemm_nt(dY, wcatT, precision=ctx.prec_bwd_nt, residual=None if ctx.has_shortcut else g)
            if Cp != Cin:
                dx = dx[:, :Cin]
        dW1, db1, dW2, db2, dWs, dbs = _fresh_grads(ctx.params, x.device)
        _call('stin_edgeconv_unpack_grads_f32', _ptr(dwb), _ptr(dw2b), Cin, Cp, H, Cout, int(ctx.has_shortcut),
              int(ctx.trans_inv), _ptr(dW1), _ptr(db1), _ptr(dWs), _ptr(dbs), _ptr(dW2), _ptr(db2), _stream(x))
        if compact and db1 is not None:
            db1 = db1_ti
        return dx, dW1, db1, dW2, db2, dWs, dbs, None, None, None, None, None


USE_NET_CALL = os.environ.get('STIN_NET_CALL', '1') != '0'
USE_CHAIN = True
USE_UNPOOL_COMMUTE = os.environ.get('STIN_UNPOOL_COMMUTE', '1') != '0'
_NET_OP = _lib.STRUCTS['stin_net_op_t']
OP_BLOCK, OP_POOL_MAX, OP_UNPOOL = _C['STIN_OP_BLOCK'], _C['STIN_OP_POOL_MAX'], _C['STIN_OP_UNPOOL']


def _align256(n):
    return (n + 255) & ~255


def usable_prepack(blk, b16):
    pp = blk._prepacked
    if pp is None:
        return None
    fsp, bsp = block_split_modes(forward_precision(blk.unbounded_input), b16, blk.dim_out)
    return pp if (len(pp) > 6 and pp[6] == b16 and pp[2] == fsp and pp[3] == bsp) else None


def net_eligible(steps, x):
    if not (USE_BLOCK_CALL and USE_EDGE_MASK and not KernelTimer.per_kernel_path() and x.is_cuda and x.dim() == 2):
        return False
    if x.dtype not in (torch.float32, torch.bfloat16) or x.shape[0] <= 1:
        return False
    b16 = x.dtype == torch.bfloat16
    packed = []
    for st in steps:
        if st[0] != 'block':
            continue
        b = st[1]
        H = b.first_filter.nn[0].weight.shape[0]
        if not edge_mask_supported(H) or st[2].n <= 1:
            return False
        packed.append(usable_prepack(b, b16) is not None)
    return bool(packed) and any(packed) == all(packed)


class NetFn(torch.autograd.Function):

    calls = 0
    sizes = collections.Counter()
    commuted = 0
    gathers_skipped = 0

    @staticmethod
    def _in_arena(rel, base, xp):
        ptrs = {k: 0 if o is None else base + o for k, o in rel.items()}
        ptrs.setdefault('x', _ptr(xp))
        return ptrs

    @staticmethod
    def _commutes(steps, si, b16, width, Ws, ti):
        return (USE_UNPOOL_COMMUTE and si > 0 and steps[si - 1][0] == 'unpool' and not b16 and Ws is not None
                and ti != TI_MODE_COMPACT and width % 4 == 0 and Ws.shape[0] % 4 == 0)

    @staticmethod
    def forward(ctx, x, meta, *params):
        steps, need_grad = meta
        NetFn.calls += 1
        NetFn.sizes[len(steps)] += 1
        lib = _lib.load()
        x, _ = _mat(x)
        dev, dt = x.device, x.dtype
        b16 = dt == torch.bfloat16
        sfx = '_bf16' if b16 else '_f32'
        es = x.element_size()
        pad = 8 if b16 else 4
        N0, Cin0 = x.shape
        xp = _pad_rows(x, pad)
        plan, off, pi = [], 0, 0
        n_rows, width = N0, Cin0

        toff, tmax, omax = 0, 0, 0

        def take(nbytes, kind='keep'):
            nonlocal off, toff, tmax, omax
            if not need_grad and kind == 'tmp':
                o = toff
                toff = _align256(toff + nbytes)
                tmax = max(tmax, toff)
                return ('tmp', o)
            if not need_grad and kind == 'out':
                omax = max(omax, _align256(nbytes))
                return ('out', 0)
            o = off
            off = _align256(off + nbytes)
            return o
        for si, stp in enumerate(steps):
            toff = 0
            last = si == len(steps) - 1
            if stp[0] == 'block':
                blk, edges, groups = stp[1], stp[2], stp[3]
                W1, b1, W2, b2, Ws, bs = params[pi:pi + 6]
                pi += 6
                H, Cout = W1.shape[0], W2.shape[0]
                Cin = width
                Cp = (Cin + pad - 1) // pad * pad
                sc = Ws is not None
                ti = trans_inv_mode(blk.first_filter.trans_inv, b16, H)
                Yw = block_yw(H, Cout, sc, ti)
                B = groups.B
                prec = forward_precision(blk.unbounded_input)
                fsp, bsp = block_split_modes(prec, b16, Cout)
                pp = usable_prepack(blk, b16)
                ws_bytes = lib.stin_edgeconv_block_fwd_workspace_bytes(Cin, Cp, H, Cout, int(sc), B)
                d = dict(kind=OP_BLOCK, N=n_rows, Cin=Cin, Cp=Cp, H=H, Cout=Cout, sc=sc, Yw=Yw, B=B, prec=prec, fsp=fsp, bsp=bsp, pp=pp,
                         ws_bytes=ws_bytes, edges=edges, groups=groups, ti=ti, eps=float(blk.first_norm.eps),
                         params=(W1, b1, W2, b2, Ws, bs))
                d['src'] = plan[-1] if NetFn._commutes(steps, si, b16, width, Ws, ti) else None
                d['oY'] = take((d['src']['n_in'] if d['src'] else n_rows) * Yw * es, 'tmp')
                d['oH'] = take(n_rows * (H + pad) * es, 'tmp')
                d['oM'] = take(max(edges.n_edges, 1) * (H // 32) * 4) if need_grad else None
                d['oA'] = take(n_rows * Cout * es, 'tmp')
                d['oS'] = take(2 * B * Cout * 4, 'tmp')
                if pp is None:
                    d['oW'] = take((Yw * Cp + H * Cout) * 4, 'tmp')
                    d['oWS'] = take(ws_bytes, 'tmp')
                elif pp[0].numel() < ws_bytes:
                    raise RuntimeError('NetFn: prepacked workspace too small for this batch (PackSet built for another batch size)')
                d['oO'] = None if last else take(n_rows * Cout * es, 'out')
                width = Cout
            else:
                pool = stp[1]
                if stp[0] == 'pool':
                    d = dict(kind=OP_POOL_MAX, pool=pool, n_in=pool.n_fine, n_out=pool.n_coarse, C=width)
                    d['oArg'] = take(pool.n_coarse * width * 4, 'tmp')
                else:
                    d = dict(kind=OP_UNPOOL, pool=pool, n_in=pool.n_coarse, n_out=pool.n_fine, C=width)
                n_rows = d['n_out']
                nxt = steps[si + 1] if not last else None
                d['skip'] = (stp[0] == 'unpool' and not need_grad and nxt is not None and nxt[0] == 'block' and
                             NetFn._commutes(steps, si + 1, b16, width, params[pi + 4], trans_inv_mode(
                                 nxt[1].first_filter.trans_inv, b16, params[pi].shape[0])))
                d['oO'] = None if (last or d['skip']) else take(n_rows * width * es, 'out')
            plan.append(d)
        if not need_grad:
            o_base, t_base, flip = off, off + 2 * omax, 0
            for d in plan:
                for k, v in d.items():
                    if isinstance(v, tuple) and len(v) == 2 and v[0] == 'tmp':
                        d[k] = t_base + v[1]
                    elif isinstance(v, tuple) and len(v) == 2 and v[0] == 'out':
                        d[k] = o_base + flip * omax
                        flip ^= 1
            off = t_base + tmax
        arena = torch.empty(off, dtype=torch.uint8, device=dev)
        out = torch.empty(n_rows, width, dtype=dt, device=dev)
        base, p_out = _ptr(arena), _ptr(out)
        assert base % 256 == 0
        stc = _NET_OP
        blob = []
        xin, ldx = None, xp.stride(0)
        first = True
        for d in plan:
            rel = {} if first else {'x': xin}
            first = False
            if d['kind'] == OP_BLOCK:
                W1, b1, W2, b2, Ws, bs = d['params']
                pp = d['pp']
                if pp is not None:
                    packed = dict(wcatT=_ptr(pp[4]), w2T=_ptr(pp[5]), fwd_ws=_ptr(pp[0]), fwd_split=d['fsp'] | BLOCK_PACKED)
                else:
                    packed = dict(fwd_split=d['fsp'])
                    rel.update(wcatT=d['oW'], w2T=d['oW'] + d['Yw'] * d['Cp'] * 4, fwd_ws=d['oWS'])
                g, cd = d['groups'], d['edges'].by_dst
                H, Cout, B = d['H'], d['Cout'], d['B']
                d['op'] = dict(kind=OP_BLOCK, Cin=d['Cin'], Cp=d['Cp'], H=H, Cout=Cout, has_shortcut=int(d['sc']), trans_inv=int(d['ti']),
                               prec_fwd=int(d['prec']), bwd_split=d['bsp'], B=B, slice_quirk=int(g.quirk), eps=d['eps'],
                               y_from_src=int(d['src'] is not None),
                               n_out=d['N'], n_in=d['N'], ldx=ldx, ldo=Cout, ldy=d['Yw'], ldh=H + pad, fwd_ws_bytes=d['ws_bytes'],
                               W1=_ptr(W1.contiguous()), b1=_ptr(b1), W2=_ptr(W2.contiguous()), b2=_ptr(b2), Ws=_ptr(Ws),
                               bs=_ptr(bs), rowptr_dst=_ptr(cd.rowptr), col_dst=_ptr(cd.col),
                               ptr_sum=_ptr(g.ptr_sum), gid=_ptr(g.gid), inv_cnt=_ptr(g.inv_cnt), **packed)
                rel.update(Y=d['oY'], hE=d['oH'], agg=d['oA'], mean=d['oS'], rstd=d['oS'] + B * Cout * 4)
                if need_grad:
                    rel['mask'] = d['oM']
                NetFn.commuted += int(d['src'] is not None)
                ev0, ev1 = KernelTimer.edge_events('stin_edge_relu_mean_fwd' + sfx, (d['N'], d['edges'].n_edges, H))
                events = dict(ev_edge0=ev0, ev_edge1=ev1)
                ldx = Cout
            else:
                pool, C = d['pool'], d['C']
                ch = pool.children
                d['op'] = dict(kind=d['kind'], Cin=C, Cp=C, Cout=C, n_out=d['n_out'], n_in=d['n_in'], ldx=ldx, ldo=C,
                               rowptr_dst=_ptr(ch.rowptr), col_dst=_ptr(ch.col), trace=_ptr(pool.trace))
                if d['kind'] == OP_POOL_MAX:
                    rel['arg'] = d['oArg']
                events = {}
                ldx = C
            d['rel'] = rel
            skip = d.get('skip', False)
            NetFn.gathers_skipped += int(skip)
            blob.append(stc.pack(**d['op'], **NetFn._in_arena(rel, base, xp), **events,
                                 out=0 if skip else p_out if d['oO'] is None else base + d['oO']))
            xin = d['oO']
        import ctypes
        buf = ctypes.create_string_buffer(b''.join(blob), len(plan) * stc.size)
        _call('stin_net_fwd', int(b16), buf, len(plan), _stream(x))
        if not need_grad:
            return out
        ctx.save_for_backward(xp, arena)
        ctx.plan = plan
        ctx.cin0 = Cin0
        ctx.params = params
        return out

    @staticmethod
    def backward(ctx, g):
        xp, arena = ctx.saved_tensors
        base = _ptr(arena)
        plan, params = ctx.plan, ctx.params
        lib = _lib.load()
        dev, dt = xp.device, xp.dtype
        b16 = dt == torch.bfloat16
        sfx = '_bf16' if b16 else '_f32'
        es = xp.element_size()
        g, ldg = _mat(g)
        _same(xp, g)
        need_dx = ctx.needs_input_grad[0]
        blocks = [d for d in plan if d['kind'] == OP_BLOCK]
        direct = []
        if all(_direct_grad_views(d['params'], dry_run=True) is not None for d in blocks):
            direct = [_direct_grad_views(d['params']) for d in blocks]
        grads = None
        if len(direct) != len(blocks):
            direct = []
            grads = [t for d in blocks for t in _fresh_grads(d['params'], dev)]
        dx_bytes, ws_off, off = 0, [], 0
        for i, d in enumerate(plan):
            if d['kind'] == OP_BLOCK:
                if i > 0 or need_dx:
                    dx_bytes = max(dx_bytes, d['N'] * d['Cp'] * es)
                d['bwd_ws_bytes'] = lib.stin_edgeconv_block_bwd_workspace_bytes(d['N'], d['Cp'], d['H'], d['Cout'], int(d['sc']), d['B'], int(b16))
                ws_off.append(off)
                off = _align256(off + d['bwd_ws_bytes'])
            else:
                dx_bytes = max(dx_bytes, d['n_in'] * d['C'] * es)
        dx_bytes = _align256(dx_bytes)
        scratch = torch.empty(2 * dx_bytes + off, dtype=torch.uint8, device=dev)
        p_scr = _ptr(scratch)
        p_ws = p_scr + 2 * dx_bytes
        dx0 = None
        d0 = plan[0]
        if need_dx:
            dx0 = torch.empty(d0['N'] if d0['kind'] == OP_BLOCK else d0['n_in'], d0['Cp'] if d0['kind'] == OP_BLOCK else d0['C'],
                              dtype=dt, device=dev)
        all_params = [p for d in blocks for p in d['params']]
        side_ok = USE_WGRAD_STREAM and _join_deferrable(all_params, direct)
        use = [side_ok and WGRAD_MIN_WORK <= float(d['N']) * d['Yw'] * d['Cp'] <= WGRAD_MAX_WORK for d in blocks]
        side_stream, any_side = 0, any(use)
        evs = [(0, 0)] * len(blocks)
        bucket = None
        if direct:
            for p in all_params:
                if p is not None:
                    bucket = p._stin_slot[0]
                    break
        seg_events = bucket is not None and bucket.wants_block_events()
        done_ev = [None] * len(blocks)
        if any_side or seg_events:
            side = _wgrad_side(dev)
        if any_side:
            side.hold.append((scratch, xp, arena, g))
            side_stream = side.stream.cuda_stream
        if any_side or seg_events:
            for bi in reversed(range(len(blocks))):
                if use[bi]:
                    tri = side.next_events()
                    evs[bi] = (tri[1].cuda_event, tri[2].cuda_event)
                    done_ev[bi] = tri[2]
                elif seg_events:
                    tri = side.next_events(track=False)
                    evs[bi] = (0, tri[2].cuda_event)
                    done_ev[bi] = tri[2]
            if grads is not None:
                for t in grads:
                    if t is not None:
                        t.record_stream(side.stream)
        stc = _NET_OP
        blob, bi = [], 0
        for i, d in enumerate(plan):
            p_dx = (_ptr(dx0) if i == 0 else p_scr + (i & 1) * dx_bytes)
            if i == 0 and not need_dx:
                p_dx = 0
            if d['kind'] == OP_BLOCK:
                e, gr = d['edges'], d['groups']
                cs = e.by_src
                gs = direct[bi] if direct else grads[6 * bi:6 * bi + 6]
                ev_dy, ev_done = evs[bi]
                ev0, ev1 = KernelTimer.edge_events('stin_edge_relu_mean_bwd_mask' + ('_ti' if d['ti'] == TI_MODE_COMPACT else '') + sfx,
                                                   (d['N'], e.n_edges, d['H']))
                blob.append(stc.pack(**d['op'], **NetFn._in_arena(d['rel'], base, xp), use_side=int(use[bi]), lddx=d['Cp'],
                                     bwd_ws_bytes=d['bwd_ws_bytes'], dx=p_dx,
                                     rowptr_src=_ptr(cs.rowptr), col_src=_ptr(cs.col), xslot=_ptr(e.xslot), w_src=_ptr(e.w_src),
                                     ptr_true=_ptr(gr.ptr_true), sid=_ptr(gr.sid if gr.quirk else None),
                                     dW1=_ptr(gs[0]), db1=_ptr(gs[1]), dW2=_ptr(gs[2]), db2=_ptr(gs[3]), dWs=_ptr(gs[4]), dbs=_ptr(gs[5]),
                                     bwd_ws=p_ws + ws_off[bi], ev_dy=ev_dy, ev_done=ev_done, ev_edge0=ev0, ev_edge1=ev1))
                bi += 1
            else:
                blob.append(stc.pack(**d['op'], **NetFn._in_arena(d['rel'], base, xp), lddx=d['C'], dx=p_dx))
        import ctypes
        buf = ctypes.create_string_buffer(b''.join(blob), len(plan) * stc.size)
        _call('stin_net_bwd', int(b16), buf, len(plan), _ptr(g), ldg, int(PREC_BWD), _stream(xp), side_stream)
        if any_side:
            _wgrad_deferred_join(dev, all_params if not direct else (), () if direct else grads)
        if dx0 is not None and dx0.shape[1] != ctx.cin0:
            dx0 = dx0[:, :ctx.cin0]
        if direct:
            sd = _WGRAD_SIDE.get(dev.index if dev.index is not None else torch.cuda.current_device())
            bucket.blocks_done([([p._stin_slot[1] for p in d['params'] if p is not None], done_ev[bi]) for bi, d in enumerate(blocks)],
                               sd.last_done if (sd is not None and sd.hold) else None)
            return (dx0, None) + (None,) * len(params)
        return (dx0, None) + tuple(grads)


def run_net(x, steps):
    params = []
    for st in steps:
        if st[0] == 'block':
            b = st[1]
            lin1, lin2 = b.first_filter.nn[0], b.first_filter.nn[2]
            sc = b.shortcut if b.dim_in != b.dim_out else None
            params += [lin1.weight, lin1.bias, lin2.weight, lin2.bias, None if sc is None else sc.weight, None if sc is None else sc.bias]
    need_grad = torch.is_grad_enabled() and (x.requires_grad or any(p is not None and p.requires_grad for p in params))
    return NetFn.apply(x, (steps, need_grad), *params)


class EdgeReluMeanFn(torch.autograd.Function):

    @staticmethod
    def forward(ctx, A, B, edges):
        A, _ = _mat(A)
        B, _ = _mat(B)
        out = torch.empty(A.shape[0], A.shape[1], dtype=torch.float32, device=A.device)
        edge_relu_mean_fwd(A, B, edges.by_dst, out)
        ctx.save_for_backward(A, B)
        ctx.edges = edges
        return out

    @staticmethod
    def backward(ctx, g):
        A, B = ctx.saved_tensors
        g, _ = _mat(g)
        dA = torch.empty_like(A)
        dB = torch.empty_like(B)
        edge_relu_mean_bwd_dst(A, B, g, ctx.edges.by_dst, dA)
        edge_relu_mean_bwd_src(A, B, g, ctx.edges.inv_deg, ctx.edges.by_src, dB)
        return dA, dB, None


def _cols_axpy_rowmask(dst, src, rowptr, c0, c1, alpha):
    _same(dst, src)
    _call('stin_cols_axpy_rowmask' + _sfx(dst), _ptr(dst), dst.stride(0), _ptr(src), src.stride(0), _ptr(rowptr), dst.shape[0], int(c0),
          int(c1), float(alpha), _stream(dst))


class NeighborMeanFn(torch.autograd.Function):

    @staticmethod
    def forward(ctx, x, edges, mean, sub_cols=None):
        ctx.edges, ctx.mean, ctx.sub_cols = edges, mean, sub_cols
        agg = segment_sum(x, edges.by_dst.rowptr, edges.by_dst.col, edges.n, mean=mean)
        if sub_cols is not None:
            xm = x if (x.dim() == 2 and x.stride(1) == 1) else x.contiguous()
            _cols_axpy_rowmask(agg, xm, edges.by_dst.rowptr, sub_cols[0], sub_cols[1], -1.0)
        return agg

    @staticmethod
    def backward(ctx, g):
        e = ctx.edges
        gs = g * e.inv_deg.view(-1, 1) if ctx.mean else g
        dx = segment_sum(gs, e.by_src.rowptr, e.by_src.col, e.n, mean=False)
        if ctx.sub_cols is not None:
            gm = g if (g.dim() == 2 and g.stride(1) == 1) else g.contiguous()
            _cols_axpy_rowmask(dx, gm, e.by_dst.rowptr, ctx.sub_cols[0], ctx.sub_cols[1], -1.0)
        return dx, None, None, None


class ScatterAddFn(torch.autograd.Function):

    @staticmethod
    def forward(ctx, src, csr):
        ctx.csr = csr
        return segment_sum(src, csr.rowptr, csr.perm, csr.n_rows, mean=False)

    @staticmethod
    def backward(ctx, g):
        raise NotImplementedError('ScatterAddFn is forward-only (benchmark / metrics op)')


class PoolMaxFn(torch.autograd.Function):
    @staticmethod
    def forward(ctx, x, pool):
        x, ldx = _mat(x)
        C = x.shape[1]
        out = torch.empty(pool.n_coarse, C, dtype=x.dtype, device=x.device)
        arg = torch.empty(pool.n_coarse, C, dtype=torch.int32, device=x.device)
        _call('stin_pool_max_fwd' + _sfx(x), _ptr(x), ldx, _ptr(pool.children.rowptr), _ptr(pool.children.col), pool.n_coarse, C,
              _ptr(out), C, _ptr(arg), _stream(x))
        ctx.save_for_backward(arg)
        ctx.pool = pool
        return out

    @staticmethod
    def backward(ctx, g):
        (arg,) = ctx.saved_tensors
        pool = ctx.pool
        g, ldg = _mat(g)
        C = g.shape[1]
        gx = torch.empty(pool.n_fine, C, dtype=g.dtype, device=g.device)
        _call('stin_pool_max_bwd' + _sfx(g), _ptr(g), ldg, _ptr(arg), _ptr(pool.trace), pool.n_fine, C, _ptr(gx), C, _stream(g))
        return gx, None


class PoolMeanFn(torch.autograd.Function):
    @staticmethod
    def forward(ctx, x, pool):
        ctx.pool = pool
        return segment_sum(x, pool.children.rowptr, pool.children.col, pool.n_coarse, mean=True)

    @staticmethod
    def backward(ctx, g):
        return gather_rows(g, ctx.pool.trace, ctx.pool.inv_count), None


class UnpoolFn(torch.autograd.Function):
    @staticmethod
    def forward(ctx, x, pool):
        ctx.pool = pool
        return gather_rows(x, pool.trace)

    @staticmethod
    def backward(ctx, g):
        p = ctx.pool
        return segment_sum(g, p.children.rowptr, p.children.col, p.n_coarse, mean=False), None


class PermuteRowsFn(torch.autograd.Function):

    @staticmethod
    def forward(ctx, x, idx, inv):
        ctx.inv = inv
        return gather_rows(x, idx)

    @staticmethod
    def backward(ctx, g):
        return gather_rows(g.contiguous(), ctx.inv), None, None


class InstanceNormActResFn(torch.autograd.Function):

    @staticmethod
    def forward(ctx, x, res, groups, act, eps=EPS):
        x, _ = _mat(x)
        mean, rstd = instance_stats(x, groups, eps)
        y = norm_act_res_fwd(x, mean, rstd, groups, res=res, act=act)
        ctx.save_for_backward(x, mean, rstd)
        ctx.groups, ctx.act, ctx.has_res = groups, act, res is not None
        return y

    @staticmethod
    def backward(ctx, g):
        x, mean, rstd = ctx.saved_tensors
        dx = instance_norm_act_bwd(x, g, mean, rstd, ctx.groups, act=ctx.act)
        return dx, (g if ctx.has_res else None), None, None, None


class MaskedL1LossFn(torch.autograd.Function):

    @staticmethod
    def forward(ctx, out, color, mask, use_weight):
        lib = _lib.load()
        out, _ = _mat(out)
        color, _ = _mat(color)
        out, color = out.contiguous(), color.contiguous()
        N, C = out.shape
        m = mask.reshape(-1).contiguous()
        if m.dtype != torch.int64:
            m = m.long()
        loss = torch.empty((), dtype=torch.float32, device=out.device)
        grad = torch.empty_like(out)
        ws_bytes = lib.stin_masked_l1_workspace_bytes(N, C)
        ws = torch.empty(ws_bytes, dtype=torch.uint8, device=out.device)
        _call('stin_masked_l1_loss_f32', _ptr(out), _ptr(color), _ptr(m), N, C, int(use_weight), _ptr(loss), _ptr(grad),
              _ptr(ws), ws_bytes, _stream(out))
        ctx.save_for_backward(grad)
        return loss

    _UNIT = {}

    @staticmethod
    def backward(ctx, g):
        (grad,) = ctx.saved_tensors
        u = MaskedL1LossFn._UNIT.get(g.device.index)
        if u is not None and g.data_ptr() == u.data_ptr():
            return grad, None, None, None
        return grad * g, None, None, None


def unit_seed(device):
    idx = device.index if device.index is not None else torch.cuda.current_device()
    u = MaskedL1LossFn._UNIT.get(idx)
    if u is None:
        u = MaskedL1LossFn._UNIT[idx] = torch.ones((), dtype=torch.float32, device=device)
    return u


def masked_l1_loss(out, color, mask, use_weight=True):
    return MaskedL1LossFn.apply(out, color, mask, use_weight)


def adam_step(p, g, m, v, vmax, lr, beta1, beta2, eps, weight_decay, step, amsgrad=True):
    _call('stin_adam_f32', _ptr(p), _ptr(g), _ptr(m), _ptr(v), _ptr(vmax), p.numel(), float(lr), float(beta1), float(beta2),
          float(eps), float(weight_decay), int(step), int(amsgrad), _stream(p))


class SliceSumFn(torch.autograd.Function):

    @staticmethod
    def forward(ctx, x, groups):
        ctx.groups = groups
        return colreduce(RED_SUM, x, groups, groups.ptr_sum)

    @staticmethod
    def backward(ctx, g):
        gr = ctx.groups
        if gr.sid is None:
            return g.expand(gr.n_rows, -1).contiguous(), None
        return g.index_select(0, gr.sid.long()), None
```

Baseline: 28.45 million vertices/s.

## Skip unpool materialization in training via row-mapped wgrad and in-place shortcut grad

The change lets training skip materializing the unpooled activation before a commuting block. The block's weight-gradient GEMM now gathers input rows through the unpool trace map inside the producer loop of the TN kernel, so the fine-resolution copy of x no longer has to be written and kept. Separately, the next op's dx is redirected to write straight into the previous block's dY shortcut slice, which removes a 2D memcpy or ride copy. The costs are indirect, less coalesced X loads in the wgrad kernel, an extra template instantiation, and more complex aliasing logic.

```diff
diff --git a/include/stin_hip.h b/include/stin_hip.h
--- a/include/stin_hip.h
+++ b/include/stin_hip.h
@@ -370,7 +370,7 @@
 #define STIN_OP_UNPOOL 2
 typedef struct stin_net_op {
     int32_t kind, Cin, Cp, H, Cout, has_shortcut, trans_inv, prec_fwd, fwd_split, bwd_split, B, slice_quirk, use_side, y_from_src,
-        reserved1, reserved2;
+        x_from_src, g_in_dy;
     float eps;
     int32_t reserved3;
     int64_t n_out, n_in, ldx, ldo, lddx, ldy, ldh;
@@ -399,6 +399,7 @@
 int stin_net_fwd(int storage, const stin_net_op_t* ops, int n_ops, stin_stream_t stream);
 int stin_net_bwd(int storage, const stin_net_op_t* ops, int n_ops, const void* g, int64_t ldg, int prec_bwd, stin_stream_t stream,
                  stin_stream_t wgrad_stream);
+int stin_net_bwd_g_in_dy(int storage, const stin_net_op_t* ops, int n_ops, int i);
 
 size_t stin_edgeconv_wgrad_workspace_bytes(int64_t N, int Cp, int H, int Cout, int has_shortcut);
 int stin_edgeconv_wgrad(int storage, const void* dagg, int64_t ld_dagg, const void* hE, int64_t ldh, const void* dY,
@@ -410,6 +411,12 @@
                            int has_shortcut, int trans_inv, int precision, float* dW1, float* db1, float* dW2, float* db2,
                            float* dWs, float* dbs, const float* ti_colsum, int64_t ti_rows, void* workspace,
                            size_t workspace_bytes, stin_stream_t stream);
+int stin_edgeconv_wgrad_map_supported(int64_t N, int Cp, int H, int Cout, int has_shortcut, int precision);
+int stin_edgeconv_wgrad_map(int storage, const void* dagg, int64_t ld_dagg, const void* hE, int64_t ldh, const void* dY,
+                            int64_t ldy, const void* x, int64_t ldx, int64_t N, int Cin, int Cp, int H, int Cout,
+                            int has_shortcut, int trans_inv, int precision, float* dW1, float* db1, float* dW2, float* db2,
+                            float* dWs, float* dbs, const int32_t* x_row_map, int64_t x_rows, void* workspace,
+                            size_t workspace_bytes, stin_stream_t stream);
 
 int stin_dilated_walk_f32(const int32_t* rowptr, const int32_t* col, const int32_t* row_of, const float* pos,
                           const float* nrm, int64_t N, int64_t E, const int32_t* dilations, int n_dil, int32_t* out,
diff --git a/surface_texture_inpainting_net_amd/csrc/stin_block.hip b/surface_texture_inpainting_net_amd/csrc/stin_block.hip
--- a/surface_texture_inpainting_net_amd/csrc/stin_block.hip
+++ b/surface_texture_inpainting_net_amd/csrc/stin_block.hip
@@ -224,11 +224,11 @@
 };
 
 static int block_bwd(int storage, const stin_net_op_t& J, const void* g, int64_t ldg, int prec_bwd, stin_stream_t stream,
-                     stin_stream_t wgrad_stream, BwdLink* link) {
+                     stin_stream_t wgrad_stream, BwdLink* link, const stin_net_op_t* Un = nullptr) {
     const int64_t N = J.n_out;
     const int Cp = J.Cp, H = J.H, Cout = J.Cout, has_shortcut = J.has_shortcut;
     STIN_REQUIRE(N >= 0 && J.Cin > 0 && Cp >= J.Cin && H > 0 && Cout > 0 && J.B > 0, STIN_E_SIZE);
-    STIN_REQUIRE(g && J.x && J.hE && J.mask && J.agg && J.mean && J.rstd && J.wcatT && J.w2T && J.rowptr_dst && J.rowptr_src && J.col_src &&
+    STIN_REQUIRE(g && (J.x || Un) && J.hE && J.mask && J.agg && J.mean && J.rstd && J.wcatT && J.w2T && J.rowptr_dst && J.rowptr_src && J.col_src &&
                      J.xslot && J.w_src && J.inv_cnt && J.dW1 && J.dW2 && J.bwd_ws && (!has_shortcut || J.dWs),
                  STIN_E_NULL);
     STIN_REQUIRE(J.bwd_ws_bytes >= stin_edgeconv_block_bwd_workspace_bytes(N, Cp, H, Cout, has_shortcut, J.B, storage), STIN_E_WORKSPACE);
@@ -289,9 +289,10 @@
         STIN_TRY(stin_gemm_nt_f32(static_cast<const float*>(dagg), Cout, J.w2T, Cout, nullptr, nullptr, 0, nullptr, 0, N, H, Cout,
                                   static_cast<float*>(dhE), H, pb, stream));
         float* dYs = dYf + (Yw - Cout);
-        const bool ride = has_shortcut && N > 0 && Cout % 4 == 0 && ldg % 4 == 0 && Yw % 4 == 0 && stin_aligned16(gf) &&
+        const bool placed = has_shortcut && gf == dYs && ldg == Yw;
+        const bool ride = has_shortcut && !placed && N > 0 && Cout % 4 == 0 && ldg % 4 == 0 && Yw % 4 == 0 && stin_aligned16(gf) &&
                           stin_aligned16(dYs) && Cout <= H;
-        const bool bind = bind_on && (!has_shortcut || ride);
+        const bool bind = bind_on && (!has_shortcut || ride || placed);
         if (bind) stin_tl_stop_event = (hipEvent_t)J.ev_dy;
         if (compact)
             STIN_EDGE_BRACKET(stin_edge_relu_mean_bwd_mask_ti_f32(static_cast<const float*>(dhE), H, J.mask, J.rowptr_dst, J.w_src,
@@ -301,7 +302,7 @@
             STIN_EDGE_BRACKET(stin_edge_relu_mean_bwd_mask_f32(static_cast<const float*>(dhE), H, J.mask, J.rowptr_dst, J.w_src, J.rowptr_src,
                                                               J.col_src, J.xslot, N, H, dYf, Yw, dYf + H, Yw, ride ? gf : nullptr, ldg,
                                                               ride ? dYs : nullptr, Yw, ride ? Cout : 0, stream));
-        if (has_shortcut && N > 0 && !ride) {
+        if (has_shortcut && N > 0 && !ride && !placed) {
             hipError_t e = hipMemcpy2DAsync(dYs, (size_t)Yw * 4, gf, (size_t)ldg * 4, (size_t)Cout * 4, (size_t)N,
                                             hipMemcpyDeviceToDevice, hs);
             if (e != hipSuccess) return (int)e;
@@ -309,8 +310,13 @@
         bound = bind && stin_tl_stop_event == nullptr;
         stin_tl_stop_event = nullptr;
         STIN_TRY(fork());
-        STIN_TRY(stin_edgeconv_wgrad_ti(0, dagg, Cout, hf, J.ldh, dYf, Yw, J.x, J.ldx, N, J.Cin, Cp, H, Cout, has_shortcut, J.trans_inv,
-                                        prec_bwd, J.dW1, J.db1, J.dW2, J.db2, J.dWs, J.dbs, ti_colsum, ti_rows, tn_ws, tn_bytes, ws_));
+        if (Un)
+            STIN_TRY(stin_edgeconv_wgrad_map(0, dagg, Cout, hf, J.ldh, dYf, Yw, Un->x, Un->ldx, N, J.Cin, Cp, H, Cout, has_shortcut,
+                                             J.trans_inv, prec_bwd, J.dW1, J.db1, J.dW2, J.db2, J.dWs, J.dbs, Un->trace, Un->n_in, tn_ws,
+                                             tn_bytes, ws_));
+        else
+            STIN_TRY(stin_edgeconv_wgrad_ti(0, dagg, Cout, hf, J.ldh, dYf, Yw, J.x, J.ldx, N, J.Cin, Cp, H, Cout, has_shortcut, J.trans_inv,
+                                            prec_bwd, J.dW1, J.db1, J.dW2, J.db2, J.dWs, J.dbs, ti_colsum, ti_rows, tn_ws, tn_bytes, ws_));
         if (J.dx != nullptr) {
             const bool link_ok = link != nullptr && link->next_agg != nullptr && link->next_ld % 4 == 0 && stin_aligned16(link->next_agg) &&
                                  stin_aligned16(link->next_mean) && stin_aligned16(link->next_rstd) && link->next_partial != nullptr;
@@ -326,6 +332,7 @@
             }
         }
     } else {
+        STIN_REQUIRE(Un == nullptr, STIN_E_UNSUPPORTED);
         const stin_bf16_t* gh = static_cast<const stin_bf16_t*>(g);
         const stin_bf16_t* hh = static_cast<const stin_bf16_t*>(J.hE);
         stin_bf16_t* dYh = static_cast<stin_bf16_t*>(dY);
@@ -370,7 +377,7 @@
         const stin_net_op_t& J = ops[i];
         if (J.kind == STIN_OP_BLOCK) {
             const stin_net_op_t* un = (i > 0 && commutes(storage, ops[i - 1], J)) ? &ops[i - 1] : nullptr;
-            STIN_REQUIRE(un != nullptr || J.y_from_src == 0, STIN_E_UNSUPPORTED);
+            STIN_REQUIRE(un != nullptr || (J.y_from_src == 0 && J.x_from_src == 0), STIN_E_UNSUPPORTED);
             STIN_TRY(block_fwd(storage, J, stream, un));
         } else if (J.kind == STIN_OP_POOL_MAX) {
             if (storage)
@@ -394,6 +401,34 @@
     return STIN_OK;
 }
 
+static bool g_in_dy(int storage, const stin_net_op_t* ops, int n_ops, int i, void** dx, int64_t* lddx) {
+    if (storage != 0 || ops == nullptr || i < 1 || i >= n_ops) return false;
+    const stin_net_op_t &J = ops[i], &Pn = ops[i - 1];
+    if (Pn.kind != STIN_OP_BLOCK || Pn.g_in_dy == 0 || Pn.has_shortcut == 0 || Pn.bwd_ws == nullptr || J.dx == nullptr) return false;
+    if (Pn.n_out <= 0 || Pn.Cp <= 0 || Pn.H <= 0 || Pn.Cout <= 0 || Pn.B <= 0) return false;
+    int64_t rows, width;
+    if (J.kind == STIN_OP_BLOCK) {
+        if (J.Cin != J.Cp) return false;
+        rows = J.n_out, width = J.Cp;
+    } else if (J.kind == STIN_OP_POOL_MAX || J.kind == STIN_OP_UNPOOL) {
+        rows = J.n_in, width = J.Cout;
+    } else {
+        return false;
+    }
+    const int Yw = stin_yw(Pn.H, Pn.Cout, Pn.has_shortcut, Pn.trans_inv);
+    if (rows != Pn.n_out || width != Pn.Cout || Pn.Cout % 4 != 0 || Yw % 4 != 0) return false;
+    if (Pn.bwd_ws_bytes < stin_edgeconv_block_bwd_workspace_bytes(Pn.n_out, Pn.Cp, Pn.H, Pn.Cout, Pn.has_shortcut, Pn.B, storage)) return false;
+    char* t = align256(Pn.bwd_ws) + bwd_layout(Pn.n_out, Pn.H, Pn.Cout, Pn.has_shortcut, Pn.B, storage).dY + (size_t)(Yw - Pn.Cout) * 4;
+    if (!stin_aligned16(t)) return false;
+    if (dx) *dx = t;
+    if (lddx) *lddx = Yw;
+    return true;
+}
+
+extern "C" int stin_net_bwd_g_in_dy(int storage, const stin_net_op_t* ops, int n_ops, int i) {
+    return g_in_dy(storage, ops, n_ops, i, nullptr, nullptr) ? 1 : 0;
+}
+
 extern "C" int stin_net_bwd(int storage, const stin_net_op_t* ops, int n_ops, const void* g, int64_t ldg, int prec_bwd,
                             stin_stream_t stream, stin_stream_t wgrad_stream) {
     STIN_REQUIRE(n_ops >= 0 && (n_ops == 0 || ops != nullptr), STIN_E_NULL);
@@ -403,9 +438,20 @@
     const double* pre_partial = nullptr;
     int64_t pre_groups = 0;
     for (int i = n_ops - 1; i >= 0; --i) {
-        const stin_net_op_t& J = ops[i];
+        stin_net_op_t Jr;
+        void* dx_in_dy = nullptr;
+        int64_t ld_in_dy = 0;
+        const bool redirect = g_in_dy(storage, ops, n_ops, i, &dx_in_dy, &ld_in_dy);
+        if (redirect) {
+            Jr = ops[i];
+            Jr.dx = dx_in_dy;
+            Jr.lddx = ld_in_dy;
+        }
+        const stin_net_op_t& J = redirect ? Jr : ops[i];
         STIN_REQUIRE(J.dx != nullptr || i == 0, STIN_E_NULL);
         if (J.kind == STIN_OP_BLOCK) {
+            const stin_net_op_t* un = (J.x_from_src != 0 && i > 0 && commutes(storage, ops[i - 1], J)) ? &ops[i - 1] : nullptr;
+            STIN_REQUIRE(un != nullptr || J.x_from_src == 0, STIN_E_UNSUPPORTED);
             BwdLink link;
             link.pre_partial = pre_partial;
             link.pre_groups = pre_groups;
@@ -424,7 +470,7 @@
                     link.next_partial_bytes = Ln.red_bytes > 256 ? Ln.red_bytes - 256 : 0;
                 }
             }
-            STIN_TRY(block_bwd(storage, J, gi, ldgi, prec_bwd, stream, wgrad_stream, &link));
+            STIN_TRY(block_bwd(storage, J, gi, ldgi, prec_bwd, stream, wgrad_stream, &link, un));
             if (link.produced_groups > 0) {
                 pre_partial = link.next_partial;
                 pre_groups = link.produced_groups;
diff --git a/surface_texture_inpainting_net_amd/csrc/stin_common.h b/surface_texture_inpainting_net_amd/csrc/stin_common.h
--- a/surface_texture_inpainting_net_amd/csrc/stin_common.h
+++ b/surface_texture_inpainting_net_amd/csrc/stin_common.h
@@ -145,9 +145,12 @@
     const float *G, *X, *row_w;
     float* slab;
     int64_t ldg, ldx, ld_w, M, chunks;
-    int Nc, K, Kq, has_bias, rows_per_chunk, tiles_i, tiles_j, TI, TJ, vec;
+    int Nc, K, Kq, has_bias, rows_per_chunk, tiles_i, tiles_j, vec;
+    short TI, TJ;
     unsigned block0;
+    const int32_t* x_row_map;
 };
+static_assert(sizeof(stin_tn_problem) == 152, "stin_tn_problem is a kernel argument: k_gemm_tn_ws indexes batch.p[] by this stride");
 struct stin_tn_batch {
     stin_tn_problem p[2];
     int n;
diff --git a/surface_texture_inpainting_net_amd/csrc/stin_gemm.hip b/surface_texture_inpainting_net_amd/csrc/stin_gemm.hip
--- a/surface_texture_inpainting_net_amd/csrc/stin_gemm.hip
+++ b/surface_texture_inpainting_net_amd/csrc/stin_gemm.hip
@@ -502,6 +502,7 @@
     p->G = static_cast<const float*>(G);
     p->X = static_cast<const float*>(X);
     p->row_w = static_cast<const float*>(row_w);
+    p->x_row_map = nullptr;
     p->slab = slab;
     p->ldg = ldg;
     p->ldx = ldx;
diff --git a/surface_texture_inpainting_net_amd/csrc/stin_wgrad.hip b/surface_texture_inpainting_net_amd/csrc/stin_wgrad.hip
--- a/surface_texture_inpainting_net_amd/csrc/stin_wgrad.hip
+++ b/surface_texture_inpainting_net_amd/csrc/stin_wgrad.hip
@@ -42,6 +42,7 @@
     bool pv[4];
 };
 
+template <bool MAPPED>
 __global__ __launch_bounds__(WS_THREADS) void k_gemm_tn_ws(const stin_tn_batch batch, const int prio) {
     __shared__ __attribute__((aligned(16))) __bf16 Gt[2][2][WS_PLANE];
     __shared__ __attribute__((aligned(16))) __bf16 Xt[2][2][WS_PLANE];
@@ -76,12 +77,26 @@
 
     float* out = batch.p[pi].slab + chunk * ((int64_t)Nc * Kq + ((Nc + 3) & ~3));
 
-    if (producer) {
+    auto produce = [&](auto USE_MAP) {
+        constexpr bool UM = decltype(USE_MAP)::value;
         const int ptid = tid & 255;
         const int c4 = ptid % 32, rg = (ptid / 32) ^ ((c4 >> 2) & 1);
         const float* gp = G + (i0 + c4 * 4 < Nc ? i0 + c4 * 4 : 0) + (mb + rg * 4) * ldg;
         const int xcol = j0 + c4 * 4 < K ? j0 + c4 * 4 : 0;
         const float* xp = X + xcol + (mb + rg * 4) * ldx;
+        const int32_t* __restrict__ xmap = nullptr;
+        if constexpr (UM) xmap = batch.p[pi].x_row_map;
+        const float* xb = X + xcol;
+        int4 xi = make_int4(0, 0, 0, 0);
+        auto load_map = [&](int64_t m, auto WHOLE) {
+            if constexpr (decltype(WHOLE)::value) {
+                return *reinterpret_cast<const int4*>(xmap + m);
+            } else {
+                const int64_t last = M - 1;
+                return make_int4(xmap[m < last ? m : last], xmap[m + 1 < last ? m + 1 : last], xmap[m + 2 < last ? m + 2 : last],
+                                 xmap[m + 3 < last ? m + 3 : last]);
+            }
+        };
         const stin_bn_tf xtf = batch.p[pi].xtf;
         stin_bn_coef4 xq;
         xq.s = xq.t = make_float4(0.f, 0.f, 0.f, 0.f);
@@ -89,13 +104,26 @@
         const float* wp = (want_bias && row_w != nullptr) ? row_w + (mb + rg * 4) * ld_w : nullptr;
         int64_t m_next = mb + rg * 4;
         float4 bs = make_float4(0.f, 0.f, 0.f, 0.f);
-        auto load_slab = [&](WsSlab& S, auto FULL) {
+        auto load_slab = [&](WsSlab& S, auto FULL, auto NEXT_WHOLE) {
             if (WS_ABL(4)) return;
+            const float* xm[4] = {nullptr, nullptr, nullptr, nullptr};
+            if constexpr (UM) {
+                const int4 id = xi;
+                xi = load_map(m_next + WS_R, NEXT_WHOLE);
+                xm[0] = xb + (int64_t)id.x * ldx;
+                xm[1] = xb + (int64_t)id.y * ldx;
+                xm[2] = xb + (int64_t)id.z * ldx;
+                xm[3] = xb + (int64_t)id.w * ldx;
+            }
+            auto xrow = [&](int r) -> const float* {
+                if constexpr (UM) return xm[r];
+                else return xp + r * ldx;
+            };
 #pragma unroll
             for (int r = 0; r < 4; ++r) {
                 if (decltype(FULL)::value) {
                     S.g[r] = ld4(gp + r * ldg);
-                    S.x[r] = ld4(xp + r * ldx);
+                    S.x[r] = ld4(xrow(r));
                     if (wp != nullptr) S.pw[r] = wp[r * ld_w];
                     S.pv[r] = true;
                 } else {
@@ -103,7 +131,7 @@
                     float4 vg = make_float4(0.f, 0.f, 0.f, 0.f), vx = vg;
                     if (in) {
                         vg = ld4(gp + r * ldg);
-                        vx = ld4(xp + r * ldx);
+                        vx = ld4(xrow(r));
                     }
                     S.g[r] = vg;
                     S.x[r] = vx;
@@ -112,7 +140,7 @@
                 }
             }
             gp += WS_R * ldg;
-            xp += WS_R * ldx;
+            if constexpr (!UM) xp += WS_R * ldx;
             if (wp != nullptr) wp += WS_R * ld_w;
             m_next += WS_R;
         };
@@ -152,11 +180,12 @@
         };
         WsSlab S0, S1;
         WS_STAMP(0);
-        load_slab(S0, std::false_type());
-        load_slab(S1, std::false_type());
+        if constexpr (UM) xi = load_map(m_next, std::false_type());
+        load_slab(S0, std::false_type(), std::false_type());
+        load_slab(S1, std::false_type(), std::false_type());
         store_slab(S0, 0);
         WS_STAMP(1);
-        load_slab(S0, std::false_type());
+        load_slab(S0, std::false_type(), std::false_type());
         __syncthreads();
         WS_STAMP(2);
         int64_t m0 = mb;
@@ -165,25 +194,33 @@
         for (; m0 + 5 * WS_R <= me; m0 += 2 * WS_R) {
             store_slab(S1, 1);
             WS_STAMP(st);
-            load_slab(S1, std::true_type());
+            load_slab(S1, std::true_type(), std::true_type());
             __syncthreads();
             WS_STAMP(st + 1);
             store_slab(S0, 0);
-            load_slab(S0, std::true_type());
+            load_slab(S0, std::true_type(), std::false_type());
             __syncthreads();
             st += 2;
         }
         WS_STAMP(62);
         for (; m0 < me; m0 += 2 * WS_R) {
             store_slab(S1, 1);
-            load_slab(S1, std::false_type());
+            load_slab(S1, std::false_type(), std::false_type());
             __syncthreads();
             store_slab(S0, 0);
-            load_slab(S0, std::false_type());
+            load_slab(S0, std::false_type(), std::false_type());
             __syncthreads();
         }
         WS_STAMP(63);
         if (want_bias) st4(&bsum[rg][c4 * 4], bs);
+    };
+    if (producer) {
+        if constexpr (MAPPED) {
+            if (batch.p[pi].x_row_map != nullptr) produce(std::true_type());
+            else produce(std::false_type());
+        } else {
+            produce(std::false_type());
+        }
     } else {
         const int wi = (wave >> 1) & 1, wj = wave & 1;
         const int kh = lane >> 5, li = lane & 31;
@@ -409,14 +446,17 @@
 int stin_tn_ws_launch(stin_tn_batch batch, stin_stream_t stream) {
     const int prio = 1;
     unsigned blocks = 0;
+    bool mapped = false;
     for (int i = 0; i < batch.n; ++i) {
         stin_tn_problem& p = batch.p[i];
+        mapped = mapped || p.x_row_map != nullptr;
         blocks = (blocks + 7u) & ~7u;
         p.block0 = blocks;
         blocks += (unsigned)((p.chunks >= 8 ? ((p.chunks + 7) / 8) * 8 : p.chunks) * (int64_t)p.tiles_i * p.tiles_j);
     }
     if (blocks == 0) return STIN_OK;
-    hipLaunchKernelGGL(k_gemm_tn_ws, dim3(blocks), dim3(WS_THREADS), 0, (hipStream_t)stream, batch, prio);
+    if (mapped) hipLaunchKernelGGL(k_gemm_tn_ws<true>, dim3(blocks), dim3(WS_THREADS), 0, (hipStream_t)stream, batch, prio);
+    else hipLaunchKernelGGL(k_gemm_tn_ws<false>, dim3(blocks), dim3(WS_THREADS), 0, (hipStream_t)stream, batch, prio);
     return stin_launch_status();
 }
 
@@ -435,11 +475,10 @@
                                   dW1, db1, dW2, db2, dWs, dbs, nullptr, 0, workspace, workspace_bytes, stream);
 }
 
-extern "C" int stin_edgeconv_wgrad_ti(int storage, const void* dagg, int64_t ld_dagg, const void* hE, int64_t ldh, const void* dY,
-                                      int64_t ldy, const void* x, int64_t ldx, int64_t N, int Cin, int Cp, int H, int Cout,
-                                      int has_shortcut, int trans_inv, int precision, float* dW1, float* db1, float* dW2, float* db2,
-                                      float* dWs, float* dbs, const float* ti_colsum, int64_t ti_rows, void* workspace,
-                                      size_t workspace_bytes, stin_stream_t stream) {
+static int wgrad_impl(int storage, const void* dagg, int64_t ld_dagg, const void* hE, int64_t ldh, const void* dY, int64_t ldy, const void* x,
+                      int64_t ldx, int64_t N, int Cin, int Cp, int H, int Cout, int has_shortcut, int trans_inv, int precision, float* dW1,
+                      float* db1, float* dW2, float* db2, float* dWs, float* dbs, const float* ti_colsum, int64_t ti_rows,
+                      const int32_t* x_row_map, int64_t x_rows, void* workspace, size_t workspace_bytes, stin_stream_t stream) {
     stin_clear_stale_error();
     STIN_REQUIRE(storage == 0 || storage == 1, STIN_E_UNSUPPORTED);
     STIN_REQUIRE(N >= 0 && Cin > 0 && Cp >= Cin && H > 0 && Cout > 0, STIN_E_SIZE);
@@ -450,6 +489,8 @@
     STIN_REQUIRE(ld_dagg >= Cout && ldh >= H + 1 && ldy >= Yw && ldx >= Cp, STIN_E_SIZE);
     STIN_REQUIRE(dW1 && dW2 && workspace && (!has_shortcut || dWs) && (N == 0 || (dagg && hE && dY && x)), STIN_E_NULL);
     STIN_REQUIRE(workspace_bytes >= stin_edgeconv_wgrad_workspace_bytes(N, Cp, H, Cout, has_shortcut), STIN_E_WORKSPACE);
+    STIN_REQUIRE(x_row_map == nullptr || (storage == 0 && !compact), STIN_E_UNSUPPORTED);
+    STIN_REQUIRE(x_row_map == nullptr || (x_rows > 0 && stin_aligned16(x_row_map)), STIN_E_SIZE);
     char* p = reinterpret_cast<char*>((reinterpret_cast<uintptr_t>(workspace) + 255) & ~(uintptr_t)255);
     float* slabA = reinterpret_cast<float*>(p);
     float* slabB = reinterpret_cast<float*>(p + up256(stin_gemm_tn_workspace_bytes(N, Cout, H, 1)));
@@ -461,6 +502,10 @@
     if (rc != STIN_OK) return rc;
     rc = stin_tn_problem_init(&pb, storage, dY, ldy, x, ldx, N, Yw, Cp, 1, nullptr, 0, precision, slabB, &wsb);
     if (rc != STIN_OK) return rc;
+    if (x_row_map != nullptr && N > 0) {
+        STIN_REQUIRE(wsb, STIN_E_UNSUPPORTED);
+        pb.x_row_map = x_row_map;
+    }
     if (wsa && wsb) {
         stin_tn_batch batch;
         batch.p[0] = pa;
@@ -499,6 +544,35 @@
     return stin_launch_status();
 }
 
+extern "C" int stin_edgeconv_wgrad_ti(int storage, const void* dagg, int64_t ld_dagg, const void* hE, int64_t ldh, const void* dY,
+                                      int64_t ldy, const void* x, int64_t ldx, int64_t N, int Cin, int Cp, int H, int Cout,
+                                      int has_shortcut, int trans_inv, int precision, float* dW1, float* db1, float* dW2, float* db2,
+                                      float* dWs, float* dbs, const float* ti_colsum, int64_t ti_rows, void* workspace,
+                                      size_t workspace_bytes, stin_stream_t stream) {
+    return wgrad_impl(storage, dagg, ld_dagg, hE, ldh, dY, ldy, x, ldx, N, Cin, Cp, H, Cout, has_shortcut, trans_inv, precision, dW1, db1, dW2,
+                      db2, dWs, dbs, ti_colsum, ti_rows, nullptr, 0, workspace, workspace_bytes, stream);
+}
+
+extern "C" int stin_edgeconv_wgrad_map(int storage, const void* dagg, int64_t ld_dagg, const void* hE, int64_t ldh, const void* dY,
+                                       int64_t ldy, const void* x, int64_t ldx, int64_t N, int Cin, int Cp, int H, int Cout,
+                                       int has_shortcut, int trans_inv, int precision, float* dW1, float* db1, float* dW2, float* db2,
+                                       float* dWs, float* dbs, const int32_t* x_row_map, int64_t x_rows, void* workspace,
+                                       size_t workspace_bytes, stin_stream_t stream) {
+    return wgrad_impl(storage, dagg, ld_dagg, hE, ldh, dY, ldy, x, ldx, N, Cin, Cp, H, Cout, has_shortcut, trans_inv, precision, dW1, db1, dW2,
+                      db2, dWs, dbs, nullptr, 0, x_row_map, x_rows, workspace, workspace_bytes, stream);
+}
+
+extern "C" int stin_edgeconv_wgrad_map_supported(int64_t N, int Cp, int H, int Cout, int has_shortcut, int precision) {
+    if (N <= 0 || Cp <= 0 || H <= 0 || Cout <= 0) return 0;
+    const int Yw = stin_yw(H, Cout, has_shortcut, 0);
+    stin_tn_problem pb;
+    int wsb = 0;
+    void* const some = reinterpret_cast<void*>(uintptr_t(256));
+    if (stin_tn_problem_init(&pb, 0, some, Yw, some, Cp, N, Yw, Cp, 1, nullptr, 0, precision, static_cast<float*>(some), &wsb) != STIN_OK)
+        return 0;
+    return wsb;
+}
+
 extern "C" int stin_edge_bwd_ti_colsum_fold_f32(const float* colsum, int64_t rows, int H, float* db1, stin_stream_t stream) {
     stin_clear_stale_error();
     STIN_REQUIRE(rows >= 0 && H > 0 && H % 4 == 0, STIN_E_SIZE);
diff --git a/surface_texture_inpainting_net_amd/functional.py b/surface_texture_inpainting_net_amd/functional.py
--- a/surface_texture_inpainting_net_amd/functional.py
+++ b/surface_texture_inpainting_net_amd/functional.py
@@ -844,6 +844,8 @@
 USE_NET_CALL = os.environ.get('STIN_NET_CALL', '1') != '0'
 USE_CHAIN = True
 USE_UNPOOL_COMMUTE = os.environ.get('STIN_UNPOOL_COMMUTE', '1') != '0'
+USE_WGRAD_MAP = True
+USE_G_IN_DY = True
 _NET_OP = _lib.STRUCTS['stin_net_op_t']
 OP_BLOCK, OP_POOL_MAX, OP_UNPOOL = _C['STIN_OP_BLOCK'], _C['STIN_OP_POOL_MAX'], _C['STIN_OP_UNPOOL']
 
@@ -895,6 +897,11 @@
     def _commutes(steps, si, b16, width, Ws, ti):
         return (USE_UNPOOL_COMMUTE and si > 0 and steps[si - 1][0] == 'unpool' and not b16 and Ws is not None
                 and ti != TI_MODE_COMPACT and width % 4 == 0 and Ws.shape[0] % 4 == 0)
+
+    @staticmethod
+    def _wgrad_mapped(n_rows, width, H, Cout):
+        return bool(USE_WGRAD_MAP and _lib.load().stin_edgeconv_wgrad_map_supported(int(n_rows), int(width), int(H), int(Cout), 1,
+                                                                                   int(PREC_BWD)))
 
     @staticmethod
     def forward(ctx, x, meta, *params):
@@ -950,6 +957,7 @@
                          ws_bytes=ws_bytes, edges=edges, groups=groups, ti=ti, eps=float(blk.first_norm.eps),
                          params=(W1, b1, W2, b2, Ws, bs))
                 d['src'] = plan[-1] if NetFn._commutes(steps, si, b16, width, Ws, ti) else None
+                d['xsrc'] = bool(need_grad and d['src'] is not None and d['src']['skip'])
                 d['oY'] = take((d['src']['n_in'] if d['src'] else n_rows) * Yw * es, 'tmp')
                 d['oH'] = take(n_rows * (H + pad) * es, 'tmp')
                 d['oM'] = take(max(edges.n_edges, 1) * (H // 32) * 4) if need_grad else None
@@ -971,9 +979,10 @@
                     d = dict(kind=OP_UNPOOL, pool=pool, n_in=pool.n_coarse, n_out=pool.n_fine, C=width)
                 n_rows = d['n_out']
                 nxt = steps[si + 1] if not last else None
-                d['skip'] = (stp[0] == 'unpool' and not need_grad and nxt is not None and nxt[0] == 'block' and
+                d['skip'] = (stp[0] == 'unpool' and nxt is not None and nxt[0] == 'block' and
                              NetFn._commutes(steps, si + 1, b16, width, params[pi + 4], trans_inv_mode(
-                                 nxt[1].first_filter.trans_inv, b16, params[pi].shape[0])))
+                                 nxt[1].first_filter.trans_inv, b16, params[pi].shape[0])) and
+                             (not need_grad or NetFn._wgrad_mapped(n_rows, width, params[pi].shape[0], params[pi + 2].shape[0])))
                 d['oO'] = None if (last or d['skip']) else take(n_rows * width * es, 'out')
             plan.append(d)
         if not need_grad:
@@ -1009,7 +1018,7 @@
                 H, Cout, B = d['H'], d['Cout'], d['B']
                 d['op'] = dict(kind=OP_BLOCK, Cin=d['Cin'], Cp=d['Cp'], H=H, Cout=Cout, has_shortcut=int(d['sc']), trans_inv=int(d['ti']),
                                prec_fwd=int(d['prec']), bwd_split=d['bsp'], B=B, slice_quirk=int(g.quirk), eps=d['eps'],
-                               y_from_src=int(d['src'] is not None),
+                               y_from_src=int(d['src'] is not None), x_from_src=int(d['xsrc']),
                                n_out=d['N'], n_in=d['N'], ldx=ldx, ldo=Cout, ldy=d['Yw'], ldh=H + pad, fwd_ws_bytes=d['ws_bytes'],
                                W1=_ptr(W1.contiguous()), b1=_ptr(b1), W2=_ptr(W2.contiguous()), b2=_ptr(b2), Ws=_ptr(Ws),
                                bs=_ptr(bs), rowptr_dst=_ptr(cd.rowptr), col_dst=_ptr(cd.col),
@@ -1133,6 +1142,7 @@
                 ev0, ev1 = KernelTimer.edge_events('stin_edge_relu_mean_bwd_mask' + ('_ti' if d['ti'] == TI_MODE_COMPACT else '') + sfx,
                                                    (d['N'], e.n_edges, d['H']))
                 blob.append(stc.pack(**d['op'], **NetFn._in_arena(d['rel'], base, xp), use_side=int(use[bi]), lddx=d['Cp'],
+                                     g_in_dy=int(USE_G_IN_DY and not b16 and d['sc']),
                                      bwd_ws_bytes=d['bwd_ws_bytes'], dx=p_dx,
                                      rowptr_src=_ptr(cs.rowptr), col_src=_ptr(cs.col), xslot=_ptr(e.xslot), w_src=_ptr(e.w_src),
                                      ptr_true=_ptr(gr.ptr_true), sid=_ptr(gr.sid if gr.quirk else None),
```

Result: faster. 29.06 million vertices/s, median of 6 (+2.1%).
